# bwpriest/pyNNGP

Measured on AMD Instinct MI355X. Metric: NNGP log-lik sweeps/sec (N=1M, m=15) at 1/2/4/8 MI355X; % HBM roofline, higher is better.
Workload: dtype f64

## Files before the change

### include/nngp.h

```cpp
#ifndef NNGP_H
#define NNGP_H

#include <stddef.h>
#include <stdint.h>

#ifdef __cplusplus
extern "C" {
#endif

#define NNGP_OK 0
#define NNGP_EINVAL (-1)
#define NNGP_ENOTPD (-2)
#define NNGP_EHIP (-3)
#define NNGP_EUNSUP (-4)

#define NNGP_COV_EXPONENTIAL 0
#define NNGP_COV_MATERN32 1
#define NNGP_COV_MATERN52 2
#define NNGP_COV_GAUSSIAN 3
#define NNGP_COV_SPHERICAL 4
#define NNGP_COV_MATERN 5

#define NNGP_ALGO_AUTO 0
#define NNGP_ALGO_LANE 1
#define NNGP_ALGO_WAVE 2
#define NNGP_ALGO_QUAD 4
#define NNGP_ALGO_PAIRB 5

int32_t nngp_resolve_algo(int32_t algo, int32_t m, int32_t kind, int32_t dim);
int32_t nngp_resolve_algo_nu(int32_t algo, int32_t m, int32_t kind, int32_t dim, double nu);

#define NNGP_MAX_M 63
#define NNGP_MAX_DIM 3

const char *nngp_version(void);

#define NNGP_ABI_VERSION 4
int32_t nngp_abi_version(void);

const char *nngp_last_error(void);

size_t nngp_knn_workspace_bytes(int64_t n_points, int32_t dim, int32_t m);
int nngp_knn_prior(const double *coords, int64_t n_points, int32_t dim, int32_t m, int64_t q0, int64_t q1,
                   int32_t *nbr, void *workspace, size_t workspace_bytes, void *stream);

int nngp_knn_prior_rows(const double *coords, int64_t n_points, int32_t dim, int32_t m, const int32_t *rows,
                        int64_t n_rows, int32_t *nbr, void *workspace, size_t workspace_bytes, void *stream);

int nngp_knn_query(const double *ref, int64_t n_ref, int32_t dim, const double *query, int64_t n_query, int32_t k,
                   int32_t *nbr, void *workspace, size_t workspace_bytes, void *stream);

size_t nngp_bf_sweep_workspace_bytes(int64_t n_rows, int32_t m, int32_t kind, int32_t dim, int32_t algo);
int nngp_bf_sweep(const double *coords, int64_t n_points, int32_t dim, const int32_t *nbr, const int32_t *order,
                  int64_t n_rows, int32_t m, int64_t i0, int32_t kind, double sigma2, double phi, double tau2,
                  double nu, const double *values, double *B, double *F, double *R, double *partials, void *workspace,
                  size_t workspace_bytes, int32_t algo, void *stream);
int nngp_bf_finalize(const void *workspace, size_t workspace_bytes, int64_t n_rows, int32_t m, int32_t kind,
                     int32_t dim, int32_t algo, double *partials, void *stream);

#define NNGP_PLAN_INFO_LEN 10
int nngp_pair_plan_supported(int32_t m, int32_t kind, int32_t dim);
size_t nngp_pair_plan_bytes(int64_t n_rows, int32_t m, int32_t dim);
int nngp_pair_plan_build(const int32_t *nbr, const int32_t *order, int64_t n_rows, int32_t m, int64_t i0,
                         int64_t n_points, int32_t dim, void *plan, size_t plan_bytes, int64_t *info, void *stream);
int nngp_bf_sweep_plan(const double *coords, int64_t n_points, int32_t dim, const int32_t *nbr, const int32_t *order,
                       int64_t n_rows, int32_t m, int64_t i0, int32_t kind, double sigma2, double phi, double tau2,
                       const double *values, double *B, double *F, double *R, double *partials, void *workspace,
                       size_t workspace_bytes, const void *plan, size_t plan_bytes, const int64_t *info,
                       void *stream);

int nngp_bf_cross(const double *ref, int64_t n_ref, int32_t dim, const double *query, int64_t n_query,
                  const int32_t *nbr, const int32_t *order, int64_t n_rows, int32_t m, int64_t q0, int32_t kind,
                  double sigma2, double phi, double tau2, double nu, const double *ref_values,
                  const double *query_values,
                  double *B, double *F, double *R, double *partials, void *workspace, size_t workspace_bytes,
                  int32_t algo, void *stream);

int nngp_matern_eval(const double *u, int64_t n, double nu, double *out, void *stream);
int64_t nngp_joint_entries(int32_t m);
int nngp_joint_dist(const double *coords, int64_t n_points, int32_t dim, const double *qcoords, int64_t n_locs,
                    const int32_t *nbr, const int32_t *order, int64_t n_rows, int32_t m, int64_t i0, double *dist,
                    void *stream);
size_t nngp_bf_sweep_blocks_workspace_bytes(int64_t n_rows);
int nngp_bf_sweep_blocks(const double *cov, const int32_t *nbr, const int32_t *order, int64_t n_points, int64_t n_rows,
                         int32_t m, int64_t i0, int64_t n_locs, const double *values, const double *qvalues, double *B,
                         double *F, double *R, double *partials, void *workspace, size_t workspace_bytes, void *stream);

size_t nngp_row_order_workspace_bytes(int64_t n_rows);
int nngp_row_order(const double *coords, int64_t n_points, int32_t dim, const int32_t *nbr, int32_t m, int64_t i0,
                   int64_t n_rows, int32_t *order, int32_t *nbr_sorted, void *workspace, size_t workspace_bytes,
                   void *stream);

int nngp_combine_partials(const double *gathered, int32_t world, double *partials, void *stream);
int nngp_combine_partials_batch(const double *gathered, int32_t world, int64_t n_slots, double *partials,
                                void *stream);

size_t nngp_reverse_workspace_bytes(int64_t n, int32_t m);
int nngp_reverse_neighbors(const int32_t *nbr, int64_t n, int32_t m, int32_t *off, int32_t *rev_j, int32_t *rev_k,
                           void *workspace, size_t workspace_bytes, void *stream);
int64_t nngp_color_moral_graph(const int32_t *nbr_host, const int32_t *off_host, const int32_t *rev_j_host,
                               int64_t n, int32_t m, int32_t *color_host);
int64_t nngp_color_moral_graph_dev(const int32_t *nbr, const int32_t *off, const int32_t *rev_j, int64_t n, int32_t m,
                                   int32_t *color, void *workspace, size_t workspace_bytes, void *stream);
size_t nngp_gibbs_prep_bytes(int64_t n, int32_t m);
int nngp_gibbs_prepare(const double *B, const double *Ft, const int32_t *off, const int32_t *rev_j,
                       const int32_t *rev_k, const int32_t *order, int64_t n, int32_t m, void *prep,
                       size_t prep_bytes, void *stream);
int nngp_gibbs_member_rows(const int32_t *members, int64_t n, const int32_t *off, int32_t *member_rows, void *stream);
int nngp_gibbs_w_sweep(const int32_t *member_rows, const int32_t *color_off_host, int32_t n_colors, const void *prep,
                       int64_t n, int32_t m, double sigma2, double tau2, const double *yres, const double *noise_w,
                       double *w, double *r, const int32_t *rev_j, const double *z, uint64_t seed, uint64_t sweep,
                       void *stream);
int nngp_gibbs_w_sweep_tiles(const int32_t *tiles, const int32_t *phase_off_host, const int32_t *phase_lds_host,
                             int32_t n_phases, const int32_t *tinfo, const int32_t *tstep, int32_t ecap,
                             const int32_t *tfp, const int32_t *off, const int32_t *rev_loc, const void *prep,
                             int64_t n, int32_t m, int64_t n_entries, double sigma2, double tau2, const double *yres,
                             const double *noise_w, double *w, double *r, const double *z, void *stream);
int nngp_gibbs_w_sweep_chains(const int32_t *member_rows, const int32_t *color_off_host, int32_t n_colors,
                              int32_t chains, const void *const *prep, int64_t n, int32_t m, const double *sigma2,
                              const double *tau2, const double *const *yres, const double *noise_w, double *const *w,
                              double *const *r, const int32_t *rev_j, const double *const *z, void *stream);
int nngp_gibbs_w_sweep_chains_il(const int32_t *member_rows, const int32_t *color_off_host, int32_t n_colors,
                                 int32_t chains, const void *const *prep, int64_t n, int32_t m, const double *sigma2,
                                 const double *tau2, const double *const *yres, const double *noise_w, double *w_il,
                                 double *r_il, const int32_t *rev_j, const double *const *z, void *stream);
int nngp_gibbs_normals(int64_t n, uint64_t seed, uint64_t sweep, double *z, void *stream);
int nngp_gibbs_prepare_range(const double *B, const double *Ft, const int32_t *off, const int32_t *rev_j,
                             const int32_t *rev_k, int64_t n, int32_t m, int64_t row0, int64_t row1, void *prep,
                             size_t prep_bytes, void *stream);
int nngp_gibbs_w_color(const int32_t *member_rows, int64_t n_members, const void *prep, int64_t n, int32_t m,
                       double sigma2, double tau2, const double *yres, const double *noise_w, double *w, double *r,
                       const int32_t *rev_j, const double *z, uint64_t seed, uint64_t sweep, double *w_out,
                       void *stream);
int nngp_gibbs_w_color_dev(const int32_t *member_rows, int64_t n_members, const void *prep, int64_t n, int32_t m,
                           const double *var, const double *yres, const double *noise_w, double *w, double *r,
                           const int32_t *rev_j, const double *z, double *w_out, void *stream);
int nngp_gibbs_w_apply(const int32_t *rows, int64_t n_rows, const double *w_src, const double *B, int64_t n, int32_t m,
                       double *w, double *r, const int32_t *rev_j, const int32_t *rev_k, void *stream);
size_t nngp_gibbs_stats_workspace_bytes(int64_t n, int32_t p);
int nngp_gibbs_stats(int64_t n, const double *r, const double *Ft, const double *yres, const double *y,
                     const double *X, int32_t p, const double *w, const double *noise_w, double *out,
                     void *workspace, size_t workspace_bytes, void *stream);

int nngp_check_partials(const double *partials_host, int64_t *first_bad_row, int64_t *first_bad_index);

double nngp_loglik_from_partials(const double *partials_host, int64_t n_rows);

#ifdef __cplusplus
}
#endif
#endif
```

### pynngp_amd/_lib.py

```python
from __future__ import annotations

import ctypes
import os
from typing import Optional, Tuple

import torch

_HERE = os.path.dirname(os.path.abspath(__file__))
LIB_PATH = os.environ.get("NNGP_LIB") or os.path.join(_HERE, "_build", "libnngp_hip.so")
SYMBOLS = (
    "nngp_version",
    "nngp_abi_version",
    "nngp_last_error",
    "nngp_knn_workspace_bytes",
    "nngp_knn_prior",
    "nngp_knn_prior_rows",
    "nngp_knn_query",
    "nngp_bf_sweep_workspace_bytes",
    "nngp_bf_sweep",
    "nngp_bf_cross",
    "nngp_bf_finalize",
    "nngp_resolve_algo",
    "nngp_resolve_algo_nu",
    "nngp_loglik_from_partials",
    "nngp_check_partials",
    "nngp_row_order_workspace_bytes",
    "nngp_row_order",
    "nngp_combine_partials",
    "nngp_combine_partials_batch",
    "nngp_matern_eval",
    "nngp_joint_entries",
    "nngp_joint_dist",
    "nngp_bf_sweep_blocks_workspace_bytes",
    "nngp_bf_sweep_blocks",
    "nngp_reverse_workspace_bytes",
    "nngp_reverse_neighbors",
    "nngp_color_moral_graph",
    "nngp_gibbs_prep_bytes",
    "nngp_gibbs_prepare",
    "nngp_gibbs_member_rows",
    "nngp_gibbs_w_sweep",
    "nngp_gibbs_normals",
    "nngp_gibbs_prepare_range",
    "nngp_gibbs_w_color",
    "nngp_gibbs_w_color_dev",
    "nngp_gibbs_w_apply",
    "nngp_gibbs_stats_workspace_bytes",
    "nngp_gibbs_stats",
    "nngp_gibbs_w_sweep_chains",
    "nngp_gibbs_w_sweep_chains_il",
    "nngp_gibbs_w_sweep_tiles",
    "nngp_color_moral_graph_dev",
    "nngp_pair_plan_supported",
    "nngp_pair_plan_bytes",
    "nngp_pair_plan_build",
    "nngp_bf_sweep_plan",
)

KIND_CODES = {"exponential": 0, "matern32": 1, "matern52": 2, "gaussian": 3, "spherical": 4, "matern": 5}
MATERN_NU_MAX = 50.0
ALGO_CODES = {"auto": 0, "lane": 1, "wave": 2, "quad": 4, "pairb": 5}
MAX_M = 63
MAX_DIM = 3
ABI_VERSION = 4
PLAN_INFO_LEN = 10
BLOCKS_MAX_M = 32


class NNGPExtensionError(RuntimeError):
    """The native library is missing, failed to load, or returned an error."""


_lib = None


def load() -> ctypes.CDLL:
    global _lib
    if _lib is not None:
        return _lib
    if not os.path.exists(LIB_PATH):
        raise NNGPExtensionError(
            f"{LIB_PATH} not found: build it with `python -c 'import __graft_entry__ as g; g.build()'` "
            "or `make -C pynngp_amd/csrc` (pynngp_amd has no CPU fallback)"
        )
    lib = ctypes.CDLL(LIB_PATH)
    P, I32, I64, D, SZ = ctypes.c_void_p, ctypes.c_int32, ctypes.c_int64, ctypes.c_double, ctypes.c_size_t
    lib.nngp_version.restype = ctypes.c_char_p
    lib.nngp_abi_version.restype = I32
    if lib.nngp_abi_version() != ABI_VERSION:
        raise NNGPExtensionError(f"{LIB_PATH} has C ABI revision {lib.nngp_abi_version()}, this binding needs "
                                 f"{ABI_VERSION}: rebuild the library")
    lib.nngp_last_error.restype = ctypes.c_char_p
    lib.nngp_knn_workspace_bytes.argtypes = [I64, I32, I32]
    lib.nngp_knn_workspace_bytes.restype = SZ
    lib.nngp_knn_prior.argtypes = [P, I64, I32, I32, I64, I64, P, P, SZ, P]
    lib.nngp_knn_prior.restype = ctypes.c_int
    lib.nngp_knn_prior_rows.argtypes = [P, I64, I32, I32, P, I64, P, P, SZ, P]
    lib.nngp_knn_prior_rows.restype = ctypes.c_int
    lib.nngp_knn_query.argtypes = [P, I64, I32, P, I64, I32, P, P, SZ, P]
    lib.nngp_knn_query.restype = ctypes.c_int
    lib.nngp_bf_sweep_workspace_bytes.argtypes = [I64, I32, I32, I32, I32]
    lib.nngp_bf_sweep_workspace_bytes.restype = SZ
    lib.nngp_bf_sweep.argtypes = [P, I64, I32, P, P, I64, I32, I64, I32, D, D, D, D, P, P, P, P, P, P, SZ, I32, P]
    lib.nngp_bf_cross.argtypes = [P, I64, I32, P, I64, P, P, I64, I32, I64, I32, D, D, D, D, P, P, P, P, P, P, P, SZ,
                                  I32, P]
    lib.nngp_bf_cross.restype = ctypes.c_int
    lib.nngp_row_order_workspace_bytes.argtypes = [I64]
    lib.nngp_row_order_workspace_bytes.restype = SZ
    lib.nngp_row_order.argtypes = [P, I64, I32, P, I32, I64, I64, P, P, P, SZ, P]
    lib.nngp_row_order.restype = ctypes.c_int
    lib.nngp_combine_partials.argtypes = [P, I32, P, P]
    lib.nngp_combine_partials_batch.argtypes = [P, I32, I64, P, P]
    lib.nngp_matern_eval.argtypes = [P, I64, D, P, P]
    lib.nngp_matern_eval.restype = ctypes.c_int
    lib.nngp_joint_entries.argtypes = [I32]
    lib.nngp_joint_entries.restype = I64
    lib.nngp_joint_dist.argtypes = [P, I64, I32, P, I64, P, P, I64, I32, I64, P, P]
    lib.nngp_joint_dist.restype = ctypes.c_int
    lib.nngp_bf_sweep_blocks_workspace_bytes.argtypes = [I64]
    lib.nngp_bf_sweep_blocks_workspace_bytes.restype = SZ
    lib.nngp_bf_sweep_blocks.argtypes = [P, P, P, I64, I64, I32, I64, I64, P, P, P, P, P, P, P, SZ, P]
    lib.nngp_bf_sweep_blocks.restype = ctypes.c_int
    lib.nngp_combine_partials_batch.restype = ctypes.c_int
    lib.nngp_bf_finalize.argtypes = [P, ctypes.c_size_t, I64, I32, I32, I32, I32, P, P]
    lib.nngp_bf_finalize.restype = ctypes.c_int
    lib.nngp_resolve_algo.argtypes = [I32, I32, I32, I32]
    lib.nngp_resolve_algo.restype = I32
    lib.nngp_resolve_algo_nu.argtypes = [I32, I32, I32, I32, D]
    lib.nngp_resolve_algo_nu.restype = I32
    lib.nngp_combine_partials.restype = ctypes.c_int
    U64 = ctypes.c_uint64
    lib.nngp_reverse_workspace_bytes.argtypes = [I64, I32]
    lib.nngp_reverse_workspace_bytes.restype = SZ
    lib.nngp_reverse_neighbors.argtypes = [P, I64, I32, P, P, P, P, SZ, P]
    lib.nngp_reverse_neighbors.restype = ctypes.c_int
    lib.nngp_color_moral_graph.argtypes = [P, P, P, I64, I32, P]
    lib.nngp_color_moral_graph.restype = I64
    lib.nngp_gibbs_prep_bytes.argtypes = [I64, I32]
    lib.nngp_gibbs_prep_bytes.restype = SZ
    lib.nngp_gibbs_prepare.argtypes = [P, P, P, P, P, P, I64, I32, P, SZ, P]
    lib.nngp_gibbs_prepare.restype = ctypes.c_int
    lib.nngp_gibbs_member_rows.argtypes = [P, I64, P, P, P]
    lib.nngp_gibbs_member_rows.restype = ctypes.c_int
    lib.nngp_gibbs_w_sweep.argtypes = [P, P, I32, P, I64, I32, D, D, P, P, P, P, P, P, U64, U64, P]
    lib.nngp_gibbs_w_sweep.restype = ctypes.c_int
    lib.nngp_gibbs_normals.argtypes = [I64, U64, U64, P, P]
    lib.nngp_gibbs_normals.restype = ctypes.c_int
    lib.nngp_gibbs_prepare_range.argtypes = [P, P, P, P, P, I64, I32, I64, I64, P, SZ, P]
    lib.nngp_gibbs_prepare_range.restype = ctypes.c_int
    lib.nngp_gibbs_w_color.argtypes = [P, I64, P, I64, I32, D, D, P, P, P, P, P, P, U64, U64, P, P]
    lib.nngp_gibbs_w_color.restype = ctypes.c_int
    lib.nngp_gibbs_w_color_dev.argtypes = [P, I64, P, I64, I32, P, P, P, P, P, P, P, P, P]
    lib.nngp_gibbs_w_color_dev.restype = ctypes.c_int
    lib.nngp_gibbs_w_apply.argtypes = [P, I64, P, P, I64, I32, P, P, P, P, P]
    lib.nngp_gibbs_w_apply.restype = ctypes.c_int
    lib.nngp_gibbs_stats_workspace_bytes.argtypes = [I64, I32]
    lib.nngp_gibbs_stats_workspace_bytes.restype = SZ
    lib.nngp_gibbs_stats.argtypes = [I64, P, P, P, P, P, I32, P, P, P, P, SZ, P]
    lib.nngp_gibbs_stats.restype = ctypes.c_int
    lib.nngp_bf_sweep.restype = ctypes.c_int
    lib.nngp_color_moral_graph_dev.argtypes = [P, P, P, I64, I32, P, P, SZ, P]
    lib.nngp_color_moral_graph_dev.restype = I64
    lib.nngp_gibbs_w_sweep_tiles.argtypes = [P, P, P, I32, P, P, I32, P, P, P, P, I64, I32, I64, D, D, P, P, P, P,
                                             P, P]
    lib.nngp_gibbs_w_sweep_tiles.restype = ctypes.c_int
    lib.nngp_gibbs_w_sweep_chains.argtypes = [P, P, I32, I32, P, I64, I32, P, P, P, P, P, P, P, P, P]
    lib.nngp_gibbs_w_sweep_chains.restype = ctypes.c_int
    lib.nngp_gibbs_w_sweep_chains_il.argtypes = [P, P, I32, I32, P, I64, I32, P, P, P, P, P, P, P, P, P]
    lib.nngp_gibbs_w_sweep_chains_il.restype = ctypes.c_int
    lib.nngp_pair_plan_supported.argtypes = [I32, I32, I32]
    lib.nngp_pair_plan_supported.restype = ctypes.c_int
    lib.nngp_pair_plan_bytes.argtypes = [I64, I32, I32]
    lib.nngp_pair_plan_bytes.restype = SZ
    lib.nngp_pair_plan_build.argtypes = [P, P, I64, I32, I64, I64, I32, P, SZ, P, P]
    lib.nngp_pair_plan_build.restype = ctypes.c_int
    lib.nngp_bf_sweep_plan.argtypes = [P, I64, I32, P, P, I64, I32, I64, I32, D, D, D, P, P, P, P, P, P, SZ, P, SZ, P,
                                       P]
    lib.nngp_bf_sweep_plan.restype = ctypes.c_int
    lib.nngp_check_partials.argtypes = [P, P, P]
    lib.nngp_check_partials.restype = ctypes.c_int
    lib.nngp_loglik_from_partials.argtypes = [P, I64]
    lib.nngp_loglik_from_partials.restype = D
    _lib = lib
    return lib


def version() -> str:
    return load().nngp_version().decode()


def resolve_algo(algo: str, m: int, kind: str, dim: int, nu: Optional[float] = None) -> str:
    if nu is not None:
        code = load().nngp_resolve_algo_nu(ALGO_CODES[algo], int(m), KIND_CODES[kind], int(dim), float(nu))
    else:
        code = load().nngp_resolve_algo(ALGO_CODES[algo], int(m), KIND_CODES[kind], int(dim))
    names = {v: k for k, v in ALGO_CODES.items()}
    return names.get(code, str(code))


def _check(rc: int, what: str) -> None:
    if rc != 0:
        msg = load().nngp_last_error().decode()
        raise NNGPExtensionError(f"{what} failed ({rc}): {msg}")


def _require_gpu(*tensors: Optional[torch.Tensor]) -> torch.device:
    dev = None
    for t in tensors:
        if t is None:
            continue
        if t.device.type != "cuda":
            raise NNGPExtensionError(
                f"pynngp_amd needs ROCm GPU tensors (got {t.device}); there is no CPU fallback"
            )
        if dev is None:
            dev = t.device
        elif t.device != dev:
            raise NNGPExtensionError(f"tensors on different devices: {dev} vs {t.device}")
    if dev is None:
        raise NNGPExtensionError("no tensor arguments")
    return dev


def _ptr(t: Optional[torch.Tensor]):
    return ctypes.c_void_p(t.data_ptr()) if t is not None else None


def _stream(dev: torch.device):
    return ctypes.c_void_p(torch.cuda.current_stream(dev).cuda_stream)


def _workspace(nbytes: int, dev: torch.device) -> torch.Tensor:
    ws = torch.empty(max(int(nbytes), 256), dtype=torch.uint8, device=dev)
    ws[:256].zero_()
    return ws


def _as_coords(coords: torch.Tensor) -> torch.Tensor:
    if coords.dim() != 2 or not 1 <= coords.shape[1] <= MAX_DIM or coords.dtype != torch.float64:
        raise ValueError(f"coords must be float64 (N, dim), 1 <= dim <= {MAX_DIM}, got {tuple(coords.shape)} "
                         f"{coords.dtype}")
    return coords.contiguous()


def _same_dim(*coords: torch.Tensor) -> int:
    dims = {c.shape[1] for c in coords}
    if len(dims) != 1:
        raise ValueError(f"coordinate arrays of different dimensions: {sorted(dims)}")
    return dims.pop()


def _check_out(t: Optional[torch.Tensor], name: str, shape, dev: torch.device) -> None:
    if t is None:
        return
    if t.dtype != torch.float64 or tuple(t.shape) != tuple(shape) or not t.is_contiguous() or t.device != dev:
        raise ValueError(f"{name} must be a contiguous float64 {tuple(shape)} tensor on {dev}, got "
                         f"{t.dtype} {tuple(t.shape)} contiguous={t.is_contiguous()} on {t.device}")


def knn_prior(coords: torch.Tensor, m: int, q0: int = 0, q1: Optional[int] = None,
              out: Optional[torch.Tensor] = None) -> torch.Tensor:
# ... 36 lines not shown
    query = _as_coords(query)
    d = _same_dim(ref, query)
    dev = _require_gpu(ref, query)
    out = torch.empty((query.shape[0], k), dtype=torch.int32, device=dev)
    lib = load()
    ws = _workspace(lib.nngp_knn_workspace_bytes(ref.shape[0], d, k), dev)
    _check(lib.nngp_knn_query(_ptr(ref), ref.shape[0], d, _ptr(query), query.shape[0], k, _ptr(out), _ptr(ws),
                              ws.numel(), _stream(dev)), "nngp_knn_query")
    return out


def _check_kind(kind: str, nu: Optional[float]) -> float:
    if kind not in KIND_CODES:
        raise ValueError(f"unknown covariance kind {kind!r}; expected one of {sorted(KIND_CODES)}")
    if kind == "matern":
        if nu is None or not 0.0 < float(nu) <= MATERN_NU_MAX:
            raise ValueError(f"the matern kind needs a smoothness 0 < nu <= {MATERN_NU_MAX:g} (got {nu!r})")
        return float(nu)
    return -1.0


class PairPlan:

    def __init__(self, buf: torch.Tensor, info, nbr: torch.Tensor, order: Optional[torch.Tensor]):
        self.buf = buf
        self.info = (ctypes.c_int64 * PLAN_INFO_LEN)(*info)
        self.n_planned, self.n_direct = int(info[0]), int(info[1])
        self.n_rows, self.m, self.dim, self.i0, self.n_points = (int(v) for v in info[2:7])
        self._nbr_ptr, self._order_ptr = nbr.data_ptr(), (order.data_ptr() if order is not None else 0)
        self._versions = (nbr._version, order._version if order is not None else 0)

    def matches(self, nbr: torch.Tensor, order: Optional[torch.Tensor], i0: int, n_points: int, dim: int) -> bool:
        return (nbr.data_ptr() == self._nbr_ptr and (order.data_ptr() if order is not None else 0) == self._order_ptr
                and (nbr._version, order._version if order is not None else 0) == self._versions
                and tuple(nbr.shape) == (self.n_rows, self.m) and i0 == self.i0 and n_points == self.n_points
                and dim == self.dim)


def pair_plan_read_bytes(buf: torch.Tensor, m: int) -> int:
    hdr = buf[:256].view(torch.int64).cpu()
    nreg, sb = int(hdr[6]), int(hdr[9])
    if nreg == 0:
        return 0
    wsb = sb // 4
    w = buf[256:256 + nreg * sb].view(nreg * 4, wsb)[:, :12].contiguous().view(torch.int32).long().cpu()
    nU, nE, st = w[:, 0], w[:, 1].clamp(min=0), w[:, 2]
    planned = (st.view(nreg, 4) == 0).all(1).repeat_interleave(4)
    np_ = (m + 2) // 2
    che = (np_ * np_ + 7) // 8
    per = 12 + che * 1024 + 256 + 256 * ((nU + 63) // 64) + 1024 * ((nE + 255) // 256)
    return int(per[planned].sum())


def pair_plan_supported(m: int, kind: str, dim: int) -> bool:
    return kind in KIND_CODES and bool(load().nngp_pair_plan_supported(int(m), KIND_CODES[kind], int(dim)))


def pair_plan(nbr: torch.Tensor, n_points: int, dim: int, i0: int = 0,
              order: Optional[torch.Tensor] = None) -> PairPlan:
    if nbr.dtype != torch.int32 or nbr.dim() != 2:
        raise ValueError(f"nbr must be int32 (rows, m), got {nbr.dtype} {tuple(nbr.shape)}")
    nbr = nbr.contiguous()
    dev = _require_gpu(nbr, order)
    rows, m = nbr.shape
    if order is not None and (order.dtype != torch.int32 or order.shape != (rows,)):
        raise ValueError("order must be int32 (rows,)")
    lib = load()
    nbytes = lib.nngp_pair_plan_bytes(rows, m, dim)
    if nbytes == 0:
        raise NNGPExtensionError(f"no pair plans for m={m}, dim={dim} (2 <= m <= 17, dim 1..3)")
    buf = _workspace(nbytes, dev)
    info = (ctypes.c_int64 * PLAN_INFO_LEN)()
    _check(lib.nngp_pair_plan_build(_ptr(nbr), _ptr(order), rows, m, int(i0), int(n_points), int(dim), _ptr(buf),
                                    buf.numel(), info, _stream(dev)), "nngp_pair_plan_build")
    return PairPlan(buf, list(info), nbr, order)


def bf_sweep(coords: torch.Tensor, nbr: torch.Tensor, i0: int, kind: str, sigma2: float, phi: float,
             tau2: float = 0.0, values: Optional[torch.Tensor] = None, want_bf: bool = True,
             algo: str = "auto", B: Optional[torch.Tensor] = None, F: Optional[torch.Tensor] = None,
             partials: Optional[torch.Tensor] = None, workspace: Optional[torch.Tensor] = None,
             order: Optional[torch.Tensor] = None,
             R: Optional[torch.Tensor] = None,
             defer: bool = False, nu: Optional[float] = None, plan: Optional[PairPlan] = None
             ) -> Tuple[Optional[torch.Tensor], Optional[torch.Tensor], torch.Tensor]:
    coords = _as_coords(coords)
    if nbr.dtype != torch.int32 or nbr.dim() != 2:
        raise ValueError(f"nbr must be int32 (rows, m), got {nbr.dtype} {tuple(nbr.shape)}")
    nbr = nbr.contiguous()
    if values is not None:
        if values.dtype != torch.float64 or values.shape != (coords.shape[0],):
            raise ValueError("values must be float64 (N,)")
        values = values.contiguous()
    dev = _require_gpu(coords, nbr, values, order)
    rows, m = nbr.shape
    if order is not None and (order.dtype != torch.int32 or order.shape != (rows,)):
        raise ValueError("order must be int32 (rows,)")
    nu = _check_kind(kind, nu)
    lib = load()
    a = ALGO_CODES[algo]
    if want_bf:
        _check_out(B, "B", (rows, m), dev)
        _check_out(F, "F", (rows,), dev)
        B = torch.empty((rows, m), dtype=torch.float64, device=dev) if B is None else B
        F = torch.empty((rows,), dtype=torch.float64, device=dev) if F is None else F
    else:
        B = F = None
    if defer:
        partials = None
    else:
        _check_out(partials, "partials", (4,), dev)
        partials = torch.empty(4, dtype=torch.float64, device=dev) if partials is None else partials
    d = coords.shape[1]
    need = lib.nngp_bf_sweep_workspace_bytes(rows, m, KIND_CODES[kind], d, a)
    if workspace is None or workspace.numel() < need:
        if defer:
            raise ValueError("defer=True needs a workspace of nngp_bf_sweep_workspace_bytes bytes")
        workspace = _workspace(need, dev)
    _check_out(R, "R", (rows,), dev)
    if workspace.device != dev or not workspace.is_contiguous():
        raise ValueError("workspace must be a contiguous tensor on the sweep's device")
    if plan is not None:
        if algo not in ("auto", "pairb"):
            raise ValueError(f"a pair plan runs the pair kernel, not algo {algo!r}")
        if not isinstance(plan, PairPlan) or plan.buf.device != dev:
            raise ValueError("plan must be a PairPlan on the sweep's device")
        if not plan.matches(nbr, order, i0, coords.shape[0], d):
            raise ValueError("stale pair plan: it was built for other nbr / order tensors (or they were modified in "
                             "place since) or another geometry; rebuild it with pair_plan")
        _check(lib.nngp_bf_sweep_plan(_ptr(coords), coords.shape[0], d, _ptr(nbr), _ptr(order), rows, m, i0,
                                      KIND_CODES[kind], float(sigma2), float(phi), float(tau2), _ptr(values), _ptr(B),
                                      _ptr(F), _ptr(R), _ptr(partials), _ptr(workspace), workspace.numel(),
                                      _ptr(plan.buf), plan.buf.numel(), plan.info, _stream(dev)),
               "nngp_bf_sweep_plan")
        return B, F, partials
    _check(lib.nngp_bf_sweep(_ptr(coords), coords.shape[0], d, _ptr(nbr), _ptr(order), rows, m, i0, KIND_CODES[kind],
                             float(sigma2), float(phi), float(tau2), nu, _ptr(values), _ptr(B), _ptr(F), _ptr(R),
                             _ptr(partials), _ptr(workspace), workspace.numel(), a, _stream(dev)),
           "nngp_bf_sweep")
    return B, F, partials


def bf_finalize(workspace: torch.Tensor, rows: int, m: int, kind: str, dim: int, algo: str = "auto",
                out: Optional[torch.Tensor] = None) -> torch.Tensor:
    dev = _require_gpu(workspace, out)
    out = torch.empty(4, dtype=torch.float64, device=dev) if out is None else out
    if not workspace.is_contiguous():
        raise ValueError("workspace must be contiguous")
    _check(load().nngp_bf_finalize(_ptr(workspace), workspace.numel() * workspace.element_size(), int(rows), int(m),
                                   KIND_CODES[kind], int(dim), ALGO_CODES[algo], _ptr(out), _stream(dev)),
           "nngp_bf_finalize")
    return out


def bf_cross(ref: torch.Tensor, query: torch.Tensor, nbr: torch.Tensor, kind: str, sigma2: float, phi: float,
             tau2: float = 0.0, ref_values: Optional[torch.Tensor] = None,
             query_values: Optional[torch.Tensor] = None, q0: int = 0, algo: str = "auto",
             B: Optional[torch.Tensor] = None, F: Optional[torch.Tensor] = None,
             partials: Optional[torch.Tensor] = None, workspace: Optional[torch.Tensor] = None,
             order: Optional[torch.Tensor] = None,
             R: Optional[torch.Tensor] = None, nu: Optional[float] = None) -> Tuple[torch.Tensor, torch.Tensor, torch.Tensor]:
    ref, query = _as_coords(ref), _as_coords(query)
    d = _same_dim(ref, query)
    if nbr.dtype != torch.int32 or nbr.dim() != 2:
        raise ValueError(f"nbr must be int32 (rows, m), got {nbr.dtype} {tuple(nbr.shape)}")
    nbr = nbr.contiguous()
    if ref_values is not None:
        if ref_values.dtype != torch.float64 or ref_values.shape != (ref.shape[0],):
            raise ValueError("ref_values must be float64 (n_ref,)")
        ref_values = ref_values.contiguous()
    if query_values is not None:
        if query_values.dtype != torch.float64 or query_values.shape != (query.shape[0],):
            raise ValueError("query_values must be float64 (n_query,)")
        query_values = query_values.contiguous()
    dev = _require_gpu(ref, query, nbr, ref_values, query_values, order)
    rows, m = nbr.shape
    if order is not None and (order.dtype != torch.int32 or order.shape != (rows,)):
        raise ValueError("order must be int32 (rows,)")
    nu = _check_kind(kind, nu)
    lib = load()
    a = ALGO_CODES[algo]
    _check_out(B, "B", (rows, m), dev)
    _check_out(F, "F", (rows,), dev)
    _check_out(partials, "partials", (4,), dev)
    _check_out(R, "R", (rows,), dev)
    B = torch.empty((rows, m), dtype=torch.float64, device=dev) if B is None else B
    F = torch.empty((rows,), dtype=torch.float64, device=dev) if F is None else F
    partials = torch.empty(4, dtype=torch.float64, device=dev) if partials is None else partials
    need = lib.nngp_bf_sweep_workspace_bytes(rows, m, KIND_CODES[kind], d, a)
    if workspace is None or workspace.numel() < need:
        workspace = _workspace(need, dev)
    _check(lib.nngp_bf_cross(_ptr(ref), ref.shape[0], d, _ptr(query), query.shape[0], _ptr(nbr), _ptr(order), rows, m,
                             int(q0), KIND_CODES[kind], float(sigma2), float(phi), float(tau2), nu, _ptr(ref_values),
                             _ptr(query_values), _ptr(B), _ptr(F), _ptr(R), _ptr(partials), _ptr(workspace),
                             workspace.numel(), a, _stream(dev)), "nngp_bf_cross")
    return B, F, partials


def joint_dist(coords: torch.Tensor, nbr: torch.Tensor, i0: int = 0, qcoords: Optional[torch.Tensor] = None,
               order: Optional[torch.Tensor] = None, out: Optional[torch.Tensor] = None) -> torch.Tensor:
    coords = _as_coords(coords)
    qcoords = coords if qcoords is None else _as_coords(qcoords)
    d = _same_dim(coords, qcoords)
    if nbr.dtype != torch.int32 or nbr.dim() != 2:
        raise ValueError(f"nbr must be int32 (rows, m), got {nbr.dtype} {tuple(nbr.shape)}")
    nbr = nbr.contiguous()
    dev = _require_gpu(coords, qcoords, nbr, order)
    rows, m = nbr.shape
    if order is not None and (order.dtype != torch.int32 or order.shape != (rows,)):
        raise ValueError("order must be int32 (rows,)")
    lib = load()
    ne = int(lib.nngp_joint_entries(m))
    _check_out(out, "out", (ne, rows), dev)
    out = torch.empty((ne, rows), dtype=torch.float64, device=dev) if out is None else out
    _check(lib.nngp_joint_dist(_ptr(coords), coords.shape[0], d, _ptr(qcoords), qcoords.shape[0], _ptr(nbr),
                               _ptr(order), rows, m, int(i0), _ptr(out), _stream(dev)), "nngp_joint_dist")
    return out


def matern(u: torch.Tensor, nu: float) -> torch.Tensor:
    if u.dtype != torch.float64:
        raise ValueError("u must be float64")
    dev = _require_gpu(u)
# ... 353 lines not shown
```

### pynngp_amd/csrc/bf_pairb.h

```cpp
#pragma once
#include <hip/hip_runtime.h>
#include <stdint.h>
#include <stdlib.h>
#include <string.h>

#include "bf_group.h"
#include "nngp_internal.h"
#include "nngp_math.h"
#include "pair_plan.h"

namespace nngp {

constexpr int kPairbDedupMax = 17;
constexpr int kPairbLeftMin = 18;
constexpr int kPairbLeftOneWaveMin = 23;
constexpr int kPairbLeftLdsRows = 5;
constexpr int kPairbLeftLdsRows1W = 7;
constexpr int kPairbLeftMaternM = 18;
constexpr int kPairbLeftLdsRowsMT = 6;
constexpr bool pairb_left(int m) { return m >= kPairbLeftMin && m <= 32; }
constexpr bool pairb_lk(int m, int kind) {
    return pairb_left(m) && (kind != NNGP_KIND_MATERN || m == kPairbLeftMaternM) &&
           (kind != NNGP_KIND_BLOCKS || m <= 24);
}
#ifndef NNGP_PHASE
#define NNGP_PHASE(name)
#endif
__device__ __forceinline__ double pr_swap(double v) { return dpp_f64<0xB1>(v); }
__device__ __forceinline__ double pr_from0(double v) { return dpp_f64<0xA0>(v); }
__device__ __forceinline__ double pr_from1(double v) { return dpp_f64<0xF5>(v); }
__device__ __forceinline__ double pr_sel(bool q1, double v1, double v0) { return q1 ? v1 : v0; }
__device__ __forceinline__ double pr_pick(uint32_t mask1, double v1, double v0) {
    const long long a = __double_as_longlong(v1), b = __double_as_longlong(v0);
    const uint32_t lo = ((uint32_t)a & mask1) | ((uint32_t)b & ~mask1);
    const uint32_t hi = ((uint32_t)(a >> 32) & mask1) | ((uint32_t)(b >> 32) & ~mask1);
    return __hiloint2double((int)hi, (int)lo);
}

constexpr int kPairbTwoWavesMax = 18;
constexpr int kPairbThreeWavesMax = 13;
constexpr int pairb_waves_per_simd(int m, int kind) {
    return m <= kPairbThreeWavesMax ? 3
           : (pairb_lk(m, kind) && kind == NNGP_KIND_MATERN) ? 1
           : (m <= kPairbTwoWavesMax || (pairb_lk(m, kind) && m < kPairbLeftOneWaveMin)) ? 2
                                                                                          : 1;
}
#define NNGP_PAIRB_ATTR \
    __attribute__((amdgpu_waves_per_eu(pairb_waves_per_simd(M, KIND), M <= kPairbThreeWavesMax ? 3 : 2)))

constexpr int kPairbThreads = 256;
constexpr int kPairbWaves = kPairbThreads / 64;
constexpr int kPairbTile = kPairbThreads / 2;
constexpr int kDeviceCUs = 256;

struct PairbTiling {
    int64_t tiles, q, rem;
};
inline PairbTiling pairb_tiling(int64_t n_rows, int m, int kind) {
    (void)m;
    (void)kind;
    const int64_t T = (n_rows + kPairbTile - 1) / kPairbTile;
    if (T == 0) return {0, 0, 0};
    return {T, n_rows / T, n_rows % T};
}
inline int64_t pairb_tiles_bound(int64_t n_rows) {
    const int64_t T = (n_rows + kPairbTile - 1) / kPairbTile;
    const int64_t b = T + 3 * kDeviceCUs - 1 < n_rows / 97 ? T + 3 * kDeviceCUs - 1 : n_rows / 97;
    return b > T ? b : T;
}

__device__ __forceinline__ void pairb_tile_store(double lm, int le, double qq, double badp, double badi,
                                                 double (*sh)[kPairbWaves][5], int par, double4* __restrict__ rec,
                                                 int32_t* __restrict__ lexp, int64_t tile) {
#pragma unroll
    for (int o = 32; o > 1; o >>= 1) {
        lm *= __shfl_xor(lm, o);
        le += __shfl_xor(le, o);
        qq += __shfl_xor(qq, o);
    }
    if (__any(badp != INFINITY || badi != INFINITY)) {
        badp = wave_min(badp);
        badi = wave_min(badi);
    }
    const int w = threadIdx.x >> 6;
    if ((threadIdx.x & 63) == 0) {
        sh[par][w][0] = lm;
        sh[par][w][1] = (double)le;
        sh[par][w][2] = qq;
        sh[par][w][3] = badp;
        sh[par][w][4] = badi;
    }
}

__device__ __forceinline__ void pairb_tile_fold(double (*sh)[kPairbWaves][5], int par, double4* __restrict__ rec,
                                                int32_t* __restrict__ lexp, int64_t tile) {
    double lm = 1.0, le = 0.0, qq = 0.0, bp = INFINITY, bi = INFINITY;
#pragma unroll
    for (int k = 0; k < kPairbWaves; ++k) {
        lm *= sh[par][k][0];
        le += sh[par][k][1];
        qq += sh[par][k][2];
        bp = fmin(bp, sh[par][k][3]);
        bi = fmin(bi, sh[par][k][4]);
    }
    rec[tile] = make_double4(__builtin_amdgcn_frexp_mant(lm), qq, bp, bi);
    lexp[tile] = (int32_t)le + __builtin_amdgcn_frexp_exp(lm);
// ... 25 lines not shown

__device__ __forceinline__ void pairb_fold_records(const double4* __restrict__ rec, const int32_t* __restrict__ lexp,
                                                   int64_t n_tiles, double* __restrict__ partials,
                                                   double (*sh)[5]) {
    constexpr int NT = kPairbThreads;
    const int t = threadIdx.x;
    double a = 1.0, e = 0.0, b = 0.0, c = INFINITY, d = INFINITY;
    for (int64_t k0 = t; k0 < n_tiles; k0 += 8 * NT) {
        double4 r[8];
        int32_t x[8];
#pragma unroll
        for (int u = 0; u < 8; ++u) {
            const int64_t k = k0 + (int64_t)u * NT;
            r[u] = k < n_tiles ? rec[k] : make_double4(1.0, 0.0, INFINITY, INFINITY);
            x[u] = k < n_tiles ? lexp[k] : 0;
        }
        double pm = 1.0;
        int32_t pe = 0;
#pragma unroll
        for (int u = 0; u < 8; ++u) {
            pm *= r[u].x;
            pe += x[u];
            b += r[u].y;
            c = fmin(c, r[u].z);
            d = fmin(d, r[u].w);
        }
        a *= pm;
        e += (double)pe;
        mant_norm(a, e);
    }
    a = wave_fold_dpp<1>(a);
    e = wave_fold_dpp<0>(e);
    mant_norm(a, e);
    b = wave_fold_dpp<0>(b);
    c = wave_fold_dpp<2>(c);
    d = wave_fold_dpp<2>(d);
    if ((t & 63) == 0) {
        sh[t >> 6][0] = a;
        sh[t >> 6][1] = e;
        sh[t >> 6][2] = b;
        sh[t >> 6][3] = c;
        sh[t >> 6][4] = d;
    }
    __syncthreads();
    if (t == 0) {
        a = 1.0, e = 0.0, b = 0.0, c = INFINITY, d = INFINITY;
#pragma unroll
        for (int w = 0; w < NT / 64; ++w) {
            a *= sh[w][0];
            e += sh[w][1];
            b += sh[w][2];
            c = fmin(c, sh[w][3]);
            d = fmin(d, sh[w][4]);
        }
        partials[0] = fma(e, 0.6931471805599453, log(a));
        partials[1] = b;
        partials[2] = c == INFINITY ? -1.0 : c;
        partials[3] = d == INFINITY ? -1.0 : d;
    }
}

__device__ __forceinline__ double pr_rcp(double x) {
    const double y = __builtin_amdgcn_rcp(x);
    const double e = fma(-x, y, 1.0);
    return fma(y, fma(e, e, e), y);
}

struct PairPlanArgs {
    const uint8_t* slots = nullptr;
    const int32_t* tiles = nullptr;
    int64_t slot_bytes = 0;
    int64_t n_tiles = 0;
};

template <int M, int KIND, int D, bool PL = false>
__global__ __launch_bounds__(kPairbThreads) NNGP_PAIRB_ATTR void bf_pairb(const double* __restrict__ coords, int64_t n_points,
                                                const int32_t* __restrict__ nbr, const int32_t* __restrict__ order,
                                                int64_t n_rows, int64_t i0, const CovParams Pc, double sigma2,
                                                const double* __restrict__ values, const double* __restrict__ qcoords,
                                                const double* __restrict__ qvalues, double* __restrict__ Bout,
                                                double* __restrict__ Fout, double* __restrict__ Rout,
                                                double4* __restrict__ rec, int32_t* __restrict__ lexp, int dim,
                                                const double* __restrict__ cblk, int64_t tq, int64_t trem,
                                                int64_t* __restrict__ hdr, const PairPlanArgs pp) {
    static_assert(M >= 1 && M <= 32, "pairb instantiated for 1 <= m <= 32");
    static_assert(D >= 0 && D <= 3, "0 (runtime dimension) <= D <= 3");
    constexpr bool CM = KIND == NNGP_KIND_BLOCKS;
    constexpr bool MT = KIND == NNGP_KIND_MATERN;
    constexpr int DA = point_arity<D>();
    const int ds = D == 0 ? dim : D;
    constexpr int NR = M + 1;
    constexpr int NP = (NR + 1) / 2;
    constexpr int T = M / 2;
    constexpr bool LEFT = !PL && pairb_lk(M, KIND);
    static_assert(!PL || (!CM && !MT && !LEFT && D >= 1 && M >= kPlanMinM && M <= kPlanMaxM),
                  "pair plans: the right-looking fused kinds, 1 <= D <= 3");
    constexpr int PSL = PL ? plan_slice_bytes(M) : 16;
    __shared__ __attribute__((aligned(16))) double wsl[PL ? kPairbWaves * PSL / 8 : 1];
    constexpr bool SLDL = !LEFT;
    constexpr int KL0 = MT ? kPairbLeftLdsRowsMT
                           : (M >= kPairbLeftOneWaveMin ? kPairbLeftLdsRows1W : kPairbLeftLdsRows);
    constexpr int KL = !LEFT ? 0 : (KL0 < M / 2 - 1 ? KL0 : M / 2 - 1);
    constexpr int LXW = (NP + 3 + 1) / 2;
    __shared__ double lbuf[LEFT ? NNGP_EXP_TAB_N + (KL * (KL + 1) + LXW) * kPairbThreads : 1];
    double(*const lrow)[kPairbThreads] = (double(*)[kPairbThreads])(lbuf + NNGP_EXP_TAB_N);
    int32_t(*const lidx)[kPairbThreads] =
        (int32_t(*)[kPairbThreads])(lbuf + NNGP_EXP_TAB_N + KL * (KL + 1) * kPairbThreads);
    __shared__ double etab_own[MT || LEFT ? 1 : NNGP_EXP_TAB_N];
    double* const etab = LEFT ? lbuf : etab_own;
    extern __shared__ double4 pairb_mtab[];
    const double* ctab = MT ? (const double*)pairb_mtab : etab;
    constexpr int kTabPer = kPairbThreads >= NNGP_EXP_TAB_N ? 1 : NNGP_EXP_TAB_N / kPairbThreads;
    static_assert(kPairbThreads >= NNGP_EXP_TAB_N || kTabPer * kPairbThreads == NNGP_EXP_TAB_N, "table fill");
    double etab_entry[kTabPer];
    if constexpr (!CM && !MT) {
#pragma unroll
        for (int e = 0; e < kTabPer; ++e)
            etab_entry[e] = nngp_exp_table_entry_unit(((int)threadIdx.x + e * kPairbThreads) & (NNGP_EXP_TAB_N - 1));
    }

    __shared__ double sh[1][kPairbWaves][5];
    const int64_t ltile = xcd_logical_block(blockIdx.x, gridDim.x);
    const int64_t tile = pp.tiles != nullptr ? (int64_t)__builtin_amdgcn_readfirstlane(pp.tiles[ltile]) : ltile;
    if (blockIdx.x == 0 && threadIdx.x == 0) hdr[0] = pp.tiles != nullptr ? pp.n_tiles : gridDim.x;
    const int q = (int)(threadIdx.x & 1);
    const bool q1 = q == 1;
    const bool lead0 = !q1;
    const double wq1 = q1 ? 1.0 : 0.0, wq0 = 1.0 - wq1;
    uint32_t mask1 = q1 ? 0xffffffffu : 0u;
    asm volatile("" : "+v"(mask1));
    {
        const int64_t lr = threadIdx.x >> 1;
        const int64_t r = tile * tq + (tile < trem ? tile : trem) + lr;
        const bool live = lr < tq + (tile < trem ? 1 : 0);
        const int64_t rl = live ? r : n_rows - 1;
        const int32_t ov = (order != nullptr ? order : nbr)[rl];
        const int64_t rr = order != nullptr ? (int64_t)ov : rl;
        const int64_t i = i0 + rr;

        int32_t jn[NP];
#pragma unroll
        for (int s = 0; s < NP; ++s) {
            const int a = 2 * s + q;
            jn[s] = nbr[rl * M + (a < M ? a : M - 1)];
        }
        double o[NP][DA], z[NP];
        const uint32_t n32 = n_points < (int64_t)0x80000000ll ? (uint32_t)n_points : 0x80000000u;
        int32_t jmax = -1, jmin = -1;
#pragma unroll
        for (int s = 0; s < NP; ++s) {
            const int a = 2 * s + q;
            const int32_t j = a < M ? jn[s] : -1;
            jmax = max(jmax, j);
            jmin = min(jmin, j);
            const bool in_range = (uint32_t)j < n32;
            const bool self = a == M;
            const double* pc = self ? qcoords + i * ds : (in_range ? coords + (int64_t)j * ds : far_point<DA>(a));
            const double* pv = self ? (qvalues != nullptr ? qvalues + i : kZeroValue)
                                    : ((values != nullptr && in_range) ? values + j : kZeroValue);
            if constexpr (CM || PL) {
            } else if constexpr (D == 0) {
                load_point_rt(pc, dim, o[s]);
            } else {
                load_point<D>(pc, o[s]);
            }
            if constexpr (!LEFT) z[s] = *pv;
        }
        const bool bad_index = (int64_t)jmax >= n_points || jmin < -1;
        if constexpr (LEFT) {
#pragma unroll
            for (int s = 0; s < NP; ++s) lidx[s][threadIdx.x] = jn[s];
            lidx[NP][threadIdx.x] = (int32_t)(uint32_t)(uint64_t)rr;
            lidx[NP + 1][threadIdx.x] = (int32_t)(uint32_t)((uint64_t)rr >> 32);
            lidx[NP + 2][threadIdx.x] = bad_index ? 1 : 0;
        }

        if constexpr (MT) {
            const int n4 = Pc.mt_noct * (NNGP_MT_K * NNGP_MT_NC / 4);
            const double4* g = (const double4*)cblk;
            for (int k = (int)threadIdx.x; k < n4; k += kPairbThreads) pairb_mtab[k] = g[k];
            __syncthreads();
        } else if constexpr (!CM && !PL) {
#pragma unroll
            for (int e = 0; e < kTabPer; ++e)
                if (kPairbThreads <= NNGP_EXP_TAB_N || threadIdx.x < NNGP_EXP_TAB_N)
                    etab[threadIdx.x + e * kPairbThreads] = etab_entry[e];
            __syncthreads();
        }

        double R[NP][NP][2];
        bool bad = false;
        bool stale_plan = false;
        double Fu, res;
        if constexpr (PL) {
            constexpr int CHE = plan_map_chunks(M);
            constexpr int PS = plan_ps(DA);
            constexpr int UK = plan_ucap(M) / 64;
            constexpr int64_t WSB = plan_wave_slot_bytes(M);
            const int wv = (int)(threadIdx.x >> 6), L = (int)(threadIdx.x & 63);
            const uint8_t* wsp = pp.slots + tile * pp.slot_bytes + (int64_t)__builtin_amdgcn_readfirstlane(wv) * WSB;
            const int nU0 = __builtin_amdgcn_readfirstlane(((const int32_t*)wsp)[0]);
            const int nE0 = __builtin_amdgcn_readfirstlane(((const int32_t*)wsp)[1]);
            const int st0 = __builtin_amdgcn_readfirstlane(((const int32_t*)wsp)[2]);
            const bool over = st0 != 0 || nU0 < 0 || nU0 > plan_ucap(M) || nE0 < 0 || nE0 > plan_ecap(M) ||
                              !plan_fits(nU0, nE0, PS, PSL);
            const int nU = over ? 0 : nU0, nE = over ? 0 : nE0;
            bad = over;
            const __amdgpu_buffer_rsrc_t srd =
                __builtin_amdgcn_make_buffer_rsrc((void*)wsp, (short)0, (int)WSB, 0x00020000);
            typedef uint32_t u32x4 __attribute__((ext_vector_type(4)));
            uint32_t mw[4 * CHE];
#pragma unroll
            for (int c = 0; c < CHE; ++c) {
                const u32x4 v = __builtin_amdgcn_raw_buffer_load_b128(srd, plan_map_off(M) + 16 * L, c * 64 * 16, 0);
                mw[4 * c] = v.x;
                mw[4 * c + 1] = v.y;
                mw[4 * c + 2] = v.z;
                mw[4 * c + 3] = v.w;
            }
            const uint32_t ck = __builtin_amdgcn_raw_buffer_load_b32(srd, plan_chk_off(M) + 4 * L, 0, 0);
            int32_t ug[UK];
#pragma unroll
            for (int k = 0; k < UK; ++k)
                ug[k] = (int32_t)__builtin_amdgcn_raw_buffer_load_b32(srd, plan_u_off() + 4 * L, 256 * k, 0);
            static_assert(kPlanPairGroup == 4, "one 16-byte word load per lane and group");
            constexpr int PG = kPlanPairGroup;
            constexpr int KG = plan_pair_groups(M);
            const int ngr = (nE + 64 * PG - 1) / (64 * PG);
            u32x4 wg[KG];
#pragma unroll
            for (int g = 0; g < KG; ++g)
                wg[g] = (g < 2 || g < ngr) ? __builtin_amdgcn_raw_buffer_load_b128(srd, plan_pair_off(M) + 16 * L, 1024 * g, 0)
                                           : u32x4{0u, 0u, 0u, 0u};
#pragma unroll
            for (int e = 0; e < kTabPer; ++e)
                if (kPairbThreads <= NNGP_EXP_TAB_N || threadIdx.x < NNGP_EXP_TAB_N)
                    etab[threadIdx.x + e * kPairbThreads] = etab_entry[e];
            __syncthreads();
            NNGP_PHASE(plan_points);
            char* const sl = (char*)wsl + wv * PSL;
            const int cb = PSL - nU * PS;
#pragma unroll
            for (int k = 0; k < UK; ++k) {
                if (64 * k < nU) {
                    const uint32_t g = (uint32_t)ug[k] < (uint32_t)n_points ? (uint32_t)ug[k] : 0u;
                    double x[DA];
                    load_point<DA>(coords + (int64_t)g * ds, x);
                    if (L + 64 * k < nU) {
                        double* pd = (double*)(sl + cb + (L + 64 * k) * PS);
                        if constexpr (DA == 2) {
                            *(double2*)pd = make_double2(x[0], x[1]);
// ... 45 lines not shown
            pair_points(wg[0], xa0, xb0);
            u32x4 wA = wg[KG > 1 ? 1 : 0], wB;
#pragma unroll 1
            for (int g = 0; g < ngr; g += 2) {
                wB = group_words(g + 2);
                pair_points(wA, xa1, xb1);
                pair_covs(g, xa0, xb0);
                if (g + 1 >= ngr) break;
                wA = group_words(g + 3);
                pair_points(wB, xa0, xb0);
                pair_covs(g + 1, xa1, xb1);
            }
            if (L == 0) *(double*)sl = 0.0;
            asm volatile("" ::: "memory");
            __builtin_amdgcn_wave_barrier();
            NNGP_PHASE(plan_fill);
            auto rd = [&](int e) -> double {
                const uint32_t off = (e & 1) ? (mw[e >> 1] >> 16) : (mw[e >> 1] & 0xffffu);
                return *(const double*)(sl + off);
            };
            int e = 0;
#pragma unroll
            for (int s = 0; s < NP; ++s) {
#pragma unroll
                for (int t = 0; t < s; ++t) {
                    R[s][t][0] = rd(e++);
                    R[s][t][1] = rd(e++);
                }
                R[s][s][0] = Pc.diag;
                R[s][s][1] = rd(e++);
            }
            uint32_t h = plan_chk_init((uint32_t)(uint64_t)rr);
#pragma unroll
            for (int s = 0; s < NP; ++s) h = plan_chk_step(h, jn[s], s);
            const int stale = h != ck ? 1 : 0;
            stale_plan = (stale | __builtin_amdgcn_mov_dpp(stale, 0xB1, 0xf, 0xf, true)) != 0;
        }
        uint32_t vm = 0;
        if constexpr (CM) {
#pragma unroll
            for (int s = 0; s < NP; ++s) {
                const int a = 2 * s + q;
                const bool ok = a == M || (a < M && (uint32_t)jn[s] < n32);
                vm |= ok ? (1u << a) : 0u;
            }
            vm |= (uint32_t)__builtin_amdgcn_mov_dpp((int)vm, 0xB1, 0xf, 0xf, true);
        }
        const double* cb = cblk + rl;
        auto ldc2 = [&](int a0, int b0, int a1, int b1) -> double {
            const int e0 = (a0 * (a0 + 1) >> 1) + b0, e1 = (a1 * (a1 + 1) >> 1) + b1;
            const uint32_t need = q1 ? ((1u << a1) | (1u << b1)) : ((1u << a0) | (1u << b0));
            const bool ok = (vm & need) == need;
            const int64_t e = ok ? (q1 ? e1 : e0) : 0;
            const double v = cb[e * n_rows];
            return ok ? v : 0.0;
        };
        if constexpr (CM && !LEFT) {
#pragma unroll
            for (int s = 0; s < NP; ++s) {
                const int a0 = 2 * s, a1 = 2 * s + 1;
#pragma unroll
                for (int t = 0; t < s; ++t) {
                    R[s][t][0] = ldc2(a0, 2 * t, a1, 2 * t + 1);
                    R[s][t][1] = ldc2(a0, 2 * t + 1, a1, 2 * t);
                }
                const double dg = ldc2(a0, a0, a1, a1);
                R[s][s][0] = ((vm >> (2 * s + q)) & 1u) ? dg : 1.0;
                const double w = ldc2(a0, a0, a1, a0);
                R[s][s][1] = q1 ? w : 0.0;
            }
        }
        if constexpr (!LEFT) {
        NNGP_PHASE(covariances);
        if constexpr (!CM && !PL) {
            double p[NP][DA];
#pragma unroll
            for (int t = 0; t < NP; ++t)
#pragma unroll
                for (int k = 0; k < DA; ++k) p[t][k] = pr_swap(o[t][k]);
#pragma unroll
            for (int s = 0; s < NP; ++s) {
#pragma unroll
                for (int t = 0; t < s; ++t) {
                    R[s][t][0] = nngp_cov_unit<KIND>(Pc, ctab, point_d2<DA>(o[s], o[t]));
                    R[s][t][1] = nngp_cov_unit<KIND>(Pc, ctab, point_d2<DA>(o[s], p[t]));
                }
                R[s][s][0] = Pc.diag;
            }
#pragma unroll
            for (int s0 = 0; s0 < NP; s0 += 2) {
                const int s1 = s0 + 1;
                if (M <= kPairbDedupMax && s1 < NP) {
                    double a[DA], b[DA];
#pragma unroll
                    for (int k = 0; k < DA; ++k) {
                        a[k] = pr_pick(mask1, o[s1][k], o[s0][k]);
                        b[k] = pr_pick(mask1, p[s1][k], p[s0][k]);
                    }
                    const double c = nngp_cov_unit<KIND>(Pc, ctab, point_d2<DA>(a, b));
                    R[s1][s1][1] = c;
                    R[s0][s0][1] = pr_from0(c);
                } else {
                    R[s0][s0][1] = nngp_cov_unit<KIND>(Pc, ctab, point_d2<DA>(o[s0], p[s0]));
                    if (s1 < NP) R[s1][s1][1] = nngp_cov_unit<KIND>(Pc, ctab, point_d2<DA>(o[s1], p[s1]));
                }
            }
        }

        NNGP_PHASE(elimination);
        if constexpr (SLDL) {
#pragma unroll
            for (int t = 0; t < T; ++t) {
                const double d00 = pr_from0(R[t][t][0]);
                const double d11 = pr_from1(R[t][t][0]);
                const double d10 = pr_from1(R[t][t][1]);
                bad |= !(d00 > 0.0);
                const double r00 = pr_rcp(d00);
                const double l10 = d10 * r00;
                const double e11 = fma(-l10, d10, d11);
                bad |= !(e11 > 0.0);
                const double r11 = pr_rcp(e11);
                R[t][t][1] = l10;
                const double town = pr_sel(q1, r11, r00), toth = pr_sel(q1, r00, r11);
                const double g1 = -l10 * wq1, g0 = -l10 * wq0;
#pragma unroll
                for (int s = t + 1; s < NP; ++s) {
                    const double x0 = R[s][t][0], x1 = R[s][t][1];
                    R[s][t][0] = fma(g1, x1, x0);
                    R[s][t][1] = fma(g0, x0, x1);
                }
#pragma unroll
                for (int u = t + 1; u < NP; ++u) {
                    const double Q0 = R[u][t][0] * town, Q1 = R[u][t][1] * toth;
                    const double P0 = pr_swap(Q0), P1 = pr_swap(Q1);
#pragma unroll
                    for (int s = u; s < NP; ++s) {
                        const double w0 = R[s][t][0], w1 = R[s][t][1];
                        R[s][u][0] = fma(-w0, Q0, fma(-w1, Q1, R[s][u][0]));
                        R[s][u][1] = fma(-w0, P1, fma(-w1, P0, R[s][u][1]));
                    }
                    R[u][t][0] = Q0;
                    R[u][t][1] = Q1;
                }
            }
        } else {
#pragma unroll
        for (int t = 0; t < T; ++t) {
            const double a00 = pr_from0(R[t][t][0]);
            const double a11 = pr_from1(R[t][t][0]);
            const double a10 = pr_from1(R[t][t][1]);
            bad |= !(a00 > 0.0);
            const double i00 = nngp_rsqrt(a00);
            const double l10 = a10 * i00;
            const double s11 = fma(-l10, l10, a11);
            bad |= !(s11 > 0.0);
            const double i11 = nngp_rsqrt(s11);
            R[t][t][0] = pr_sel(q1, i11, i00);
            R[t][t][1] = l10;
            const double u01 = -(l10 * i00) * i11;
            const double c00 = pr_sel(q1, i11, i00), c10 = u01 * wq1;
            const double c01 = u01 * wq0, c11 = pr_sel(q1, i00, i11);
#pragma unroll
            for (int s = t + 1; s < NP; ++s) {
                const double x0 = R[s][t][0], x1 = R[s][t][1];
                const double y0 = fma(x0, c00, x1 * c10);
                const double y1 = fma(x0, c01, x1 * c11);
                R[s][t][0] = y0;
                R[s][t][1] = y1;
            }
#pragma unroll
            for (int u = t + 1; u < NP; ++u) {
                const double S0 = R[u][t][0], S1 = R[u][t][1];
                const double P0 = pr_swap(S0), P1 = pr_swap(S1);
#pragma unroll
                for (int s = u; s < NP; ++s) {
                    const double y0 = R[s][t][0], y1 = R[s][t][1];
                    R[s][u][0] = fma(-y0, S0, fma(-y1, S1, R[s][u][0]));
                    R[s][u][1] = fma(-y0, P1, fma(-y1, P0, R[s][u][1]));
                }
            }
        }
        }

        NNGP_PHASE(lastpair);
        if (M % 2 == 1 && SLDL) {
            const double a00 = pr_from0(R[T][T][0]);
            const double a11 = pr_from1(R[T][T][0]);
            const double a10 = pr_from1(R[T][T][1]);
            bad |= !(a00 > 0.0);
            const double l10 = a10 * pr_rcp(a00);
            Fu = fma(-l10, a10, a11);
            R[T][T][0] = 1.0;
            R[T][T][1] = l10;
        } else if (M % 2 == 1) {
            const double a00 = pr_from0(R[T][T][0]);
            const double a11 = pr_from1(R[T][T][0]);
            const double a10 = pr_from1(R[T][T][1]);
            bad |= !(a00 > 0.0);
            const double i00 = nngp_rsqrt(a00);
            const double l10 = a10 * i00;
            Fu = fma(-l10, l10, a11);
            R[T][T][0] = i00;
            R[T][T][1] = l10;
        } else {
            Fu = pr_from0(R[T][T][0]);
        }
        } else {
            NNGP_PHASE(leftlooking);
            double pnext[DA], wpnext = 0.0;
#pragma unroll
            for (int u = 0; u < NP; ++u) {
                if constexpr (CM) {
#pragma unroll
                    for (int s = u + 1; s < NP; ++s) {
                        R[s][u][0] = ldc2(2 * s, 2 * u, 2 * s + 1, 2 * u + 1);
                        R[s][u][1] = ldc2(2 * s, 2 * u + 1, 2 * s + 1, 2 * u);
                    }
                    const double dg = ldc2(2 * u, 2 * u, 2 * u + 1, 2 * u + 1);
                    R[u][u][0] = ((vm >> (2 * u + q)) & 1u) ? dg : 1.0;
                    const double wv = ldc2(2 * u, 2 * u, 2 * u + 1, 2 * u);
                    R[u][u][1] = q1 ? wv : 0.0;
                } else {
                double pu[DA];
#pragma unroll
                for (int k = 0; k < DA; ++k) pu[k] = (u % 2 == 1) ? pnext[k] : pr_swap(o[u][k]);
#pragma unroll
                for (int s = u + 1; s < NP; ++s) {
                    R[s][u][0] = nngp_cov_unit<KIND>(Pc, ctab, point_d2<DA>(o[s], o[u]));
                    R[s][u][1] = nngp_cov_unit<KIND>(Pc, ctab, point_d2<DA>(o[s], pu));
                }
                R[u][u][0] = Pc.diag;
                if (u % 2 == 0 && u + 1 < NP) {
                    double a[DA], b[DA];
#pragma unroll
                    for (int k = 0; k < DA; ++k) {
                        pnext[k] = pr_swap(o[u + 1][k]);
                        a[k] = pr_pick(mask1, o[u + 1][k], o[u][k]);
                        b[k] = pr_pick(mask1, pnext[k], pu[k]);
                    }
                    wpnext = nngp_cov_unit<KIND>(Pc, ctab, point_d2<DA>(a, b));
                    R[u][u][1] = pr_from0(wpnext);
                } else if (u % 2 == 1) {
                    R[u][u][1] = wpnext;
                } else {
                    R[u][u][1] = nngp_cov_unit<KIND>(Pc, ctab, point_d2<DA>(o[u], pu));
                }
                }
#pragma unroll
                for (int t = 0; t < u; ++t) {
                    const double S0 = R[u][t][0], S1 = R[u][t][1];
                    const double P0 = pr_swap(S0), P1 = pr_swap(S1);
#pragma unroll
                    for (int s = u; s < NP; ++s) {
                        const double y0 = R[s][t][0], y1 = R[s][t][1];
                        R[s][u][0] = fma(-y0, S0, fma(-y1, S1, R[s][u][0]));
                        R[s][u][1] = fma(-y0, P1, fma(-y1, P0, R[s][u][1]));
                    }
                }
                if (u < T) {
                    const double a00 = pr_from0(R[u][u][0]);
                    const double a11 = pr_from1(R[u][u][0]);
                    const double a10 = pr_from1(R[u][u][1]);
                    bad |= !(a00 > 0.0);
                    const double i00 = nngp_rsqrt(a00);
                    const double l10 = a10 * i00;
                    const double s11 = fma(-l10, l10, a11);
                    bad |= !(s11 > 0.0);
                    const double i11 = nngp_rsqrt(s11);
                    R[u][u][0] = pr_sel(q1, i11, i00);
                    R[u][u][1] = l10;
                    const double u01 = -(l10 * i00) * i11;
                    const double c00 = pr_sel(q1, i11, i00), c10 = u01 * wq1;
                    const double c01 = u01 * wq0, c11 = pr_sel(q1, i00, i11);
#pragma unroll
                    for (int s = u + 1; s < NP; ++s) {
                        const double x0 = R[s][u][0], x1 = R[s][u][1];
                        R[s][u][0] = fma(x0, c00, x1 * c10);
                        R[s][u][1] = fma(x0, c01, x1 * c11);
                    }
                } else if (M % 2 == 1) {
                    const double a00 = pr_from0(R[T][T][0]);
                    const double a11 = pr_from1(R[T][T][0]);
                    const double a10 = pr_from1(R[T][T][1]);
                    bad |= !(a00 > 0.0);
                    const double i00 = nngp_rsqrt(a00);
                    const double l10 = a10 * i00;
                    Fu = fma(-l10, l10, a11);
                    R[T][T][0] = i00;
                    R[T][T][1] = l10;
                } else {
                    Fu = pr_from0(R[T][T][0]);
                }
                if (u < KL) {
#pragma unroll
                    for (int t = 0; t <= u; ++t) {
                        lrow[u * (u + 1) + 2 * t][threadIdx.x] = R[u][t][0];
                        lrow[u * (u + 1) + 2 * t + 1][threadIdx.x] = R[u][t][1];
                    }
                }
            }
        }
        auto RB = [&](int u, int t, int k) -> double {
            if (u < KL) return lrow[u * (u + 1) + 2 * t + k][threadIdx.x];
            return R[u][t][k];
        };
        bad |= !(Fu > 0.0);
        const double F = Fu * sigma2;
        int64_t rrl = rr, il = i;
        bool bidx = bad_index || stale_plan;
        if constexpr (LEFT) {
            __builtin_amdgcn_fence(__ATOMIC_ACQUIRE, "workgroup");
            rrl = (int64_t)(((uint64_t)(uint32_t)lidx[NP + 1][threadIdx.x] << 32) | (uint32_t)lidx[NP][threadIdx.x]);
            il = i0 + rrl;
            bidx = lidx[NP + 2][threadIdx.x] != 0;
        }

        {
            constexpr int SM = M / 2;
            constexpr bool VQ1 = (M % 2) == 1;
            NNGP_PHASE(backsub);
            if constexpr (LEFT) {
#pragma unroll
                for (int s = 0; s < NP; ++s) {
                    const int a = 2 * s + q;
                    const int32_t j = a < M ? lidx[s][threadIdx.x] : -1;
                    const bool in_range = (uint32_t)j < n32;
                    const double* pv = a == M ? (qvalues != nullptr ? qvalues + il : kZeroValue)
                                              : ((values != nullptr && in_range) ? values + j : kZeroValue);
                    z[s] = *pv;
                }
            }
            double bown[NP];
#pragma unroll
            for (int s = 0; s < NP; ++s) bown[s] = 0.0;
            if (M % 2 == 1) bown[T] = RB(T, T, 1) * RB(T, T, 0);
#pragma unroll
            for (int t = T - 1; t >= 0; --t) {
                double acc0 = 0.0, acc1 = 0.0;
#pragma unroll
                for (int u = t + 1; u < NP; ++u) {
                    if (2 * u >= M) continue;
                    const bool row_ok = 2 * u + 1 < M;
                    double bu = bown[u];
                    if (!row_ok) bu = q1 ? 0.0 : bu;
                    acc0 = fma(RB(u, t, 0), bu, acc0);
                    acc1 = fma(RB(u, t, 1), bu, acc1);
                }
                const double tot = acc0 + pr_swap(acc1);
                const double vrow0 = RB(SM, t, 0), vrow1 = RB(SM, t, 1);
                double v;
                if (VQ1) {
                    v = pr_sel(q1, vrow0, pr_swap(vrow1));
                } else {
                    v = pr_sel(q1, pr_swap(vrow1), vrow0);
                }
                const double l10 = RB(t, t, 1);
                double bx, b0;
                if constexpr (SLDL) {
                    bx = v - tot;
                    b0 = fma(-l10, pr_swap(bx), bx);
                } else {
                    const double iown = RB(t, t, 0);
                    bx = (v - tot) * iown;
                    b0 = fma(-(l10 * iown), pr_swap(bx), bx);
                }
                bown[t] = pr_sel(q1, bx, b0);
            }
            NNGP_PHASE(residual);
            {
                double acc = 0.0;
#pragma unroll
                for (int s = 0; s < NP; ++s) {
                    if (2 * s >= M) continue;
                    double bs = bown[s];
                    if (2 * s + 1 >= M) bs = q1 ? 0.0 : bs;
                    acc = fma(bs, z[s], acc);
                }
                const double zm = z[SM];
                const double vi = VQ1 ? pr_from1(zm) : pr_from0(zm);
                res = vi - (acc + pr_swap(acc));
            }
            NNGP_PHASE(stores);
            if (Bout != nullptr && live) {
                const double bscale = (bad || stale_plan) ? NAN : 1.0;
#pragma unroll
                for (int s = 0; s < NP; ++s) {
                    const int a = 2 * s + q;
                    if (a < M) Bout[rrl * M + a] = bown[s] * bscale;
                }
            }
        }
        NNGP_PHASE(tail);
        const bool lead = live && lead0;
        if (Fout != nullptr && lead) Fout[rrl] = (bad || stale_plan) ? NAN : F;
        if (Rout != nullptr && lead) Rout[rrl] = (bad || stale_plan) ? NAN : res;
        pairb_tile_store(lead ? __builtin_amdgcn_frexp_mant(F) : 1.0, lead ? __builtin_amdgcn_frexp_exp(F) : 0,
                         lead ? res * res * pr_rcp(F) : 0.0, (lead && bad) ? (double)il : INFINITY,
                         (live && bidx) ? (double)il : INFINITY, sh, 0, rec, lexp, tile);
        __syncthreads();
        if (threadIdx.x == 0) pairb_tile_fold(sh, 0, rec, lexp, tile);
    }
}

inline size_t pairb_align(size_t b) { return (b + 255) & ~(size_t)255; }
constexpr size_t kPairbHeader = 256;
inline size_t bf_pairb_workspace_bytes(int64_t n_rows) {
    const int64_t t = pairb_tiles_bound(n_rows);
    return t > 0 ? kPairbHeader + pairb_align((size_t)t * 32) + pairb_align((size_t)t * 4) : 0;
}
inline int64_t* pairb_hdr(void* ws) { return (int64_t*)ws; }
inline double4* pairb_rec(void* ws) { return (double4*)((char*)ws + kPairbHeader); }
inline int32_t* pairb_lexp(void* ws, int64_t n_rows) {
    return (int32_t*)((char*)ws + kPairbHeader + pairb_align((size_t)pairb_tiles_bound(n_rows) * 32));
}

template <int M, int KIND, int D, bool PL = false>
static void launch_pairb_mkd(const BfArgs& a, const CovParams& Pc, hipStream_t s, const PairPlanArgs* ppl = nullptr) {
    const size_t lds = KIND == NNGP_KIND_MATERN ? NNGP_MT_BYTES(Pc.mt_noct) : 0;
    const PairbTiling tl = pairb_tiling(a.n_rows, M, KIND);
    PairPlanArgs pp = ppl != nullptr ? *ppl : PairPlanArgs{};
    if (!PL && a.tiles != nullptr) {
        pp.tiles = a.tiles;
        pp.n_tiles = a.n_tiles;
    }
    const int64_t nb = PL ? a.n_plan_blocks : (a.tiles != nullptr ? a.n_tile_list : tl.tiles);
    if (nb == 0) return;
    hipLaunchKernelGGL((bf_pairb<M, KIND, D, PL>), dim3((unsigned)nb), dim3(kPairbThreads), lds, s, a.coords,
                       a.n_points, a.nbr, a.order, a.n_rows, a.i0, Pc, KIND == NNGP_KIND_BLOCKS ? 1.0 : a.sigma2, a.values,
                       a.qcoords, a.qvalues, a.B, a.F, a.R, pairb_rec(a.bpart), pairb_lexp(a.bpart, a.n_rows), a.dim,
                       a.cblk, tl.q, tl.rem, pairb_hdr(a.bpart), pp);
}

template <int M, int KIND, int D>
static void launch_pairb_planned_mkd(const BfArgs& a, const CovParams& Pc, const PlanLaunch& pl, hipStream_t s) {
    PairPlanArgs pp;
    pp.slots = pl.plan + kPlanGlobalHdr;
    pp.slot_bytes = pl.slot_bytes;
    pp.n_tiles = pl.n_regions;
    pp.tiles = pl.planned;
    BfArgs b = a;
    b.n_plan_blocks = pl.n_planned;
    launch_pairb_mkd<M, KIND, D, true>(b, Pc, s, &pp);
}

template <int M, int D>
static bool launch_pairb_planned_if(const BfArgs& a, const CovParams& Pc, const PlanLaunch& pl, hipStream_t s) {
    if (a.m != M || a.dim != D) return false;
    switch (a.kind) {
        case 0: launch_pairb_planned_mkd<M, 0, D>(a, Pc, pl, s); return true;
        case 1: launch_pairb_planned_mkd<M, 1, D>(a, Pc, pl, s); return true;
        case 2: launch_pairb_planned_mkd<M, 2, D>(a, Pc, pl, s); return true;
        case 3: launch_pairb_planned_mkd<M, 3, D>(a, Pc, pl, s); return true;
        case 4: launch_pairb_planned_mkd<M, 4, D>(a, Pc, pl, s); return true;
        default: return false;
    }
}

template <int M>
static bool launch_pairb_generic_if(const BfArgs& a, const CovParams& Pc, hipStream_t s) {
    if (a.m != M) return false;
    launch_pairb_mkd<M, NNGP_KIND_GENERIC, 0>(a, Pc, s);
    return true;
}

template <int M>
static bool launch_pairb_blocks_if(const BfArgs& a, const CovParams& Pc, hipStream_t s) {
    if (a.m != M) return false;
    launch_pairb_mkd<M, NNGP_KIND_BLOCKS, 2>(a, Pc, s);
    return true;
}

template <int M, int D>
static bool launch_pairb_if(const BfArgs& a, const CovParams& Pc, hipStream_t s) {
    if (a.m != M || a.dim != D) return false;
    switch (a.kind) {
        case 0: launch_pairb_mkd<M, 0, D>(a, Pc, s); return true;
        case 1: launch_pairb_mkd<M, 1, D>(a, Pc, s); return true;
        case 2: launch_pairb_mkd<M, 2, D>(a, Pc, s); return true;
        case 3: launch_pairb_mkd<M, 3, D>(a, Pc, s); return true;
        case 4: launch_pairb_mkd<M, 4, D>(a, Pc, s); return true;
        case NNGP_KIND_MATERN:
            if constexpr (M <= 24) {
                launch_pairb_mkd<M, NNGP_KIND_MATERN, D>(a, Pc, s);
                return true;
            } else {
                return false;
            }
        default: return false;
    }
}

}
```

### pynngp_amd/csrc/capi.hip

```cpp
#include <hip/hip_runtime.h>
#include <math.h>
#include <stdarg.h>
#include <stdio.h>
#include <string.h>

#include "../../include/nngp.h"
#include "nngp_internal.h"
#include "bf_pairb.h"

namespace {
thread_local char g_err[512] = "";

int fail(int code, const char* fmt, ...) {
    va_list ap;
    va_start(ap, fmt);
    vsnprintf(g_err, sizeof g_err, fmt, ap);
    va_end(ap);
    return code;
}

int hip_fail(hipError_t e, const char* what) {
    return fail(NNGP_EHIP, "%s: %s", what, hipGetErrorString(e));
}

size_t align256(size_t x) { return (x + 255) & ~(size_t)255; }

int resolve_algo(int32_t algo, int32_t m, int32_t kind, int32_t dim) {
    (void)dim;
    if (algo != NNGP_ALGO_AUTO) return algo;
    if (kind == NNGP_COV_MATERN)
        return m >= 1 && m <= 24 ? nngp::kAlgoPairB : (m >= 25 && m <= 32 ? nngp::kAlgoQuad : nngp::kAlgoWave);
    if (m >= 1 && m <= 32) return m == 31 ? nngp::kAlgoQuad : nngp::kAlgoPairB;
    return nngp::kAlgoWave;
}

int resolve_algo_nu(int32_t algo, int32_t m, int32_t kind, int32_t dim, double nu) {
    const int a = resolve_algo(algo, m, kind, dim);
    if (algo != NNGP_ALGO_AUTO || kind != NNGP_COV_MATERN || (a != nngp::kAlgoPairB && a != nngp::kAlgoQuad)) return a;
    int e0, noct;
    return nu > 0.0 && nu <= NNGP_MATERN_NU_MAX && nngp::matern_table_extent(nu, &e0, &noct) ? a : nngp::kAlgoWave;
}

int64_t bf_blocks(int64_t n_rows, int algo, int m) { return nngp::bf_record_count(n_rows, algo, m); }
}

extern "C" {

const char* nngp_version(void) { return "pynngp_amd 0.4.0 gfx950"; }

int32_t nngp_abi_version(void) { return NNGP_ABI_VERSION; }

const char* nngp_last_error(void) { return g_err; }

int32_t nngp_resolve_algo(int32_t algo, int32_t m, int32_t kind, int32_t dim) { return resolve_algo(algo, m, kind, dim); }

int32_t nngp_resolve_algo_nu(int32_t algo, int32_t m, int32_t kind, int32_t dim, double nu) {
    return resolve_algo_nu(algo, m, kind, dim, nu);
}

int nngp_check_partials(const double* p, int64_t* first_bad_row, int64_t* first_bad_index) {
    if (p == nullptr) return fail(NNGP_EINVAL, "partials must be non-null");
    if (first_bad_row != nullptr) *first_bad_row = p[2] >= 0.0 ? (int64_t)p[2] : -1;
    if (first_bad_index != nullptr) *first_bad_index = p[3] >= 0.0 ? (int64_t)p[3] : -1;
    if (p[3] >= 0.0) return fail(NNGP_EINVAL, "neighbour index out of range at location %lld", (long long)p[3]);
    if (p[2] >= 0.0) return fail(NNGP_ENOTPD, "C_N or F not positive definite at location %lld", (long long)p[2]);
    return NNGP_OK;
}

double nngp_loglik_from_partials(const double* p, int64_t n_rows) {
    return -0.5 * ((double)n_rows * 1.8378770664093453 + p[0] + p[1]);
}

size_t nngp_bf_sweep_workspace_bytes(int64_t n_rows, int32_t m, int32_t kind, int32_t dim, int32_t algo) {
    if (n_rows < 0 || m < 0 || m > NNGP_MAX_M) return 0;
    const int a = resolve_algo(algo, m, kind, dim);
    const int64_t nbw = n_rows > 0 ? bf_blocks(n_rows, nngp::kAlgoWave, m) : 0;
    if (kind == NNGP_COV_MATERN && a == nngp::kAlgoPairB) {
        const size_t pb = nngp::bf_pairb_workspace_bytes(n_rows) + align256(NNGP_MT_BYTES(NNGP_MT_MAX_OCT));
        const size_t wb = align256((size_t)nbw * 4 * sizeof(double));
        return algo == NNGP_ALGO_AUTO && wb > pb ? wb : pb;
    }
    if (kind == NNGP_COV_MATERN && a == nngp::kAlgoQuad) {
        const int64_t nq = n_rows > 0 ? bf_blocks(n_rows, nngp::kAlgoQuad, m) : 0;
        const size_t qb = align256((size_t)nq * 4 * sizeof(double)) + align256(NNGP_MT_BYTES(NNGP_MT_MAX_OCT));
        const size_t wb = align256((size_t)nbw * 4 * sizeof(double));
        return algo == NNGP_ALGO_AUTO && wb > qb ? wb : qb;
    }
    if (a == nngp::kAlgoPairB) return nngp::bf_pairb_workspace_bytes(n_rows);
    const int64_t nb = n_rows > 0 ? bf_blocks(n_rows, a, m) : 0;
    return align256((size_t)nb * 4 * sizeof(double));
}

static int bf_common(const double* coords, int64_t n_points, int32_t dim, const double* qcoords, int64_t n_locs,
                     const int32_t* nbr, const int32_t* order, int64_t n_rows, int32_t m, int64_t i0, int32_t kind,
                     double sigma2, double phi, double tau2, double nu, const double* values, const double* qvalues, double* B,
                     double* F, double* R, double* partials, void* workspace, size_t workspace_bytes, int32_t algo,
                     void* stream) {
    if (coords == nullptr || qcoords == nullptr || workspace == nullptr)
        return fail(NNGP_EINVAL, "coordinates and workspace must be non-null");
    if (dim < 1 || dim > NNGP_MAX_DIM) return fail(NNGP_EUNSUP, "dim=%d outside [1, %d]", dim, NNGP_MAX_DIM);
    if (m < 0 || m > NNGP_MAX_M) return fail(NNGP_EUNSUP, "m=%d outside [0, %d]", m, NNGP_MAX_M);
    if (m > 0 && n_rows > 0 && nbr == nullptr) return fail(NNGP_EINVAL, "nbr must be non-null for m > 0");
    if (n_points < 1 || n_rows < 0 || i0 < 0 || i0 + n_rows > n_locs)
        return fail(NNGP_EINVAL, "rows [%lld, %lld) outside [0, %lld)", (long long)i0, (long long)(i0 + n_rows),
                    (long long)n_locs);
    if (kind < NNGP_COV_EXPONENTIAL || kind > NNGP_COV_MATERN) return fail(NNGP_EINVAL, "unknown kind %d", kind);
    if (!(sigma2 > 0.0) || !(phi > 0.0) || !(tau2 >= 0.0) || !isfinite(sigma2) || !isfinite(phi) || !isfinite(tau2))
        return fail(NNGP_EINVAL, "theta must satisfy sigma2 > 0, phi > 0, tau2 >= 0 (finite)");
    if (kind == NNGP_COV_MATERN && !(nu > 0.0 && nu <= NNGP_MATERN_NU_MAX))
        return fail(NNGP_EINVAL, "the matern kind needs 0 < nu <= %g (nu=%g)", NNGP_MATERN_NU_MAX, nu);
    if (B != nullptr && F == nullptr) return fail(NNGP_EINVAL, "B given without F");
    if (F != nullptr && B == nullptr && m > 0 && n_rows > 0) return fail(NNGP_EINVAL, "F given without B");
    if (R != nullptr && values == nullptr) return fail(NNGP_EINVAL, "R (residuals) needs values");
    if (((uintptr_t)workspace & 255) != 0) return fail(NNGP_EINVAL, "workspace must be 256-byte aligned");
    int a = resolve_algo_nu(algo, m, kind, dim, nu);
    if (a != nngp::kAlgoLane && a != nngp::kAlgoWave && a != nngp::kAlgoQuad && a != nngp::kAlgoPairB)
        return fail(NNGP_EINVAL, "unknown algo %d", algo);
    if (kind == NNGP_COV_MATERN && a != nngp::kAlgoWave && a != nngp::kAlgoPairB && a != nngp::kAlgoQuad)
        return fail(NNGP_EUNSUP, "the matern kind runs on the pair (m <= 24), four-lane (25..32) or wavefront kernel, "
                                 "not algo %d", algo);
    if (kind == NNGP_COV_MATERN && (a == nngp::kAlgoPairB || a == nngp::kAlgoQuad)) {
        int e0, noct;
        if (!nngp::matern_table_extent(nu, &e0, &noct))
            return fail(NNGP_EUNSUP, "matern nu=%g needs %d table octaves (> %d; nu below ~%g): use NNGP_ALGO_AUTO or "
                                     "WAVE", nu, noct, NNGP_MT_MAX_OCT, NNGP_MT_NU_MIN);
    }
    const bool classic = dim == 2 && kind <= NNGP_COV_MATERN32;
    if (a == nngp::kAlgoLane && !classic)
        return fail(NNGP_EUNSUP, "the lane kernel serves 2-D exponential and Matern-3/2 only "
                                 "(kind=%d, dim=%d): use NNGP_ALGO_AUTO, PAIRB, QUAD or WAVE", kind, dim);
    if (a == nngp::kAlgoLane && (m < 1 || m > nngp::kLaneMaxM))
        return fail(NNGP_EUNSUP, "lane kernel needs 1 <= m <= %d (m=%d)", nngp::kLaneMaxM, m);
    if (a == nngp::kAlgoQuad && !nngp::bf_group_supported(m, 4))
        return fail(NNGP_EUNSUP, "no 4-lane kernel instantiated for m=%d (25..32)", m);
    if (a == nngp::kAlgoPairB && !nngp::bf_pairb_supported(m))
        return fail(NNGP_EUNSUP, "no blocked pair kernel instantiated for m=%d", m);
    if (a == nngp::kAlgoPairB && kind == NNGP_COV_MATERN && m > 24)
        return fail(NNGP_EUNSUP, "the matern kind runs on the pair kernel for m <= 24 (m=%d): use NNGP_ALGO_AUTO or "
                                 "QUAD", m);
    const size_t need = nngp_bf_sweep_workspace_bytes(n_rows, m, kind, dim, algo);
    if (workspace_bytes < need)
        return fail(NNGP_EINVAL, "workspace too small: %zu < %zu bytes", workspace_bytes, need);

    hipStream_t s = (hipStream_t)stream;
    nngp::BfArgs args{coords, n_points, nbr, n_rows, i0, m, kind, dim, sigma2, phi, tau2, nu, order, values, qcoords,
                      qvalues, B, F, R, partials, (double*)workspace};
    hipError_t e = nngp::bf_launch(args, a, s);
    if (e != hipSuccess) return hip_fail(e, "bf_sweep launch");
    return NNGP_OK;
}

int nngp_bf_sweep(const double* coords, int64_t n_points, int32_t dim, const int32_t* nbr, const int32_t* order,
                  int64_t n_rows, int32_t m, int64_t i0, int32_t kind, double sigma2, double phi, double tau2,
                  double nu, const double* values, double* B, double* F, double* R, double* partials, void* workspace,
                  size_t workspace_bytes, int32_t algo, void* stream) {
    return bf_common(coords, n_points, dim, coords, n_points, nbr, order, n_rows, m, i0, kind, sigma2, phi, tau2, nu,
                     values, values, B, F, R, partials, workspace, workspace_bytes, algo, stream);
}

int nngp_bf_cross(const double* ref, int64_t n_ref, int32_t dim, const double* query, int64_t n_query,
                  const int32_t* nbr, const int32_t* order, int64_t n_rows, int32_t m, int64_t q0, int32_t kind,
                  double sigma2, double phi, double tau2, double nu, const double* ref_values,
                  const double* query_values, double* B, double* F, double* R, double* partials, void* workspace,
                  size_t workspace_bytes, int32_t algo, void* stream) {
    if (query_values != nullptr && ref_values == nullptr)
        return fail(NNGP_EINVAL, "query_values need ref_values");
    return bf_common(ref, n_ref, dim, query, n_query, nbr, order, n_rows, m, q0, kind, sigma2, phi, tau2, nu, ref_values,
                     query_values, B, F, R, partials, workspace, workspace_bytes, algo, stream);
}

int nngp_pair_plan_supported(int32_t m, int32_t kind, int32_t dim) {
    return nngp::bf_pairb_planned_supported(m, kind, dim) ? 1 : 0;
}

size_t nngp_pair_plan_bytes(int64_t n_rows, int32_t m, int32_t dim) {
    if (n_rows < 0 || n_rows > INT32_MAX || !nngp::bf_pairb_planned_supported(m, 0, dim)) return 0;
    return (size_t)nngp::plan_total_bytes(n_rows, m);
}

int nngp_pair_plan_build(const int32_t* nbr, const int32_t* order, int64_t n_rows, int32_t m, int64_t i0,
                         int64_t n_points, int32_t dim, void* plan, size_t plan_bytes, int64_t* info, void* stream) {
    if (plan == nullptr || info == nullptr || (n_rows > 0 && nbr == nullptr))
        return fail(NNGP_EINVAL, "plan, info (and nbr for n_rows > 0) must be non-null");
    if (!nngp::bf_pairb_planned_supported(m, 0, dim))
        return fail(NNGP_EUNSUP, "pair plans serve 2 <= m <= 17, dim 1..3 (m=%d, dim=%d)", m, dim);
    if (n_rows < 0 || n_rows > INT32_MAX || i0 < 0 || n_points < 1 || i0 + n_rows > n_points || n_points > INT32_MAX)
        return fail(NNGP_EINVAL, "rows [%lld, %lld) outside [0, %lld) (or n_rows / n_points >= 2^31)", (long long)i0,
                    (long long)(i0 + n_rows), (long long)n_points);
    if (((uintptr_t)plan & 255) != 0) return fail(NNGP_EINVAL, "plan must be 256-byte aligned");
    const size_t need = (size_t)nngp::plan_total_bytes(n_rows, m);
    if (plan_bytes < need) return fail(NNGP_EINVAL, "plan too small: %zu < %zu bytes", plan_bytes, need);
    hipStream_t s = (hipStream_t)stream;
    const nngp::PairbTiling tl = nngp::pairb_tiling(n_rows, m, 0);
    if (tl.tiles != nngp::plan_regions(n_rows)) return fail(NNGP_EUNSUP, "plan regions differ from the pair tiling");
    hipError_t e = nngp::pair_plan_build_launch(nbr, order, n_rows, m, dim, i0, n_points, tl.q, tl.rem, plan, s);
    if (e != hipSuccess) return hip_fail(e, "pair_plan build");
    nngp::PlanHeader h;
    e = hipMemcpyAsync(&h, plan, sizeof h, hipMemcpyDeviceToHost, s);
    if (e == hipSuccess) e = hipStreamSynchronize(s);
    if (e != hipSuccess) return hip_fail(e, "pair_plan counts");
    info[0] = h.n_planned;
    info[1] = h.n_direct;
    info[2] = n_rows;
    info[3] = m;
    info[4] = dim;
    info[5] = i0;
    info[6] = n_points;
    info[7] = nngp::kPlanMagic;
    info[8] = (int64_t)(uintptr_t)nbr;
    info[9] = (int64_t)(uintptr_t)order;
    return NNGP_OK;
}

int nngp_bf_sweep_plan(const double* coords, int64_t n_points, int32_t dim, const int32_t* nbr, const int32_t* order,
                       int64_t n_rows, int32_t m, int64_t i0, int32_t kind, double sigma2, double phi, double tau2,
                       const double* values, double* B, double* F, double* R, double* partials, void* workspace,
                       size_t workspace_bytes, const void* plan, size_t plan_bytes, const int64_t* info,
                       void* stream) {
    if (coords == nullptr || workspace == nullptr || plan == nullptr || info == nullptr)
        return fail(NNGP_EINVAL, "coordinates, workspace, plan and info must be non-null");
    if (info[7] != nngp::kPlanMagic || info[2] != n_rows || info[3] != m || info[4] != dim || info[5] != i0 ||
        info[6] != n_points)
        return fail(NNGP_EINVAL, "the plan was built for (n_rows %lld, m %lld, dim %lld, i0 %lld, n_points %lld), not "
                                 "this sweep's (%lld, %d, %d, %lld, %lld)", (long long)info[2], (long long)info[3],
                    (long long)info[4], (long long)info[5], (long long)info[6], (long long)n_rows, m, dim,
                    (long long)i0, (long long)n_points);
    if (info[8] != (int64_t)(uintptr_t)nbr || info[9] != (int64_t)(uintptr_t)order)
        return fail(NNGP_EINVAL, "stale plan: it was built for other nbr / order buffers (rebuild it with the "
                                 "sweep's neighbour sets)");
    if (!nngp::bf_pairb_planned_supported(m, kind, dim))
        return fail(NNGP_EUNSUP, "planned sweeps serve kinds 0..4, 2 <= m <= 17, dim 1..3 (kind=%d)", kind);
    if (plan_bytes < (size_t)nngp::plan_total_bytes(n_rows, m)) return fail(NNGP_EINVAL, "plan too small");
    const int64_t nreg = nngp::plan_regions(n_rows);
    if (info[0] < 0 || info[1] < 0 || info[0] + info[1] != nreg)
        return fail(NNGP_EINVAL, "plan counts %lld + %lld != %lld tiles", (long long)info[0], (long long)info[1],
                    (long long)nreg);
    if (m < 1 || (n_rows > 0 && nbr == nullptr)) return fail(NNGP_EINVAL, "nbr must be non-null");
    if (!(sigma2 > 0.0) || !(phi > 0.0) || !(tau2 >= 0.0) || !isfinite(sigma2) || !isfinite(phi) || !isfinite(tau2))
        return fail(NNGP_EINVAL, "theta must satisfy sigma2 > 0, phi > 0, tau2 >= 0 (finite)");
    if (B != nullptr && F == nullptr) return fail(NNGP_EINVAL, "B given without F");
// ... 486 lines not shown
```

### pynngp_amd/csrc/nngp_internal.h

```cpp
#pragma once
#include <hip/hip_runtime.h>
#include <stdint.h>

#include "nngp_math.h"
#include "pair_plan.h"

namespace nngp {

constexpr double kFar = 1e150;
static __device__ double2 kFarPoints[64] = {{1e150, 0.0}, {2e150, 0.0}, {3e150, 0.0}, {4e150, 0.0}, {5e150, 0.0}, {6e150, 0.0}, {7e150, 0.0}, {8e150, 0.0}, {9e150, 0.0}, {10e150, 0.0}, {11e150, 0.0}, {12e150, 0.0}, {13e150, 0.0}, {14e150, 0.0}, {15e150, 0.0}, {16e150, 0.0}, {17e150, 0.0}, {18e150, 0.0}, {19e150, 0.0}, {20e150, 0.0}, {21e150, 0.0}, {22e150, 0.0}, {23e150, 0.0}, {24e150, 0.0}, {25e150, 0.0}, {26e150, 0.0}, {27e150, 0.0}, {28e150, 0.0}, {29e150, 0.0}, {30e150, 0.0}, {31e150, 0.0}, {32e150, 0.0}, {33e150, 0.0}, {34e150, 0.0}, {35e150, 0.0}, {36e150, 0.0}, {37e150, 0.0}, {38e150, 0.0}, {39e150, 0.0}, {40e150, 0.0}, {41e150, 0.0}, {42e150, 0.0}, {43e150, 0.0}, {44e150, 0.0}, {45e150, 0.0}, {46e150, 0.0}, {47e150, 0.0}, {48e150, 0.0}, {49e150, 0.0}, {50e150, 0.0}, {51e150, 0.0}, {52e150, 0.0}, {53e150, 0.0}, {54e150, 0.0}, {55e150, 0.0}, {56e150, 0.0}, {57e150, 0.0}, {58e150, 0.0}, {59e150, 0.0}, {60e150, 0.0}, {61e150, 0.0}, {62e150, 0.0}, {63e150, 0.0}, {64e150, 0.0}};
static __device__ double kZeroValue[1] = {0.0};
static __device__ double kFarPoints1[64] = {1e150, 2e150, 3e150, 4e150, 5e150, 6e150, 7e150, 8e150, 9e150, 10e150, 11e150, 12e150, 13e150, 14e150, 15e150, 16e150, 17e150, 18e150, 19e150, 20e150, 21e150, 22e150, 23e150, 24e150, 25e150, 26e150, 27e150, 28e150, 29e150, 30e150, 31e150, 32e150, 33e150, 34e150, 35e150, 36e150, 37e150, 38e150, 39e150, 40e150, 41e150, 42e150, 43e150, 44e150, 45e150, 46e150, 47e150, 48e150, 49e150, 50e150, 51e150, 52e150, 53e150, 54e150, 55e150, 56e150, 57e150, 58e150, 59e150, 60e150, 61e150, 62e150, 63e150, 64e150};
static __device__ double kFarPoints3[64 * 3] = {1e150, 0.0, 0.0, 2e150, 0.0, 0.0, 3e150, 0.0, 0.0, 4e150, 0.0, 0.0, 5e150, 0.0, 0.0, 6e150, 0.0, 0.0, 7e150, 0.0, 0.0, 8e150, 0.0, 0.0, 9e150, 0.0, 0.0, 10e150, 0.0, 0.0, 11e150, 0.0, 0.0, 12e150, 0.0, 0.0, 13e150, 0.0, 0.0, 14e150, 0.0, 0.0, 15e150, 0.0, 0.0, 16e150, 0.0, 0.0, 17e150, 0.0, 0.0, 18e150, 0.0, 0.0, 19e150, 0.0, 0.0, 20e150, 0.0, 0.0, 21e150, 0.0, 0.0, 22e150, 0.0, 0.0, 23e150, 0.0, 0.0, 24e150, 0.0, 0.0, 25e150, 0.0, 0.0, 26e150, 0.0, 0.0, 27e150, 0.0, 0.0, 28e150, 0.0, 0.0, 29e150, 0.0, 0.0, 30e150, 0.0, 0.0, 31e150, 0.0, 0.0, 32e150, 0.0, 0.0, 33e150, 0.0, 0.0, 34e150, 0.0, 0.0, 35e150, 0.0, 0.0, 36e150, 0.0, 0.0, 37e150, 0.0, 0.0, 38e150, 0.0, 0.0, 39e150, 0.0, 0.0, 40e150, 0.0, 0.0, 41e150, 0.0, 0.0, 42e150, 0.0, 0.0, 43e150, 0.0, 0.0, 44e150, 0.0, 0.0, 45e150, 0.0, 0.0, 46e150, 0.0, 0.0, 47e150, 0.0, 0.0, 48e150, 0.0, 0.0, 49e150, 0.0, 0.0, 50e150, 0.0, 0.0, 51e150, 0.0, 0.0, 52e150, 0.0, 0.0, 53e150, 0.0, 0.0, 54e150, 0.0, 0.0, 55e150, 0.0, 0.0, 56e150, 0.0, 0.0, 57e150, 0.0, 0.0, 58e150, 0.0, 0.0, 59e150, 0.0, 0.0, 60e150, 0.0, 0.0, 61e150, 0.0, 0.0, 62e150, 0.0, 0.0, 63e150, 0.0, 0.0, 64e150, 0.0, 0.0};

template <int D>
__device__ __forceinline__ const double* far_point(int a) {
    if constexpr (D == 1) return kFarPoints1 + (a & 63);
    else if constexpr (D == 2) return (const double*)(kFarPoints + (a & 63));
    else return kFarPoints3 + 3 * (a & 63);
}
template <int D>
constexpr int point_arity() { return D == 0 ? 3 : D; }

template <int D>
__device__ __forceinline__ void load_point(const double* __restrict__ p, double (&x)[D]) {
    if constexpr (D == 2) {
        const double2 v = *(const double2*)p;
        x[0] = v.x;
        x[1] = v.y;
    } else {
#pragma unroll
        for (int k = 0; k < D; ++k) x[k] = p[k];
    }
}

__device__ __forceinline__ void load_point_rt(const double* __restrict__ p, int dim, double (&x)[3]) {
#pragma unroll
    for (int k = 0; k < 3; ++k) x[k] = *(k < dim ? p + k : kZeroValue);
}

template <int D>
__device__ __forceinline__ double point_d2(const double (&a)[D], const double (&b)[D]) {
    double acc = NNGP_D2_FLOOR;
#pragma unroll
    for (int k = D - 1; k >= 0; --k) {
        const double t = a[k] - b[k];
        acc = fma(t, t, acc);
    }
    return acc;
}

constexpr int kAlgoAuto = 0;
constexpr int kAlgoLane = 1;
constexpr int kAlgoWave = 2;
constexpr int kAlgoQuad = 4;
constexpr int kAlgoPairB = 5;
constexpr int kLaneMaxM = 16;

struct BfArgs {
    const double* coords;
    int64_t n_points;
    const int32_t* nbr;
    int64_t n_rows;
    int64_t i0;
    int m;
    int kind;
    int dim;
    double sigma2, phi, tau2;
    double nu;
    const int32_t* order;
    const double* values;
    const double* qcoords;
    const double* qvalues;
    double* B;
    double* F;
    double* R;
    double* partials;
    double* bpart;
    const double* cblk = nullptr;
    const int32_t* tiles = nullptr;
    int64_t n_tiles = 0, n_tile_list = 0, n_plan_blocks = 0;
};

int64_t bf_record_count(int64_t n_rows, int algo, int m);
hipError_t bf_finalize_launch(const double* bpart, int64_t n_records, double* partials, hipStream_t s);
hipError_t bf_finalize_pairb_launch(void* ws, int64_t n_rows, double* partials, hipStream_t s);
hipError_t bf_launch(const BfArgs& a, int algo, hipStream_t s);
hipError_t combine_partials_launch(const double* gathered, int world, int64_t n_slots, double* out, hipStream_t s);
bool bf_wave_launch(const BfArgs& a, const CovParams& P, int64_t n_blocks, hipStream_t s);
bool bf_group_launch(const BfArgs& a, const CovParams& P, int lanes, hipStream_t s);
bool bf_group_supported(int m, int lanes);
bool bf_pairb_launch(const BfArgs& a, const CovParams& P, hipStream_t s);
bool bf_pairb_supported(int m);
bool bf_pairb_blocks_launch(const BfArgs& a, hipStream_t s);
bool bf_pairb_planned_supported(int m, int kind, int dim);
bool bf_pairb_planned_launch(const BfArgs& a, const CovParams& P, const PlanLaunch& pl, hipStream_t s);
hipError_t bf_launch_planned(const BfArgs& a, const PlanLaunch& pl, hipStream_t s);
size_t pair_plan_build_lds(int m);
hipError_t pair_plan_build_launch(const int32_t* nbr, const int32_t* order, int64_t n_rows, int m, int dim, int64_t i0,
                                  int64_t n_points, int64_t tq, int64_t trem, void* plan, hipStream_t s);
bool bf_pairb_blocks_supported(int m);
bool bf_group_blocks_launch(const BfArgs& a, hipStream_t s);
bool bf_group_blocks_supported(int m);
hipError_t matern_table_launch(const CovParams& P, double* tab, hipStream_t s);
bool matern_table_extent(double nu, int* e0, int* noct);
bool matern_table_params(double nu, CovParams* p);
hipError_t matern_eval_launch(const double* u, int64_t n, double nu, double* out, hipStream_t s);
hipError_t joint_dist_launch(const double* coords, int64_t n_points, int dim, const double* qcoords,
                             const int32_t* nbr, const int32_t* order, int64_t n_rows, int m, int64_t i0, double* dist,
                             hipStream_t s);
int64_t bf_group_blocks(int64_t n_rows, int lanes);
int64_t bf_lane_blocks(int64_t n_rows);
int64_t bf_wave_blocks(int64_t n_rows);

constexpr int kKnnMaxLevels = 16;
struct KnnLevel {
    int64_t np;
    int g;
    int64_t n_cells;
    size_t off_idx_sorted, off_pts_sorted, off_cell_start;
};
struct KnnPlan {
    int64_t n_points;
    int dim;
    int g;
    int64_t n_cells;
    int n_levels;
    KnnLevel lv[kKnnMaxLevels];
    size_t sort_temp_bytes;
    size_t total_bytes;
    size_t off_bbox, off_key, off_key_sorted, off_sort_temp, off_idx, off_perm;
};

hipError_t knn_plan(int64_t n_points, int dim, KnnPlan* plan);
hipError_t knn_launch(bool prior, const double* coords, int64_t n_points, int m, const double* query, int64_t q0,
                      int64_t q1, const int32_t* rows, int32_t* nbr, void* workspace, const KnnPlan& plan,
                      hipStream_t s);

size_t reverse_workspace_bytes(int64_t n, int m);
hipError_t reverse_launch(const int32_t* nbr, int64_t n, int m, int32_t* off, int32_t* rev_j, int32_t* rev_k,
                          void* workspace, hipStream_t s);
int64_t color_moral_graph_host(const int32_t* nbr, const int32_t* off, const int32_t* rev_j, int64_t n, int m,
                               int32_t* color);
int64_t color_moral_graph_device(const int32_t* nbr, const int32_t* off, const int32_t* rev_j, int64_t n, int m,
                                 int32_t* color, void* workspace, hipStream_t s, hipError_t* err);
size_t gibbs_prep_bytes(int64_t n, int m);
hipError_t philox_normals_launch(int64_t n, uint64_t seed, uint64_t sweep, double* z, hipStream_t s);
hipError_t gibbs_prepare_launch(const double* B, const double* Ft, const int32_t* off, const int32_t* rev_j,
                                const int32_t* rev_k, const int32_t* order, int64_t n, int m, void* prep,
                                hipStream_t s);
hipError_t gibbs_prepare_range_launch(const double* B, const double* Ft, const int32_t* off, const int32_t* rev_j,
                                      const int32_t* rev_k, int64_t n, int m, int64_t row0, int64_t row1, void* prep,
                                      hipStream_t s);
hipError_t gibbs_w_color_launch(const int32_t* member_rows, int64_t n_members, const void* prep, int64_t n, int m,
                                double sigma2, double tau2, const double* yres, const double* noise_w, double* w,
                                double* r, const int32_t* rev_j, const double* z, uint64_t seed, uint64_t sweep,
                                double* w_out, const double* var, hipStream_t s);
hipError_t gibbs_w_apply_launch(const int32_t* rows, int64_t n_rows, const double* wsrc, const double* B, int m,
                                double* w, double* r, const int32_t* rev_j, const int32_t* rev_k, hipStream_t s);
hipError_t gibbs_member_rows_launch(const int32_t* members, int64_t n, const int32_t* off, int32_t* rows,
                                    hipStream_t s);
hipError_t gibbs_tile_sweep_launch(const int32_t* tiles, const int32_t* phase_off_host, const int32_t* phase_lds_host,
                                   int n_phases, const int32_t* tinfo, const int32_t* tstep, int ecap,
                                   const int32_t* tfp, const int32_t* off, const int32_t* rev_loc, const void* prep,
                                   int64_t n, int m, int64_t n_entries, double sigma2, double tau2,
                                   const double* yres, const double* noise_w, double* w, double* r, const double* z,
                                   hipStream_t s);
hipError_t gibbs_w_sweep_launch(const int32_t* member_rows, int n_colors, const int32_t* color_off_host,
                                const void* prep, int64_t n, int m, double sigma2, double tau2,
                                const double* yres, const double* noise_w, double* w, double* r,
                                const int32_t* rev_j, const double* z, uint64_t seed, uint64_t sweep, hipStream_t s);
hipError_t gibbs_w_sweep_chains_launch(const int32_t* member_rows, int n_colors, const int32_t* color_off_host,
                                       int chains, const void* const* preps, int64_t n, int m, const double* sigma2,
                                       const double* tau2, const double* const* yres, const double* noise_w,
                                       double* const* w, double* const* r, const int32_t* rev_j,
                                       const double* const* z, hipStream_t s, double* w_il = nullptr,
                                       double* r_il = nullptr);
size_t gibbs_stats_workspace_bytes(int64_t n, int p);
hipError_t gibbs_stats_launch(int64_t n, const double* r, const double* Ft, const double* yres, const double* y,
                              const double* X, int p, const double* w, const double* noise_w, double* out,
                              void* workspace, hipStream_t s);

size_t row_order_workspace_bytes(int64_t n_rows);
// ... 63 lines not shown
```

### pynngp_amd/csrc/nngp_math.h

```cpp
#pragma once

#include "exp2_table.h"
#include "rgamma_series.h"

#ifdef NNGP_MATH_HOST
#include <math.h>
#include <string.h>
#include <stdint.h>
#define NNGP_FN static inline
#define NNGP_HD static inline
static inline double nngp_rsq_approx(double x) {
    double y = 1.0 / sqrt(x);
    uint64_t u;
    memcpy(&u, &x, 8);
    return y * ((u >> 7) & 1 ? 1.0 + 0x1p-24 : 1.0 - 0x1p-24);
}
static inline int32_t nngp_lo_dword(double t) {
    uint64_t u;
    memcpy(&u, &t, 8);
    return (int32_t)(uint32_t)u;
}
static const double kExp2Tab[256] = NNGP_EXP2_TAB;
#else
#include <hip/hip_runtime.h>
// ... 344 lines not shown
    const double g = e * fma(0.375, e, 0.5);
    return fma(s, g, s);
}

NNGP_FN double nngp_rsqrt(double x) {
    const double y = nngp_rsq_approx(x);
    const double e = fma(-(x * y), y, 1.0);
    const double g = e * fma(0.375, e, 0.5);
    return fma(y, g, y);
}

template <int KIND>
NNGP_FN double nngp_cov_d2(const CovParams& P, const double* tab, double d2) {
    const double x = fmin(d2, P.d2max);
    if (KIND == NNGP_KIND_GAUSSIAN) return nngp_exp_tab(P, tab, x);
    const double d = nngp_sqrt(x);
    if (KIND == NNGP_KIND_MATERN) return P.sigma2 * nngp_matern_rho(P, P.phi * d);
    if (KIND == NNGP_KIND_GENERIC) {
        const double e = nngp_exp_tab(P, tab, P.gauss ? x : d);
        const double u = fmin(P.phi * d, P.umax);
        return fma(u, fma(u, fma(u, P.c[2], P.c[1]), P.c[0]), 1.0) * e;
    }
    if (KIND == NNGP_KIND_SPHERICAL) {
        const double u = fmin(P.phi * d, 1.0);
        const double p = fma(u, fma(0.5 * u, u, -1.5), 1.0);
        return P.sigma2 * p;
    }
    const double e = nngp_exp_tab(P, tab, d);
    if (KIND == NNGP_KIND_MATERN32) {
        const double pd = P.phi * d;
        return fma(pd, e, e);
    }
    if (KIND == NNGP_KIND_MATERN52) {
        const double u = P.phi * d;
        const double p = fma(fma(u, 1.0 / 3.0, 1.0), u, 1.0);
        return p * e;
    }
    return e;
}

NNGP_FN double nngp_d2(double ax, double ay, double bx, double by) {
    const double dx = ax - bx;
    const double dy = ay - by;
    return fma(dx, dx, fma(dy, dy, NNGP_D2_FLOOR));
}

#define NNGP_UNIT_CLAMP (1023.0 + 1.0 / 1024.0)
NNGP_HD CovParams nngp_cov_params_unit(int kind, double phi, double tau2_over_sigma2) {
    CovParams p = nngp_cov_params(kind, 1.0, phi, tau2_over_sigma2);
    if (kind == NNGP_KIND_GAUSSIAN) {
        p.d2max = NNGP_UNIT_CLAMP / (phi * phi * NNGP_LOG2E);
    } else if (kind != NNGP_KIND_SPHERICAL) {
        const double dmax = NNGP_UNIT_CLAMP / (phi * NNGP_LOG2E);
        p.d2max = dmax * dmax;
    }
    return p;
}

NNGP_FN double nngp_exp_unit(const CovParams& P, const double* tab, double u) {
    const double t = fma(P.nphi256, u, NNGP_EXP_MAGIC);
    const double k = t - NNGP_EXP_MAGIC;
    const double f = fma(P.nphi256, u, -k);
    const int32_t ki = nngp_lo_dword(t);
    const double Tadj = tab[ki & (NNGP_EXP_TAB_N - 1)];
    constexpr double Q[4] = NNGP_EXP2_Q;
    double q = fma(Q[3], f, Q[2]);
    q = fma(q, f, Q[1]);
    q = fma(q, f, Q[0]);
    const double fq = f * q;
#ifdef NNGP_MATH_HOST
    uint64_t bits;
    memcpy(&bits, &Tadj, 8);
    bits += (uint64_t)((uint32_t)ki << 12) << 32;
    double Ts;
    memcpy(&Ts, &bits, 8);
#else
    const long long tb = __double_as_longlong(Tadj);
    const int32_t hi = (int32_t)(tb >> 32) + (int32_t)((uint32_t)ki << 12);
    const double Ts = __hiloint2double(hi, (int32_t)(tb & 0xffffffffll));
#endif
    return fma(Ts, fq, Ts);
}

template <int KIND>
NNGP_FN double nngp_cov_unit(const CovParams& P, const double* tab, double d2) {
    if (KIND == NNGP_KIND_MATERN) return nngp_matern_tab(P, tab, d2);
    const double x = fmin(d2, P.d2max);
    if (KIND == NNGP_KIND_GAUSSIAN) return nngp_exp_unit(P, tab, x);
    const double d = nngp_sqrt(x);
    if (KIND == NNGP_KIND_SPHERICAL) {
        const double u = fmin(P.phi * d, 1.0);
        return fma(u, fma(0.5 * u, u, -1.5), 1.0);
    }
    if (KIND == NNGP_KIND_GENERIC) {
        const double e = nngp_exp_unit(P, tab, P.gauss ? x : d);
        const double u = fmin(P.phi * d, P.umax);
        return fma(u, fma(u, fma(u, P.c[2], P.c[1]), P.c[0]), 1.0) * e;
    }
    const double e = nngp_exp_unit(P, tab, d);
    if (KIND == NNGP_KIND_MATERN32) return fma(P.phi * d, e, e);
    if (KIND == NNGP_KIND_MATERN52) {
        const double u = P.phi * d;
        return fma(fma(u, 1.0 / 3.0, 1.0), u, 1.0) * e;
    }
    return e;
}

#ifndef NNGP_MATH_HOST
NNGP_FN double nngp_exp_table_entry_unit(int j) {
    const long long b = __double_as_longlong(kExp2Tab[j]);
    return __hiloint2double((int32_t)(b >> 32) - (j << 12), (int32_t)(b & 0xffffffffll));
}
NNGP_FN double nngp_exp_table_fetch_unit() { return nngp_exp_table_entry_unit((int)threadIdx.x & (NNGP_EXP_TAB_N - 1)); }
NNGP_FN void nngp_exp_table_store_unit(double* tab, double v) {
    if (threadIdx.x < NNGP_EXP_TAB_N) tab[threadIdx.x] = v;
    __syncthreads();
}

NNGP_FN void nngp_exp_table_load_unit(double* tab) {
    for (int j = threadIdx.x; j < NNGP_EXP_TAB_N; j += blockDim.x) {
        const long long b = __double_as_longlong(kExp2Tab[j]);
        tab[j] = __hiloint2double((int32_t)(b >> 32) - (j << 12), (int32_t)(b & 0xffffffffll));
    }
    __syncthreads();
}
#else
static inline void nngp_exp_table_load_unit(double* tab) {
    for (int j = 0; j < NNGP_EXP_TAB_N; ++j) {
        uint64_t b;
        memcpy(&b, &kExp2Tab[j], 8);
        b -= (uint64_t)((uint32_t)j << 12) << 32;
        memcpy(&tab[j], &b, 8);
    }
}
#endif
```

### pynngp_amd/csrc/torch_ops.cpp

```cpp
#include <ATen/ATen.h>
#include <ATen/hip/HIPContext.h>
#include <c10/core/DeviceGuard.h>
#include <torch/library.h>

#include "../../include/nngp.h"

namespace {

void* stream(const at::Tensor& t) { return (void*)at::hip::getCurrentHIPStream(t.device().index()).stream(); }

void check_rc(int rc, const char* what) { TORCH_CHECK(rc == NNGP_OK, what, " failed (", rc, "): ", nngp_last_error()); }

void check_coords(const at::Tensor& c, const char* name) {
    TORCH_CHECK(c.is_cuda(), name, " must be a ROCm GPU tensor (there is no CPU fallback)");
    TORCH_CHECK(c.scalar_type() == at::kDouble && c.dim() == 2 && c.size(1) >= 1 && c.size(1) <= NNGP_MAX_DIM,
                name, " must be float64 (N, dim), 1 <= dim <= ", NNGP_MAX_DIM);
    TORCH_CHECK(c.is_contiguous(), name, " must be contiguous");
}

void check_same_device(const at::Tensor& a, const at::Tensor& b, const char* name) {
    TORCH_CHECK(b.device() == a.device(), name, " is on ", b.device(), ", expected ", a.device());
}

void check_f64(const c10::optional<at::Tensor>& t, at::IntArrayRef shape, const at::Tensor& like, const char* name) {
    if (!t.has_value()) return;
    TORCH_CHECK(t->scalar_type() == at::kDouble && t->sizes() == shape && t->is_contiguous(), name,
                " must be a contiguous float64 tensor of shape ", shape);
    check_same_device(like, *t, name);
}

void check_nbr(const at::Tensor& nbr, const at::Tensor& like) {
    TORCH_CHECK(nbr.scalar_type() == at::kInt && nbr.dim() == 2 && nbr.is_contiguous(),
                "nbr must be a contiguous int32 (rows, m) tensor");
    check_same_device(like, nbr, "nbr");
}

template <typename T>
T* ptr(const c10::optional<at::Tensor>& t) {
    return t.has_value() ? (T*)t->data_ptr() : nullptr;
}

at::Tensor workspace(int64_t bytes, const at::Tensor& like) {
    auto ws = at::empty({bytes > 256 ? bytes : 256}, like.options().dtype(at::kByte));
    ws.narrow(0, 0, 256).zero_();
    return ws;
}

at::Tensor knn_prior(const at::Tensor& coords, int64_t m, int64_t q0, int64_t q1) {
    check_coords(coords, "coords");
    const at::OptionalDeviceGuard guard(coords.device());
    const int64_t n = coords.size(0), d = coords.size(1);
    TORCH_CHECK(0 <= q0 && q0 <= q1 && q1 <= n, "query rows [", q0, ", ", q1, ") outside [0, ", n, ")");
    auto out = at::empty({q1 - q0, m}, coords.options().dtype(at::kInt));
    auto ws = workspace((int64_t)nngp_knn_workspace_bytes(n, (int32_t)d, (int32_t)m), coords);
    check_rc(nngp_knn_prior(coords.data_ptr<double>(), n, (int32_t)d, (int32_t)m, q0, q1, out.data_ptr<int32_t>(),
                            ws.data_ptr(), ws.numel(), stream(coords)),
             "nngp_knn_prior");
    return out;
}

at::Tensor knn_prior_rows(const at::Tensor& coords, int64_t m, const at::Tensor& rows) {
    check_coords(coords, "coords");
    const at::OptionalDeviceGuard guard(coords.device());
    TORCH_CHECK(rows.scalar_type() == at::kInt && rows.dim() == 1 && rows.is_contiguous(), "rows must be int32 (n_rows,)");
    check_same_device(coords, rows, "rows");
    const int64_t n = coords.size(0), d = coords.size(1);
    auto out = at::empty({rows.size(0), m}, coords.options().dtype(at::kInt));
    auto ws = workspace((int64_t)nngp_knn_workspace_bytes(n, (int32_t)d, (int32_t)m), coords);
    check_rc(nngp_knn_prior_rows(coords.data_ptr<double>(), n, (int32_t)d, (int32_t)m, rows.data_ptr<int32_t>(),
                                 rows.size(0), out.data_ptr<int32_t>(), ws.data_ptr(), ws.numel(), stream(coords)),
             "nngp_knn_prior_rows");
    return out;
}

at::Tensor knn_query(const at::Tensor& ref, const at::Tensor& query, int64_t k) {
    check_coords(ref, "ref");
    const at::OptionalDeviceGuard guard(ref.device());
    check_coords(query, "query");
    check_same_device(ref, query, "query");
    TORCH_CHECK(ref.size(1) == query.size(1), "ref and query have different dimensions");
    const int64_t d = ref.size(1);
    auto out = at::empty({query.size(0), k}, ref.options().dtype(at::kInt));
    auto ws = workspace((int64_t)nngp_knn_workspace_bytes(ref.size(0), (int32_t)d, (int32_t)k), ref);
    check_rc(nngp_knn_query(ref.data_ptr<double>(), ref.size(0), (int32_t)d, query.data_ptr<double>(), query.size(0),
                            (int32_t)k, out.data_ptr<int32_t>(), ws.data_ptr(), ws.numel(), stream(ref)),
             "nngp_knn_query");
    return out;
}

void bf_sweep_out(const at::Tensor& coords, const at::Tensor& nbr, const c10::optional<at::Tensor>& order, int64_t i0,
                  int64_t kind, double sigma2, double phi, double tau2, const c10::optional<at::Tensor>& values,
                  const c10::optional<at::Tensor>& B, const c10::optional<at::Tensor>& F,
                  const c10::optional<at::Tensor>& R, const at::Tensor& partials, const at::Tensor& ws,
                  int64_t algo, double nu, const c10::optional<at::Tensor>& plan,
                  const c10::optional<at::Tensor>& plan_info) {
    check_coords(coords, "coords");
    const at::OptionalDeviceGuard guard(coords.device());
    check_nbr(nbr, coords);
    const int64_t rows = nbr.size(0), m = nbr.size(1), n = coords.size(0), d = coords.size(1);
    if (order.has_value()) {
        TORCH_CHECK(order->scalar_type() == at::kInt && order->sizes() == at::IntArrayRef{rows} && order->is_contiguous(),
                    "order must be a contiguous int32 (rows,) tensor");
        check_same_device(coords, *order, "order");
    }
    check_f64(values, {n}, coords, "values");
    check_f64(B, {rows, m}, coords, "B");
    check_f64(F, {rows}, coords, "F");
    check_f64(R, {rows}, coords, "R");
    check_f64(partials, {4}, coords, "partials");
    TORCH_CHECK(ws.is_contiguous(), "workspace must be contiguous");
    check_same_device(coords, ws, "workspace");
    if (plan.has_value()) {
        TORCH_CHECK(plan_info.has_value() && plan_info->device().is_cpu() && plan_info->scalar_type() == at::kLong &&
                        plan_info->numel() == NNGP_PLAN_INFO_LEN && plan_info->is_contiguous(),
                    "plan_info must be the pair_plan op's CPU int64 (", NNGP_PLAN_INFO_LEN, ",) tensor");
        TORCH_CHECK(plan->scalar_type() == at::kByte && plan->is_contiguous(), "plan must be a contiguous uint8 tensor");
        check_same_device(coords, *plan, "plan");
        TORCH_CHECK(algo == NNGP_ALGO_AUTO || algo == NNGP_ALGO_PAIRB, "a pair plan runs the pair kernel (algo ", algo, ")");
        check_rc(nngp_bf_sweep_plan(coords.data_ptr<double>(), n, (int32_t)d, nbr.data_ptr<int32_t>(), ptr<int32_t>(order),
                                    rows, (int32_t)m, i0, (int32_t)kind, sigma2, phi, tau2, ptr<double>(values),
                                    ptr<double>(B), ptr<double>(F), ptr<double>(R), partials.data_ptr<double>(),
                                    ws.data_ptr(), (size_t)ws.nbytes(), plan->data_ptr(), (size_t)plan->nbytes(),
                                    plan_info->data_ptr<int64_t>(), stream(coords)),
                 "nngp_bf_sweep_plan");
        return;
    }
    check_rc(nngp_bf_sweep(coords.data_ptr<double>(), n, (int32_t)d, nbr.data_ptr<int32_t>(), ptr<int32_t>(order), rows,
                           (int32_t)m, i0, (int32_t)kind, sigma2, phi, tau2, nu, ptr<double>(values), ptr<double>(B),
                           ptr<double>(F), ptr<double>(R), partials.data_ptr<double>(), ws.data_ptr(),
                           (size_t)ws.nbytes(), (int32_t)algo, stream(coords)),
             "nngp_bf_sweep");
}

std::tuple<at::Tensor, at::Tensor, at::Tensor> bf_sweep(const at::Tensor& coords, const at::Tensor& nbr, int64_t i0,
                                                        int64_t kind, double sigma2, double phi, double tau2,
                                                        const c10::optional<at::Tensor>& values, bool want_bf,
                                                        int64_t algo, const c10::optional<at::Tensor>& order,
                                                        double nu) {
    check_coords(coords, "coords");
    const at::OptionalDeviceGuard guard(coords.device());
    check_nbr(nbr, coords);
    const int64_t rows = nbr.size(0), m = nbr.size(1);
    auto f64 = coords.options();
    at::Tensor B = want_bf ? at::empty({rows, m}, f64) : at::empty({0, m}, f64);
    at::Tensor F = want_bf ? at::empty({rows}, f64) : at::empty({0}, f64);
    at::Tensor p = at::empty({4}, f64);
    auto ws = workspace((int64_t)nngp_bf_sweep_workspace_bytes(rows, (int32_t)m, (int32_t)kind,
                                                               (int32_t)coords.size(1), (int32_t)algo), coords);
    bf_sweep_out(coords, nbr, order, i0, kind, sigma2, phi, tau2, values,
                 want_bf ? c10::optional<at::Tensor>(B) : c10::nullopt,
                 want_bf ? c10::optional<at::Tensor>(F) : c10::nullopt, c10::nullopt, p, ws, algo, nu, c10::nullopt,
                 c10::nullopt);
    return {B, F, p};
}

std::tuple<at::Tensor, at::Tensor, at::Tensor> bf_cross(const at::Tensor& ref, const at::Tensor& query,
                                                        const at::Tensor& nbr, int64_t kind, double sigma2, double phi,
                                                        double tau2, const c10::optional<at::Tensor>& ref_values,
                                                        int64_t algo, double nu) {
    check_coords(ref, "ref");
    const at::OptionalDeviceGuard guard(ref.device());
    check_coords(query, "query");
    check_same_device(ref, query, "query");
    TORCH_CHECK(ref.size(1) == query.size(1), "ref and query have different dimensions");
    check_nbr(nbr, ref);
    const int64_t rows = nbr.size(0), m = nbr.size(1), d = ref.size(1);
    check_f64(ref_values, {ref.size(0)}, ref, "ref_values");
    auto f64 = ref.options();
    at::Tensor B = at::empty({rows, m}, f64), F = at::empty({rows}, f64), R = at::empty({rows}, f64);
    at::Tensor p = at::empty({4}, f64);
    auto ws = workspace((int64_t)nngp_bf_sweep_workspace_bytes(rows, (int32_t)m, (int32_t)kind, (int32_t)d,
                                                               (int32_t)algo), ref);
    check_rc(nngp_bf_cross(ref.data_ptr<double>(), ref.size(0), (int32_t)d, query.data_ptr<double>(), query.size(0),
                           nbr.data_ptr<int32_t>(), nullptr, rows, (int32_t)m, 0, (int32_t)kind, sigma2, phi, tau2,
                           nu, ptr<double>(ref_values), nullptr, B.data_ptr<double>(), F.data_ptr<double>(),
                           ref_values.has_value() ? R.data_ptr<double>() : nullptr, p.data_ptr<double>(),
                           ws.data_ptr(), ws.nbytes(), (int32_t)algo, stream(ref)),
             "nngp_bf_cross");
    at::Tensor mean = ref_values.has_value() ? R.neg() : at::zeros({rows}, f64);
    return {B, F, mean};
}

std::tuple<at::Tensor, at::Tensor> pair_plan(const at::Tensor& nbr, const c10::optional<at::Tensor>& order, int64_t i0,
                                             int64_t n_points, int64_t dim) {
    TORCH_CHECK(nbr.is_cuda(), "nbr must be a ROCm GPU tensor (there is no CPU fallback)");
    const at::OptionalDeviceGuard guard(nbr.device());
    check_nbr(nbr, nbr);
    const int64_t rows = nbr.size(0), m = nbr.size(1);
    if (order.has_value()) {
        TORCH_CHECK(order->scalar_type() == at::kInt && order->sizes() == at::IntArrayRef{rows} && order->is_contiguous(),
                    "order must be a contiguous int32 (rows,) tensor");
        check_same_device(nbr, *order, "order");
    }
    const size_t bytes = nngp_pair_plan_bytes(rows, (int32_t)m, (int32_t)dim);
    TORCH_CHECK(bytes > 0, "no pair plans for m=", m, ", dim=", dim, " (2 <= m <= 17, dim 1..3)");
    auto plan = workspace((int64_t)bytes, nbr);
    auto info = at::empty({NNGP_PLAN_INFO_LEN}, at::TensorOptions().dtype(at::kLong));
    check_rc(nngp_pair_plan_build(nbr.data_ptr<int32_t>(), ptr<int32_t>(order), rows, (int32_t)m, i0, n_points,
                                  (int32_t)dim, plan.data_ptr(), (size_t)plan.nbytes(), info.data_ptr<int64_t>(),
                                  stream(nbr)),
             "nngp_pair_plan_build");
    return {plan, info};
}

std::tuple<at::Tensor, at::Tensor> row_order(const at::Tensor& coords, int64_t i0, int64_t rows,
                                             const c10::optional<at::Tensor>& nbr) {
    check_coords(coords, "coords");
    const at::OptionalDeviceGuard guard(coords.device());
    const int64_t n = coords.size(0);
    TORCH_CHECK(0 <= i0 && 0 <= rows && i0 + rows <= n, "rows [", i0, ", ", i0 + rows, ") outside [0, ", n, ")");
    int64_t m = 0;
    if (nbr.has_value()) {
        check_nbr(*nbr, coords);
        TORCH_CHECK(nbr->size(0) == rows, "nbr must have one row per location");
        m = nbr->size(1);
    }
    auto order = at::empty({rows}, coords.options().dtype(at::kInt));
    at::Tensor srt = nbr.has_value() ? at::empty_like(*nbr) : at::empty({0, 0}, coords.options().dtype(at::kInt));
    auto ws = workspace((int64_t)nngp_row_order_workspace_bytes(rows), coords);
    check_rc(nngp_row_order(coords.data_ptr<double>(), n, (int32_t)coords.size(1), ptr<int32_t>(nbr), (int32_t)m, i0,
                            rows, order.data_ptr<int32_t>(), nbr.has_value() ? srt.data_ptr<int32_t>() : nullptr,
                            ws.data_ptr(), ws.nbytes(), stream(coords)),
             "nngp_row_order");
    return {order, srt};
}

void combine_partials_out(const at::Tensor& gathered, const at::Tensor& out) {
    TORCH_CHECK(gathered.is_cuda() && gathered.scalar_type() == at::kDouble &&
                    (gathered.dim() == 2 || gathered.dim() == 3) && gathered.size(-1) == 4 && gathered.is_contiguous(),
                "gathered must be a contiguous float64 (world, 4) or (world, n_slots, 4) GPU tensor");
    const at::OptionalDeviceGuard guard(gathered.device());
    const int64_t slots = gathered.dim() == 3 ? gathered.size(1) : 1;
    if (gathered.dim() == 3)
        check_f64(out, {slots, 4}, gathered, "out");
    else
        check_f64(out, {4}, gathered, "out");
    check_rc(nngp_combine_partials_batch(gathered.data_ptr<double>(), (int32_t)gathered.size(0), slots,
                                         out.data_ptr<double>(), stream(gathered)),
             "nngp_combine_partials_batch");
}

}

TORCH_LIBRARY(nngp, m) {
    m.def("knn_prior(Tensor coords, int m, int q0, int q1) -> Tensor");
    m.def("knn_prior_rows(Tensor coords, int m, Tensor rows) -> Tensor");
    m.def("knn_query(Tensor ref, Tensor query, int k) -> Tensor");
    m.def("bf_sweep(Tensor coords, Tensor nbr, int i0, int kind, float sigma2, float phi, float tau2, Tensor? values, "
          "bool want_bf, int algo, Tensor? order=None, float nu=-1.0) -> (Tensor, Tensor, Tensor)");
    m.def("bf_sweep_out(Tensor coords, Tensor nbr, Tensor? order, int i0, int kind, float sigma2, float phi, "
          "float tau2, Tensor? values, Tensor(a!)? B, Tensor(b!)? F, Tensor(c!)? R, Tensor(d!) partials, "
          "Tensor(e!) workspace, int algo, float nu=-1.0, Tensor? plan=None, Tensor? plan_info=None) -> ()");
    m.def("pair_plan(Tensor nbr, Tensor? order, int i0, int n_points, int dim) -> (Tensor, Tensor)");
    m.def("bf_cross(Tensor ref, Tensor query, Tensor nbr, int kind, float sigma2, float phi, float tau2, "
          "Tensor? ref_values, int algo, float nu=-1.0) -> (Tensor, Tensor, Tensor)");
    m.def("row_order(Tensor coords, int i0, int rows, Tensor? nbr) -> (Tensor, Tensor)");
    m.def("combine_partials_out(Tensor gathered, Tensor(a!) out) -> ()");
}

TORCH_LIBRARY_IMPL(nngp, CUDA, m) {
    m.impl("knn_prior", &knn_prior);
    m.impl("knn_prior_rows", &knn_prior_rows);
    m.impl("knn_query", &knn_query);
    m.impl("bf_sweep", &bf_sweep);
    m.impl("bf_sweep_out", &bf_sweep_out);
    m.impl("bf_cross", &bf_cross);
    m.impl("row_order", &row_order);
    m.impl("pair_plan", &pair_plan);
    m.impl("combine_partials_out", &combine_partials_out);
}
```

### pynngp_amd/gibbs.py

```python
from __future__ import annotations

import dataclasses
import math
from typing import Optional

import numpy as np
import torch

from . import _lib, ops
from .nngp import NNGPNumericalError, _default_device


def _as_points(a, what):
    h = np.ascontiguousarray(a, dtype=np.float64)
    if h.ndim == 1:
        h = h[:, None]
    if h.ndim != 2 or not 1 <= h.shape[1] <= _lib.MAX_DIM or h.shape[0] < 1:
        raise ValueError(f"{what} must be (N >= 1, d) with 1 <= d <= {_lib.MAX_DIM}, got {h.shape}")
    if not np.all(np.isfinite(h)):
        raise ValueError(f"{what} must be finite (NaN / inf would silently decouple locations)")
    return h


def colour_dag(nbr, off, rev_j, n_s):
# ... 149 lines not shown
                x_ref = np.asarray(X_ref, dtype=np.float64).reshape(n_s, -1)
                if x_ref.shape[1] != self.p or not np.all(np.isfinite(x_ref)):
                    raise ValueError(f"X_ref must be finite ({n_s}, {self.p})")
                X_n[:n_s][free] = x_ref[free]
            un_nodes = np.concatenate([un_nodes, self.unobserved_ref])
            un_sd = np.concatenate([un_sd, np.ones(self.unobserved_ref.size)])
            x_un = np.concatenate([x_un, x_ref[self.unobserved_ref]])
        XtX = (X_n * h_n[:, None]).T @ X_n
        if np.linalg.matrix_rank(XtX) < self.p:
            raise ValueError("X' H X is singular over the observed locations")
        self._XtX_inv = np.linalg.inv(XtX)
        self._XtX_inv_chol = np.linalg.cholesky(self._XtX_inv)
        homoscedastic = eps is None and self.n_obs == n

        off0, rev_j0, _ = _lib.reverse_neighbors(nbr0)
        colors0, self.n_colors, self.n_colors_ref = colour_dag(nbr0, off0, rev_j0, n_s)
        del off0, rev_j0
        perm, _ = _lib.row_order(coords0)
        self._relabel(perm.long(), coords0, y_n, X_n, None if homoscedastic else h_n, nbr0, colors0)
        self._tiles = None
        if sweep == "tiled":
            from .gibbs_tiles import build_tile_plan

            tp0 = build_tile_plan(self.coords, self.off, self.rev_j, self._colors_d, self.n_colors, self.n_colors_ref,
                                  tile_nodes=self._tile_nodes, max_levels=self._tile_max_levels,
                                  coarse=self._tile_coarse)
            t0 = tp0.tnodes.long()
            self._relabel(self.perm[t0], coords0, y_n, X_n, None if homoscedastic else h_n, nbr0, colors0)
            self._tiles = build_tile_plan(self.coords, self.off, self.rev_j, self._colors_d, self.n_colors,
                                          self.n_colors_ref, assign=(tp0.node_tile[t0], tp0.tile_level, tp0.coarse_tile))
            assert self._tiles.contiguous
            del tp0, t0
        del self._colors_d
        pos_h = self.pos.cpu().numpy()
        self._un_nodes = torch.from_numpy(pos_h[un_nodes].astype(np.int64)).to(dev)
        self._un_sd = to(un_sd)
        self._un_X = to(x_un.reshape(-1, self.p))
        self.y_unobserved = torch.zeros(len(un_nodes), dtype=torch.float64, device=dev)
        self._zy = torch.empty(len(un_nodes), dtype=torch.float64, device=dev)

        self.beta = self._XtX_inv @ ((X_n * h_n[:, None]).T @ y_n)
        self.sigma2 = float(sigma2)
        self.tau2 = float(tau2)
        lo, hi = self.priors.phi_unif
        self.phi = float(phi) if phi is not None else math.sqrt(lo * hi)
        self.phi_tuning = float(phi_tuning)
        self.yres = self._residual_y(self.beta)
        if w_init is None:
            obs_idx = np.nonzero(observed)[0]
            t_obs = t_dev[torch.from_numpy(obs_idx).to(dev)]
            k = min(5, self.n_obs)
            idx = _lib.knn_query(t_obs, coords0, k).long()
            r_obs = y_host[observed] - X_t[observed] @ self.beta
            w0 = to(r_obs)[idx].mean(dim=1).cpu().numpy()
        else:
            w0 = np.asarray(w_init, dtype=np.float64).reshape(-1)
            if w0.shape != (n,):
                raise ValueError(f"w_init must hold one value per node ({n}: reference points, then the data "
                                 "locations outside the reference set)")
        self.w = to(w0)[self.perm].contiguous()
        self.iteration = 0
        self.n_accept = 0
        self.n_notpd_reject = 0

        z = lambda *s: torch.empty(s, dtype=torch.float64, device=dev)
        self.B, self.Ft, self.r = z(n, self.m), z(n), z(n)
        self._B2, self._Ft2, self._r2 = z(n, self.m), z(n), z(n)
        self._part = z(4)
        self._z = z(n)
        ops.load()
        if self._custom is not None:
            if not 1 <= self.m <= _lib.BLOCKS_MAX_M:
                raise ValueError(f"a callable covariance needs 1 <= m <= {_lib.BLOCKS_MAX_M} (m={self.m})")
            self._cblocks = self._custom.blocks(self.coords, self.nbr, 0)
            self._ws = _lib._workspace(_lib.load().nngp_bf_sweep_blocks_workspace_bytes(n), dev)
            self._kind_code, self._algo_code = -1, ops.algo_code(algo)
        else:
            self._ws = _lib.bf_workspace(n, self.m, algo, dev, kind=kind, dim=self.coords.shape[1])
            self._kind_code, self._algo_code = ops.kind_code(kind), ops.algo_code(algo)
        self._plan = (None, None)
        if (self._use_plan and self._custom is None and algo in ("auto", "pairb")
                and _lib.pair_plan_supported(self.m, kind, self.coords.shape[1])):
            self._plan = ops.pair_plan(self.nbr, None, 0, n, self.coords.shape[1])
        self._stats_buf = z(2 + self.p)
        self._sweep_into(self.phi, self.B, self.Ft, self.r)
        self._prep = _lib.gibbs_prepare(self.B, self.Ft, self.off, self.rev_j, self.rev_k)
        ph = self._part.cpu().numpy()
        self._check(ph)
        self.sum_logF, self.quad = float(ph[0]), float(ph[1])

    def _relabel(self, perm, coords0, y_n, X_n, h_n, nbr0, colors0):
        dev = self.device
        to = lambda a: torch.as_tensor(np.ascontiguousarray(a, dtype=np.float64)).to(dev)
        n = coords0.shape[0]
        self.perm = perm
        self.pos = torch.empty_like(self.perm)
        self.pos[self.perm] = torch.arange(n, device=dev)
        self.coords = coords0[self.perm].contiguous()
        self.y = to(y_n)[self.perm].contiguous()
        self.X = to(X_n)[self.perm].contiguous()
        self._Xcols = self.X.t().contiguous()
        self.noise_w = None if h_n is None else to(h_n)[self.perm].contiguous()
        nb = nbr0[self.perm].long()
        self.nbr = torch.where(nb >= 0, self.pos[nb.clamp(min=0)], -1).to(torch.int32).contiguous()
        self.off, self.rev_j, self.rev_k = _lib.reverse_neighbors(self.nbr)
        colors_d = colors0[self.perm]
        self._colors_d = colors_d
        self.colors = colors_d.cpu().numpy()
        self.members = torch.sort(colors_d, stable=True)[1].to(torch.int32)
        self.color_off = np.concatenate([[0], np.cumsum(torch.bincount(colors_d, minlength=self.n_colors).cpu().numpy())
                                         ]).astype(np.int32)

    def _residual_y(self, beta):
        out = getattr(self, "_yres_buf", None)
        if out is None:
            out = self._yres_buf = torch.empty_like(self.y)
        if self.p == 0:
            return out.copy_(self.y)
        torch.sub(self.y, self._Xcols[0], alpha=float(beta[0]), out=out)
        for c in range(1, self.p):
            out.sub_(self._Xcols[c], alpha=float(beta[c]))
        return out

    def _sweep_into(self, phi, B, Ft, r):
        if self._custom is not None:
            _lib.bf_sweep_blocks(self._cblocks, self.nbr, self.n, 0, values=self.w, qvalues=self.w, R=r, B=B, F=Ft,
                                 partials=self._part, workspace=self._ws)
            return
        torch.ops.nngp.bf_sweep_out(self.coords, self.nbr, None, 0, self._kind_code, 1.0, float(phi), 0.0, self.w, B,
                                    Ft, r, self._part, self._ws, self._algo_code, self._nu_arg, *self._plan)

    @staticmethod
    def _check(p):
        if p[2] >= 0:
            raise NNGPNumericalError(
                f"latent NNGP factor not positive definite at location {int(p[2])} at the initial phi "
                "(duplicate or near-duplicate coordinates make C_N singular; remove duplicates or lower phi)")

    def _ig(self, a, b):
        return 1.0 / self.rng.gamma(a, 1.0 / b)

    def loglik_w(self, sum_logF, quad, sigma2):
        return -0.5 * (self.n * math.log(2 * math.pi * sigma2) + sum_logF + quad / sigma2)

    def update_phi(self):
        prop = self._phi_draw()
        if prop is not None:
            self._phi_decide(prop, self._propose(prop[0]))

    def _phi_draw(self):
        if self.fix_phi:
            return None
        phi_p = self.phi * math.exp(self.phi_tuning * self.rng.standard_normal())
        lo, hi = self.priors.phi_unif
        u = self.rng.random()
        if not lo <= phi_p <= hi:
            return None
        return phi_p, u

    def _phi_decide(self, prop, ph):
        phi_p, u = prop
        if ph[2] >= 0:
            self.n_notpd_reject += 1
            return
        l_new = self.loglik_w(ph[0], ph[1], self.sigma2)
        l_old = self.loglik_w(self.sum_logF, self.quad, self.sigma2)
        if math.log(u) < l_new - l_old + math.log(phi_p) - math.log(self.phi):
            self.phi = phi_p
            self.B, self._B2 = self._B2, self.B
            self.Ft, self._Ft2 = self._Ft2, self.Ft
            self.r, self._r2 = self._r2, self.r
            self._prepare()
            self.sum_logF, self.quad = float(ph[0]), float(ph[1])
            self.n_accept += 1

    def _propose(self, phi):
        self._sweep_into(phi, self._B2, self._Ft2, self._r2)
        return self._part.cpu().numpy()

    def _prepare(self):
        self._prep = _lib.gibbs_prepare(self.B, self.Ft, self.off, self.rev_j, self.rev_k, prep=self._prep)

    def _stats(self):
        return self._stats_dev().cpu().numpy()

    def _stats_dev(self):
        return _lib.gibbs_stats(self.r, self.Ft, self.yres, self.y, self.X, self.w, out=self._stats_buf,
                                noise_w=self.noise_w)

    def _member_rows_t(self):
        if getattr(self, "_member_rows", None) is None and self.members.numel() > 0:
            self._member_rows = _lib.gibbs_member_rows(self.members, self.off)
        return getattr(self, "_member_rows", None)

    def _assemble(self, t):
        return t

    def _assemble_unobserved(self, t):
        return t

    def _sweep_colours(self, c0, c1):
        if c1 > c0:
            self._member_rows_t()
            _lib.gibbs_w_sweep(self.members, self.color_off[c0:c1 + 1], self._prep, self.m, self.sigma2, self.tau2,
                               self.yres, self.w, self.r, self.off, self.rev_j, self.seed, self.iteration, z=self._z,
                               noise_w=self.noise_w, member_rows=self._member_rows)

    def update_wt(self):
        self._sweep_colours(self.n_colors_ref, self.n_colors)

    def update_ws(self):
        self._sweep_colours(0, self.n_colors_ref)

# ... 266 lines not shown
```

### pynngp_amd/ops.py

```python
from __future__ import annotations

import os

import torch

from . import _lib

_KINDS = tuple(_lib.KIND_CODES)
_ALGOS = dict(_lib.ALGO_CODES)
LIB_PATH = os.path.join(os.path.dirname(os.path.abspath(__file__)), "_build", "libnngp_torch_ops.so")

_loaded = False


def load() -> None:
    global _loaded
    if _loaded:
        return
    if not os.path.exists(LIB_PATH):
        raise _lib.NNGPExtensionError(
            f"{LIB_PATH} not found: build it with `python -c 'import __graft_entry__ as g; g.build()'` "
            "(pynngp_amd has no CPU fallback)")
    _lib.load()
    torch.ops.load_library(LIB_PATH)
    _register_fakes()
    _loaded = True


def _register_fakes() -> None:
    def fake(name):
        return torch.library.register_fake(f"nngp::{name}")

    @fake("knn_prior")
    def _(coords, m, q0, q1):
        return coords.new_empty((q1 - q0, m), dtype=torch.int32)

    @fake("knn_prior_rows")
    def _(coords, m, rows):
        return coords.new_empty((rows.shape[0], m), dtype=torch.int32)

    @fake("knn_query")
    def _(ref, query, k):
        return query.new_empty((query.shape[0], k), dtype=torch.int32)

    @fake("bf_sweep")
    def _(coords, nbr, i0, kind, sigma2, phi, tau2, values, want_bf, algo, order=None, nu=-1.0):
        rows, m = nbr.shape
        if want_bf:
            return coords.new_empty((rows, m)), coords.new_empty((rows,)), coords.new_empty((4,))
        return coords.new_empty((0, m)), coords.new_empty((0,)), coords.new_empty((4,))

    @fake("bf_sweep_out")
    def _(coords, nbr, order, i0, kind, sigma2, phi, tau2, values, B, F, R, partials, workspace, algo, nu=-1.0,
          plan=None, plan_info=None):
        return None

    @fake("pair_plan")
    def _(nbr, order, i0, n_points, dim):
        raise RuntimeError("pair_plan is a setup call (it synchronises to read its tile counts): build it eagerly")

    @fake("bf_cross")
    def _(ref, query, nbr, kind, sigma2, phi, tau2, ref_values, algo, nu=-1.0):
        rows, m = nbr.shape
        return query.new_empty((rows, m)), query.new_empty((rows,)), query.new_empty((rows,))

    @fake("row_order")
    def _(coords, i0, rows, nbr):
        srt = torch.empty_like(nbr) if nbr is not None else coords.new_empty((0, 0), dtype=torch.int32)
        return coords.new_empty((rows,), dtype=torch.int32), srt

    @fake("combine_partials_out")
    def _(gathered, out):
        return None


def kind_code(kind: str) -> int:
    try:
        return _KINDS.index(kind)
    except ValueError:
        raise ValueError(f"unknown covariance kind {kind!r}; expected one of {_KINDS}") from None


def algo_code(algo: str) -> int:
    try:
        return _ALGOS[algo]
    except KeyError:
        raise ValueError(f"unknown algo {algo!r}; expected one of {tuple(_ALGOS)}") from None


def bf_sweep_out(coords, nbr, order, i0, kind: str, theta, values, B, F, R, partials, workspace,
                 algo: str = "auto", plan=None) -> None:
    load()
    nu = float(theta[3]) if len(theta) > 3 else -1.0
    pbuf, pinfo = plan if plan is not None else (None, None)
    torch.ops.nngp.bf_sweep_out(coords, nbr, order, int(i0), kind_code(kind), float(theta[0]), float(theta[1]),
                                float(theta[2]), values, B, F, R, partials, workspace, algo_code(algo), nu, pbuf,
                                pinfo)


def pair_plan(nbr, order, i0: int, n_points: int, dim: int):
    load()
    return torch.ops.nngp.pair_plan(nbr, order, int(i0), int(n_points), int(dim))


def pair_plan_supported(m: int, kind: str, dim: int) -> bool:
    return _lib.pair_plan_supported(m, kind, dim)
```

### pynngp_amd/sweep.py

```python
from __future__ import annotations

import math
import time
from typing import Callable, Optional

import torch
import torch.distributed as dist

from . import _lib, ops
from .nngp import Covariance, LOG_2PI, _raise_on_bad


PLAN_DEFAULT = False


def shard_range(n: int, rank: int, world: int):
    return (n * rank) // world, (n * (rank + 1)) // world


def _collective_default(collective: Optional[bool]) -> bool:
    if collective is not None:
        return bool(collective)
    return dist.is_available() and dist.is_initialized()


def combine_partials(local: torch.Tensor, world: int, group=None, force: bool = False) -> torch.Tensor:
    if world == 1 and not force:
        return local
    gathered = torch.empty((world, 4), dtype=local.dtype, device=local.device)
    dist.all_gather_into_tensor(gathered, local.reshape(1, 4), group=group)
    if gathered.device.type == "cuda":
        ops.load()
        out = torch.empty(4, dtype=local.dtype, device=local.device)
        torch.ops.nngp.combine_partials_out(gathered, out)
        return out
    return combine_partials_host(gathered)


class ShardedLogLik:

    def __init__(self, coords: torch.Tensor, m: int, rank: int = 0, world: int = 1, group=None,
                 algo: str = "auto", build_nbr: Optional[Callable] = None, compute: Optional[Callable] = None,
                 spatial_order: bool = True, layout: str = "natural", build_perm: Optional[Callable] = None,
                 api: str = "ops", collective: Optional[bool] = None, plan: Optional[bool] = None):
        if layout not in ("natural", "storage"):
            raise ValueError(f"layout must be 'natural' or 'storage', got {layout!r}")
        if api not in ("ops", "ctypes"):
            raise ValueError(f"api must be 'ops' (torch.ops.nngp) or 'ctypes' (the same C ABI via ctypes), got {api!r}")
        self.api = api
        self.layout = layout
        if not bool(torch.isfinite(coords).all()):
            raise ValueError("coordinates must be finite (NaN / inf would silently decouple locations)")
        self.coords = coords
        self.n = coords.shape[0]
        self.m = int(m)
        self.rank, self.world, self.group = rank, world, group
        self.collective = _collective_default(collective)
        self.lo, self.hi = shard_range(self.n, rank, world)
        self.algo = algo
        self._compute = compute
        self._ws = None
        self._partials = None
        self.order = None
        self.perm = self.pos = None
        if layout == "storage":
            perm = _lib.row_order(coords)[0] if build_perm is None else build_perm(coords)
            self.perm = perm
            self.pos = torch.empty(self.n, dtype=torch.int32, device=coords.device)
            self.pos[perm.long()] = torch.arange(self.n, dtype=torch.int32, device=coords.device)
            self._coords_sweep = coords[perm.long()].contiguous()
            rows = perm[self.lo:self.hi].contiguous()
            nbr0 = _lib.knn_prior_rows(coords, self.m, rows) if build_nbr is None else build_nbr(coords, self.m, rows)
            nb = nbr0.long()
            self.nbr = torch.where(nb >= 0, self.pos[nb.clamp(min=0)], -1).to(torch.int32).contiguous()
            self._nbr_sweep = self.nbr
            self._vstore = torch.empty(self.n, dtype=torch.float64, device=coords.device)
        else:
            self._coords_sweep = coords
            if build_nbr is None:
                self.nbr = _lib.knn_prior(coords, self.m, self.lo, self.hi)
            else:
                self.nbr = build_nbr(coords, self.m, self.lo, self.hi)
            self._nbr_sweep = self.nbr
            if compute is None and spatial_order and self.hi > self.lo:
                self.order, self._nbr_sweep = _lib.row_order(coords, self.lo, self.hi - self.lo, self.nbr)
        if compute is None:
            ops.load()
            self._sweep_op = torch.ops.nngp.bf_sweep_out.default
            self._algo_code = ops.algo_code(algo)
            self._ws = _lib.bf_workspace(self.hi - self.lo, self.m, algo, coords.device, dim=coords.shape[1])
            self._partials = torch.empty(4, dtype=torch.float64, device=coords.device)
            self._B = torch.empty((self.hi - self.lo, self.m), dtype=torch.float64, device=coords.device)
            self._F = torch.empty((self.hi - self.lo,), dtype=torch.float64, device=coords.device)
        self._plan = self._plan_ctypes = None
        self.plan_build_s = 0.0
        self.plan_read_bytes = 0
        want = plan if plan is not None else PLAN_DEFAULT
        d = coords.shape[1]
        if (compute is None and want and self.hi > self.lo and algo in ("auto", "pairb")
                and _lib.pair_plan_supported(self.m, "exponential", d)):
            t0 = time.perf_counter()
            self._plan = ops.pair_plan(self._nbr_sweep, self.order, self.lo, self.n, d)
            self.plan_build_s = time.perf_counter() - t0
            self._plan_ctypes = _lib.PairPlan(self._plan[0], self._plan[1].tolist(), self._nbr_sweep, self.order)
            self.plan_read_bytes = _lib.pair_plan_read_bytes(self._plan[0], self.m)
        elif plan:
            raise ValueError(f"pair plans serve algo auto / pairb, 2 <= m <= 17, dim 1..3 (m={self.m}, dim={d})")

    @property
    def planned(self) -> bool:
        return self._plan is not None

    def _plan_for(self, kind: str):
        return self._plan if (self._plan is not None and _lib.KIND_CODES.get(kind, 99) <= 4) else None

    def to_storage(self, values: torch.Tensor, out: Optional[torch.Tensor] = None) -> torch.Tensor:
        return torch.index_select(values, 0, self.perm, out=out)

    def local_partials(self, cov: Covariance, values: Optional[torch.Tensor], want_bf: bool = True,
                       values_layout: str = "input", out: Optional[torch.Tensor] = None) -> torch.Tensor:
        if self.layout == "storage" and values is not None and values_layout == "input":
            values = self.to_storage(values, out=self._vstore)
        if self._compute is not None:
            p = self._compute(self, cov, values, want_bf)
            return p if out is None else out.copy_(p)
        B, F = (self._B, self._F) if want_bf else (None, None)
        p = self._partials if out is None else out
        s2, phi, tau2 = cov.theta
        plan = self._plan_for(cov.kind)
        if self.api == "ctypes":
            _lib.bf_sweep(self._coords_sweep, self._nbr_sweep, self.lo, cov.kind, s2, phi, tau2, values=values,
                          want_bf=want_bf, algo=self.algo, B=B, F=F, partials=p, workspace=self._ws, order=self.order,
                          nu=cov.nu_arg, plan=self._plan_ctypes if plan is not None else None)
            return p
        pb, pi = plan if plan is not None else (None, None)
        self._sweep_op(self._coords_sweep, self._nbr_sweep, self.order, self.lo, ops.kind_code(cov.kind),
                       float(s2), float(phi), float(tau2), values, B, F, None, p, self._ws, self._algo_code,
                       -1.0 if cov.nu_arg is None else cov.nu_arg, pb, pi)
        return p

    def partials(self, cov: Covariance, values: Optional[torch.Tensor], want_bf: bool = True,
                 values_layout: str = "input") -> torch.Tensor:
        return combine_partials(self.local_partials(cov, values, want_bf, values_layout), self.world, self.group,
                                force=self.collective)

    def loglik(self, cov: Covariance, values: torch.Tensor, want_bf: bool = False,
               values_layout: str = "input") -> float:
        p = self.partials(cov, values, want_bf, values_layout).cpu().numpy()
        _raise_on_bad(p)
        return -0.5 * (self.n * LOG_2PI + p[0] + p[1])

    def loglik_scan(self, covs, values: torch.Tensor, values_layout: str = "input") -> list:
        covs = list(covs)
        if self.layout == "storage" and values is not None and values_layout == "input":
            values = self.to_storage(values, out=self._vstore)
            values_layout = "storage"
        pipe = PipelinedCombine(self, len(covs))
        for k, cov in enumerate(covs):
            self.local_partials(cov, values, False, values_layout, out=pipe.local[k])
            pipe.exchange(k)
        res = pipe.finish().cpu().numpy()
        out = []
        for p in res:
            _raise_on_bad(p)
            out.append(-0.5 * (self.n * LOG_2PI + p[0] + p[1]))
        return out

    @property
    def rows_input(self) -> torch.Tensor:
        if self.layout == "storage":
            return self.perm[self.lo:self.hi].long()
        return torch.arange(self.lo, self.hi, device=self.coords.device)

    @property
    def B(self):
        return self._B

    @property
    def F(self):
        return self._F


class PipelinedCombine:

    def __init__(self, sweep: "ShardedLogLik", slots: int, batch: int = 16):
        dev = sweep.coords.device
        self.sweep = sweep
        self.world = sweep.world
        self.active = self.world > 1 or getattr(sweep, "collective", False)
        if dev.type == "cuda":
            ops.load()
        self.batch = max(1, int(batch))
        self.local = torch.empty((slots, 4), dtype=torch.float64, device=dev)
        self.gathered = torch.empty((slots * self.world * 4,), dtype=torch.float64, device=dev)
        self.results = torch.empty((slots, 4), dtype=torch.float64, device=dev)
        self.side = torch.cuda.Stream(device=dev) if dev.type == "cuda" else None
        self.k = 0
        self.flushed = 0
        self.n_collectives = 0

    def exchange(self, k: int) -> None:
        self.k = max(self.k, k + 1)
        if self.active and self.k - self.flushed >= self.batch:
            self._flush()

    def _flush(self) -> None:
        b0, b1 = self.flushed, self.k
        if b1 <= b0:
            return
        nb = b1 - b0
        out = self.gathered[b0 * self.world * 4: b1 * self.world * 4]
        work = dist.all_gather_into_tensor(out, self.local[b0:b1].reshape(-1), group=self.sweep.group,
                                           async_op=True)
        self.flushed = b1
        self.n_collectives += 1
        g = out.view(self.world, nb, 4)
        if self.side is None:
            work.wait()
            for j in range(nb):
                self.results[b0 + j].copy_(combine_partials_host(g[:, j, :]))
            return
# ... 29 lines not shown
```

Measured before the change: 5.827 billion.

## Add neighbor certificate to skip index and clamp checks on trusted tiles

Adds a setup-time neighbor certificate that marks, per tile, whether every neighbor index is in range and valid. The pairb sweep kernel reads this bitmask and, for certified tiles, runs a specialised body that drops index bounds checks, far-point substitution and covariance clamping. This is meant to cut per-pair branching and ALU work in the hot sweep. It costs a one-time build pass plus a duplicated kernel body, which raises code size and possibly register pressure.

```diff
diff --git a/include/nngp.h b/include/nngp.h
--- a/include/nngp.h
+++ b/include/nngp.h
@@ -68,6 +68,18 @@
                        const double *values, double *B, double *F, double *R, double *partials, void *workspace,
                        size_t workspace_bytes, const void *plan, size_t plan_bytes, const int64_t *info,
                        void *stream);
+
+#define NNGP_CERT_INFO_LEN 16
+size_t nngp_nbr_cert_bytes(int64_t n_rows);
+int nngp_nbr_cert_build(const double *coords, int64_t n_points, int32_t dim, const int32_t *nbr, const int32_t *order,
+                        int64_t n_rows, int32_t m, int64_t i0, void *cert, size_t cert_bytes, int64_t *info,
+                        void *stream);
+int64_t nngp_nbr_cert_trusted_tiles(const int64_t *info, int32_t kind, double sigma2, double phi, double tau2);
+int nngp_bf_sweep_cert(const double *coords, int64_t n_points, int32_t dim, const int32_t *nbr, const int32_t *order,
+                       int64_t n_rows, int32_t m, int64_t i0, int32_t kind, double sigma2, double phi, double tau2,
+                       double nu, const double *values, double *B, double *F, double *R, double *partials,
+                       void *workspace, size_t workspace_bytes, int32_t algo, const void *cert, size_t cert_bytes,
+                       const int64_t *info, void *stream);
 
 int nngp_bf_cross(const double *ref, int64_t n_ref, int32_t dim, const double *query, int64_t n_query,
                   const int32_t *nbr, const int32_t *order, int64_t n_rows, int32_t m, int64_t q0, int32_t kind,
diff --git a/pynngp_amd/_lib.py b/pynngp_amd/_lib.py
--- a/pynngp_amd/_lib.py
+++ b/pynngp_amd/_lib.py
@@ -55,6 +55,10 @@
     "nngp_pair_plan_bytes",
     "nngp_pair_plan_build",
     "nngp_bf_sweep_plan",
+    "nngp_nbr_cert_bytes",
+    "nngp_nbr_cert_build",
+    "nngp_nbr_cert_trusted_tiles",
+    "nngp_bf_sweep_cert",
 )
 
 KIND_CODES = {"exponential": 0, "matern32": 1, "matern52": 2, "gaussian": 3, "spherical": 4, "matern": 5}
@@ -64,6 +68,7 @@
 MAX_DIM = 3
 ABI_VERSION = 4
 PLAN_INFO_LEN = 10
+CERT_INFO_LEN = 16
 BLOCKS_MAX_M = 32
 
 
@@ -177,6 +182,15 @@
     lib.nngp_bf_sweep_plan.argtypes = [P, I64, I32, P, P, I64, I32, I64, I32, D, D, D, P, P, P, P, P, P, SZ, P, SZ, P,
                                        P]
     lib.nngp_bf_sweep_plan.restype = ctypes.c_int
+    lib.nngp_nbr_cert_bytes.argtypes = [I64]
+    lib.nngp_nbr_cert_bytes.restype = SZ
+    lib.nngp_nbr_cert_build.argtypes = [P, I64, I32, P, P, I64, I32, I64, P, SZ, P, P]
+    lib.nngp_nbr_cert_build.restype = ctypes.c_int
+    lib.nngp_nbr_cert_trusted_tiles.argtypes = [P, I32, D, D, D]
+    lib.nngp_nbr_cert_trusted_tiles.restype = I64
+    lib.nngp_bf_sweep_cert.argtypes = [P, I64, I32, P, P, I64, I32, I64, I32, D, D, D, D, P, P, P, P, P, P, SZ, I32, P,
+                                       SZ, P, P]
+    lib.nngp_bf_sweep_cert.restype = ctypes.c_int
     lib.nngp_check_partials.argtypes = [P, P, P]
     lib.nngp_check_partials.restype = ctypes.c_int
     lib.nngp_loglik_from_partials.argtypes = [P, I64]
@@ -379,8 +393,8 @@
              partials: Optional[torch.Tensor] = None, workspace: Optional[torch.Tensor] = None,
              order: Optional[torch.Tensor] = None,
              R: Optional[torch.Tensor] = None,
-             defer: bool = False, nu: Optional[float] = None, plan: Optional[PairPlan] = None
-             ) -> Tuple[Optional[torch.Tensor], Optional[torch.Tensor], torch.Tensor]:
+             defer: bool = False, nu: Optional[float] = None, plan: Optional[PairPlan] = None,
+             cert=None) -> Tuple[Optional[torch.Tensor], Optional[torch.Tensor], torch.Tensor]:
     coords = _as_coords(coords)
     if nbr.dtype != torch.int32 or nbr.dim() != 2:
         raise ValueError(f"nbr must be int32 (rows, m), got {nbr.dtype} {tuple(nbr.shape)}")
@@ -431,11 +445,37 @@
                                       _ptr(plan.buf), plan.buf.numel(), plan.info, _stream(dev)),
                "nngp_bf_sweep_plan")
         return B, F, partials
+    if cert is not None:
+        cbuf, cinfo = cert
+        if cbuf.device != dev:
+            raise ValueError("cert must be on the sweep's device")
+        _check(lib.nngp_bf_sweep_cert(_ptr(coords), coords.shape[0], d, _ptr(nbr), _ptr(order), rows, m, i0,
+                                      KIND_CODES[kind], float(sigma2), float(phi), float(tau2), nu, _ptr(values),
+                                      _ptr(B), _ptr(F), _ptr(R), _ptr(partials), _ptr(workspace), workspace.numel(), a,
+                                      _ptr(cbuf), cbuf.numel(), cinfo, _stream(dev)),
+               "nngp_bf_sweep_cert")
+        return B, F, partials
     _check(lib.nngp_bf_sweep(_ptr(coords), coords.shape[0], d, _ptr(nbr), _ptr(order), rows, m, i0, KIND_CODES[kind],
                              float(sigma2), float(phi), float(tau2), nu, _ptr(values), _ptr(B), _ptr(F), _ptr(R),
                              _ptr(partials), _ptr(workspace), workspace.numel(), a, _stream(dev)),
            "nngp_bf_sweep")
     return B, F, partials
+
+
+def nbr_cert(coords: torch.Tensor, nbr: torch.Tensor, i0: int = 0, order: Optional[torch.Tensor] = None):
+    if not (coords.is_contiguous() and nbr.is_contiguous() and coords.dtype == torch.float64 and coords.dim() == 2
+            and nbr.dtype == torch.int32 and nbr.dim() == 2):
+        raise ValueError("nbr_cert needs contiguous float64 (N, dim) coords and int32 (rows, m) nbr")
+    dev = _require_gpu(coords, nbr, order)
+    rows, m = nbr.shape
+    if order is not None and (order.dtype != torch.int32 or order.shape != (rows,) or not order.is_contiguous()):
+        raise ValueError("order must be a contiguous int32 (rows,) tensor")
+    lib = load()
+    buf = _workspace(lib.nngp_nbr_cert_bytes(rows), dev)
+    info = (ctypes.c_int64 * CERT_INFO_LEN)()
+    _check(lib.nngp_nbr_cert_build(_ptr(coords), coords.shape[0], coords.shape[1], _ptr(nbr), _ptr(order), rows, m,
+                                   int(i0), _ptr(buf), buf.numel(), info, _stream(dev)), "nngp_nbr_cert_build")
+    return buf, info
 
 
 def bf_finalize(workspace: torch.Tensor, rows: int, m: int, kind: str, dim: int, algo: str = "auto",
diff --git a/pynngp_amd/csrc/bf_pairb.h b/pynngp_amd/csrc/bf_pairb.h
--- a/pynngp_amd/csrc/bf_pairb.h
+++ b/pynngp_amd/csrc/bf_pairb.h
@@ -3,6 +3,8 @@
 #include <stdint.h>
 #include <stdlib.h>
 #include <string.h>
+
+#include <type_traits>
 
 #include "bf_group.h"
 #include "nngp_internal.h"
@@ -22,6 +24,10 @@
 constexpr bool pairb_lk(int m, int kind) {
     return pairb_left(m) && (kind != NNGP_KIND_MATERN || m == kPairbLeftMaternM) &&
            (kind != NNGP_KIND_BLOCKS || m <= 24);
+}
+constexpr int kPairbCertMaxM = 24;
+constexpr bool pairb_cert_trustable(int m, int kind, int d, bool planned) {
+    return !planned && kind >= 0 && kind <= 4 && d >= 1 && d <= 3 && m >= 1 && m <= kPairbCertMaxM;
 }
 #ifndef NNGP_PHASE
 #define NNGP_PHASE(name)
@@ -213,9 +219,11 @@
                                                 double* __restrict__ Fout, double* __restrict__ Rout,
                                                 double4* __restrict__ rec, int32_t* __restrict__ lexp, int dim,
                                                 const double* __restrict__ cblk, int64_t tq, int64_t trem,
-                                                int64_t* __restrict__ hdr, const PairPlanArgs pp) {
+                                                int64_t* __restrict__ hdr, const PairPlanArgs pp,
+                                                const uint32_t* __restrict__ ckmask) {
     static_assert(M >= 1 && M <= 32, "pairb instantiated for 1 <= m <= 32");
     static_assert(D >= 0 && D <= 3, "0 (runtime dimension) <= D <= 3");
+    constexpr bool TRUSTABLE = pairb_cert_trustable(M, KIND, D, PL);
     constexpr bool CM = KIND == NNGP_KIND_BLOCKS;
     constexpr bool MT = KIND == NNGP_KIND_MATERN;
     constexpr int DA = point_arity<D>();
@@ -260,11 +268,16 @@
     const double wq1 = q1 ? 1.0 : 0.0, wq0 = 1.0 - wq1;
     uint32_t mask1 = q1 ? 0xffffffffu : 0u;
     asm volatile("" : "+v"(mask1));
-    {
+    auto body = [&](auto trust_tag) __attribute__((always_inline)) {
+        constexpr bool TRUST = decltype(trust_tag)::value;
+        auto cov = [&](double d2, int s, int t) __attribute__((always_inline)) -> double {
+            const bool clamp = !TRUST || (M % 2 == 0 && (s == NP - 1 || t == NP - 1));
+            return clamp ? nngp_cov_unit<KIND, true>(Pc, ctab, d2) : nngp_cov_unit<KIND, false>(Pc, ctab, d2);
+        };
         const int64_t lr = threadIdx.x >> 1;
         const int64_t r = tile * tq + (tile < trem ? tile : trem) + lr;
         const bool live = lr < tq + (tile < trem ? 1 : 0);
-        const int64_t rl = live ? r : n_rows - 1;
+        const int64_t rl = live ? r : (TRUST ? r - lr : n_rows - 1);
         const int32_t ov = (order != nullptr ? order : nbr)[rl];
         const int64_t rr = order != nullptr ? (int64_t)ov : rl;
         const int64_t i = i0 + rr;
@@ -284,7 +297,7 @@
             const int32_t j = a < M ? jn[s] : -1;
             jmax = max(jmax, j);
             jmin = min(jmin, j);
-            const bool in_range = (uint32_t)j < n32;
+            const bool in_range = TRUST ? (s < NP - 1 || M % 2 == 1) : (uint32_t)j < n32;
             const bool self = a == M;
             const double* pc = self ? qcoords + i * ds : (in_range ? coords + (int64_t)j * ds : far_point<DA>(a));
             const double* pv = self ? (qvalues != nullptr ? qvalues + i : kZeroValue)
@@ -297,7 +310,7 @@
             }
             if constexpr (!LEFT) z[s] = *pv;
         }
-        const bool bad_index = (int64_t)jmax >= n_points || jmin < -1;
+        const bool bad_index = !TRUST && ((int64_t)jmax >= n_points || jmin < -1);
         if constexpr (LEFT) {
 #pragma unroll
             for (int s = 0; s < NP; ++s) lidx[s][threadIdx.x] = jn[s];
@@ -509,8 +522,8 @@
             for (int s = 0; s < NP; ++s) {
 #pragma unroll
                 for (int t = 0; t < s; ++t) {
-                    R[s][t][0] = nngp_cov_unit<KIND>(Pc, ctab, point_d2<DA>(o[s], o[t]));
-                    R[s][t][1] = nngp_cov_unit<KIND>(Pc, ctab, point_d2<DA>(o[s], p[t]));
+                    R[s][t][0] = cov(point_d2<DA>(o[s], o[t]), s, t);
+                    R[s][t][1] = cov(point_d2<DA>(o[s], p[t]), s, t);
                 }
                 R[s][s][0] = Pc.diag;
             }
@@ -524,12 +537,12 @@
                         a[k] = pr_pick(mask1, o[s1][k], o[s0][k]);
                         b[k] = pr_pick(mask1, p[s1][k], p[s0][k]);
                     }
-                    const double c = nngp_cov_unit<KIND>(Pc, ctab, point_d2<DA>(a, b));
+                    const double c = cov(point_d2<DA>(a, b), s0, s1);
                     R[s1][s1][1] = c;
                     R[s0][s0][1] = pr_from0(c);
                 } else {
-                    R[s0][s0][1] = nngp_cov_unit<KIND>(Pc, ctab, point_d2<DA>(o[s0], p[s0]));
-                    if (s1 < NP) R[s1][s1][1] = nngp_cov_unit<KIND>(Pc, ctab, point_d2<DA>(o[s1], p[s1]));
+                    R[s0][s0][1] = cov(point_d2<DA>(o[s0], p[s0]), s0, s0);
+                    if (s1 < NP) R[s1][s1][1] = cov(point_d2<DA>(o[s1], p[s1]), s1, s1);
                 }
             }
         }
@@ -653,8 +666,8 @@
                 for (int k = 0; k < DA; ++k) pu[k] = (u % 2 == 1) ? pnext[k] : pr_swap(o[u][k]);
 #pragma unroll
                 for (int s = u + 1; s < NP; ++s) {
-                    R[s][u][0] = nngp_cov_unit<KIND>(Pc, ctab, point_d2<DA>(o[s], o[u]));
-                    R[s][u][1] = nngp_cov_unit<KIND>(Pc, ctab, point_d2<DA>(o[s], pu));
+                    R[s][u][0] = cov(point_d2<DA>(o[s], o[u]), s, u);
+                    R[s][u][1] = cov(point_d2<DA>(o[s], pu), s, u);
                 }
                 R[u][u][0] = Pc.diag;
                 if (u % 2 == 0 && u + 1 < NP) {
@@ -665,12 +678,12 @@
                         a[k] = pr_pick(mask1, o[u + 1][k], o[u][k]);
                         b[k] = pr_pick(mask1, pnext[k], pu[k]);
                     }
-                    wpnext = nngp_cov_unit<KIND>(Pc, ctab, point_d2<DA>(a, b));
+                    wpnext = cov(point_d2<DA>(a, b), u, u + 1);
                     R[u][u][1] = pr_from0(wpnext);
                 } else if (u % 2 == 1) {
                     R[u][u][1] = wpnext;
                 } else {
-                    R[u][u][1] = nngp_cov_unit<KIND>(Pc, ctab, point_d2<DA>(o[u], pu));
+                    R[u][u][1] = cov(point_d2<DA>(o[u], pu), u, u);
                 }
                 }
 #pragma unroll
@@ -739,7 +752,7 @@
             __builtin_amdgcn_fence(__ATOMIC_ACQUIRE, "workgroup");
             rrl = (int64_t)(((uint64_t)(uint32_t)lidx[NP + 1][threadIdx.x] << 32) | (uint32_t)lidx[NP][threadIdx.x]);
             il = i0 + rrl;
-            bidx = lidx[NP + 2][threadIdx.x] != 0;
+            bidx = !TRUST && lidx[NP + 2][threadIdx.x] != 0;
         }
 
         {
@@ -751,7 +764,7 @@
                 for (int s = 0; s < NP; ++s) {
                     const int a = 2 * s + q;
                     const int32_t j = a < M ? lidx[s][threadIdx.x] : -1;
-                    const bool in_range = (uint32_t)j < n32;
+                    const bool in_range = TRUST ? (s < NP - 1 || M % 2 == 1) : (uint32_t)j < n32;
                     const double* pv = a == M ? (qvalues != nullptr ? qvalues + il : kZeroValue)
                                               : ((values != nullptr && in_range) ? values + j : kZeroValue);
                     z[s] = *pv;
@@ -826,7 +839,17 @@
                          (live && bidx) ? (double)il : INFINITY, sh, 0, rec, lexp, tile);
         __syncthreads();
         if (threadIdx.x == 0) pairb_tile_fold(sh, 0, rec, lexp, tile);
-    }
+    };
+    if constexpr (TRUSTABLE) {
+        const bool trusted =
+            ckmask != nullptr &&
+            ((uint32_t)__builtin_amdgcn_readfirstlane((int)ckmask[tile >> 5]) >> (uint32_t)(tile & 31) & 1u) == 0u;
+        if (trusted) {
+            body(std::true_type{});
+            return;
+        }
+    }
+    body(std::false_type{});
 }
 
 inline size_t pairb_align(size_t b) { return (b + 255) & ~(size_t)255; }
@@ -855,7 +878,7 @@
     hipLaunchKernelGGL((bf_pairb<M, KIND, D, PL>), dim3((unsigned)nb), dim3(kPairbThreads), lds, s, a.coords,
                        a.n_points, a.nbr, a.order, a.n_rows, a.i0, Pc, KIND == NNGP_KIND_BLOCKS ? 1.0 : a.sigma2, a.values,
                        a.qcoords, a.qvalues, a.B, a.F, a.R, pairb_rec(a.bpart), pairb_lexp(a.bpart, a.n_rows), a.dim,
-                       a.cblk, tl.q, tl.rem, pairb_hdr(a.bpart), pp);
+                       a.cblk, tl.q, tl.rem, pairb_hdr(a.bpart), pp, a.checked);
 }
 
 template <int M, int KIND, int D>
diff --git a/pynngp_amd/csrc/capi.hip b/pynngp_amd/csrc/capi.hip
--- a/pynngp_amd/csrc/capi.hip
+++ b/pynngp_amd/csrc/capi.hip
@@ -7,6 +7,7 @@
 #include "../../include/nngp.h"
 #include "nngp_internal.h"
 #include "bf_pairb.h"
+#include "nbr_cert.h"
 
 namespace {
 thread_local char g_err[512] = "";
@@ -95,7 +96,7 @@
                      const int32_t* nbr, const int32_t* order, int64_t n_rows, int32_t m, int64_t i0, int32_t kind,
                      double sigma2, double phi, double tau2, double nu, const double* values, const double* qvalues, double* B,
                      double* F, double* R, double* partials, void* workspace, size_t workspace_bytes, int32_t algo,
-                     void* stream) {
+                     void* stream, const uint32_t* checked = nullptr) {
     if (coords == nullptr || qcoords == nullptr || workspace == nullptr)
         return fail(NNGP_EINVAL, "coordinates and workspace must be non-null");
     if (dim < 1 || dim > NNGP_MAX_DIM) return fail(NNGP_EUNSUP, "dim=%d outside [1, %d]", dim, NNGP_MAX_DIM);
@@ -145,6 +146,7 @@
     hipStream_t s = (hipStream_t)stream;
     nngp::BfArgs args{coords, n_points, nbr, n_rows, i0, m, kind, dim, sigma2, phi, tau2, nu, order, values, qcoords,
                       qvalues, B, F, R, partials, (double*)workspace};
+    if (a == nngp::kAlgoPairB) args.checked = checked;
     hipError_t e = nngp::bf_launch(args, a, s);
     if (e != hipSuccess) return hip_fail(e, "bf_sweep launch");
     return NNGP_OK;
@@ -156,6 +158,80 @@
                   size_t workspace_bytes, int32_t algo, void* stream) {
     return bf_common(coords, n_points, dim, coords, n_points, nbr, order, n_rows, m, i0, kind, sigma2, phi, tau2, nu,
                      values, values, B, F, R, partials, workspace, workspace_bytes, algo, stream);
+}
+
+size_t nngp_nbr_cert_bytes(int64_t n_rows) { return n_rows < 0 ? 0 : nngp::cert_total_bytes(n_rows); }
+
+int nngp_nbr_cert_build(const double* coords, int64_t n_points, int32_t dim, const int32_t* nbr, const int32_t* order,
+                        int64_t n_rows, int32_t m, int64_t i0, void* cert, size_t cert_bytes, int64_t* info,
+                        void* stream) {
+    if (coords == nullptr || cert == nullptr || info == nullptr || (n_rows > 0 && nbr == nullptr))
+        return fail(NNGP_EINVAL, "coords, cert, info (and nbr for n_rows > 0) must be non-null");
+    if (dim < 1 || dim > NNGP_MAX_DIM) return fail(NNGP_EUNSUP, "dim=%d outside [1, %d]", dim, NNGP_MAX_DIM);
+    if (m < 1 || m > NNGP_MAX_M) return fail(NNGP_EUNSUP, "m=%d outside [1, %d]", m, NNGP_MAX_M);
+    if (n_points < 1 || n_rows < 0 || i0 < 0 || i0 + n_rows > n_points)
+        return fail(NNGP_EINVAL, "rows [%lld, %lld) outside [0, %lld)", (long long)i0, (long long)(i0 + n_rows),
+                    (long long)n_points);
+    if (((uintptr_t)cert & 255) != 0) return fail(NNGP_EINVAL, "cert must be 256-byte aligned");
+    const size_t need = nngp::cert_total_bytes(n_rows);
+    if (cert_bytes < need) return fail(NNGP_EINVAL, "cert too small: %zu < %zu bytes", cert_bytes, need);
+    hipStream_t s = (hipStream_t)stream;
+    hipError_t e = nngp::nbr_cert_launch(coords, n_points, dim, nbr, n_rows, m, cert, s);
+    if (e != hipSuccess) return hip_fail(e, "nbr_cert build");
+    const int64_t tiles = nngp::cert_tiles(n_rows);
+    int32_t n_checked = 0;
+    double rec[nngp::kCertSpanBlocks * 8];
+    e = hipMemcpyAsync(&n_checked, cert, sizeof n_checked, hipMemcpyDeviceToHost, s);
+    if (e == hipSuccess)
+        e = hipMemcpyAsync(rec, (const char*)cert + nngp::cert_span_off(tiles), sizeof rec, hipMemcpyDeviceToHost, s);
+    if (e == hipSuccess) e = hipStreamSynchronize(s);
+    if (e != hipSuccess) return hip_fail(e, "nbr_cert counts");
+    double span = 0.0;
+    if (!nngp::cert_span_fold(rec, nngp::kCertSpanBlocks, dim, &span))
+        return fail(NNGP_EINVAL, "coordinates must be finite (and their bounding box's squared diagonal too)");
+    for (int k = 0; k < NNGP_CERT_INFO_LEN; ++k) info[k] = 0;
+    info[nngp::kCertIMagic] = nngp::kCertMagic;
+    info[nngp::kCertICoords] = (int64_t)(uintptr_t)coords;
+    info[nngp::kCertINbr] = (int64_t)(uintptr_t)nbr;
+    info[nngp::kCertIOrder] = (int64_t)(uintptr_t)order;
+    info[nngp::kCertINPoints] = n_points;
+    info[nngp::kCertIDim] = dim;
+    info[nngp::kCertINRows] = n_rows;
+    info[nngp::kCertIM] = m;
+    info[nngp::kCertII0] = i0;
+    info[nngp::kCertITiles] = tiles;
+    info[nngp::kCertIChecked] = n_checked;
+    memcpy(&info[nngp::kCertISpan], &span, sizeof span);
+    return NNGP_OK;
+}
+
+int64_t nngp_nbr_cert_trusted_tiles(const int64_t* info, int32_t kind, double sigma2, double phi, double tau2) {
+    return nngp::cert_trusted_tiles(info, kind, sigma2, phi, tau2);
+}
+
+int nngp_bf_sweep_cert(const double* coords, int64_t n_points, int32_t dim, const int32_t* nbr, const int32_t* order,
+                       int64_t n_rows, int32_t m, int64_t i0, int32_t kind, double sigma2, double phi, double tau2,
+                       double nu, const double* values, double* B, double* F, double* R, double* partials,
+                       void* workspace, size_t workspace_bytes, int32_t algo, const void* cert, size_t cert_bytes,
+                       const int64_t* info, void* stream) {
+    if (cert == nullptr || info == nullptr) return fail(NNGP_EINVAL, "cert and info must be non-null");
+    if (info[nngp::kCertIMagic] != nngp::kCertMagic) return fail(NNGP_EINVAL, "info is not a certificate's");
+    if (info[nngp::kCertICoords] != (int64_t)(uintptr_t)coords || info[nngp::kCertINbr] != (int64_t)(uintptr_t)nbr ||
+        info[nngp::kCertIOrder] != (int64_t)(uintptr_t)order)
+        return fail(NNGP_EINVAL, "the certificate was built for other coords / nbr / order buffers (rebuild it for "
+                                 "this sweep's)");
+    if (info[nngp::kCertINPoints] != n_points || info[nngp::kCertIDim] != dim || info[nngp::kCertINRows] != n_rows ||
+        info[nngp::kCertIM] != m || info[nngp::kCertII0] != i0)
+        return fail(NNGP_EINVAL, "the certificate was built for (n_points %lld, dim %lld, n_rows %lld, m %lld, i0 %lld), "
+                                 "not this sweep's (%lld, %d, %lld, %d, %lld)", (long long)info[nngp::kCertINPoints],
+                    (long long)info[nngp::kCertIDim], (long long)info[nngp::kCertINRows], (long long)info[nngp::kCertIM],
+                    (long long)info[nngp::kCertII0], (long long)n_points, dim, (long long)n_rows, m, (long long)i0);
+    if (n_rows < 0 || cert_bytes < nngp::cert_total_bytes(n_rows) || info[nngp::kCertITiles] != nngp::cert_tiles(n_rows))
+        return fail(NNGP_EINVAL, "cert too small for %lld rows", (long long)n_rows);
+    const bool use = nngp_nbr_cert_trusted_tiles(info, kind, sigma2, phi, tau2) > 0;
+    const uint32_t* checked = use ? (const uint32_t*)((const char*)cert + nngp::kCertMaskOff) : nullptr;
+    return bf_common(coords, n_points, dim, coords, n_points, nbr, order, n_rows, m, i0, kind, sigma2, phi, tau2, nu,
+                     values, values, B, F, R, partials, workspace, workspace_bytes, algo, stream, checked);
 }
 
 int nngp_bf_cross(const double* ref, int64_t n_ref, int32_t dim, const double* query, int64_t n_query,
diff --git a/pynngp_amd/csrc/nbr_cert.h b/pynngp_amd/csrc/nbr_cert.h
--- /dev/null
+++ b/pynngp_amd/csrc/nbr_cert.h
@@ -0,0 +1,93 @@
+#pragma once
+#include <math.h>
+#include <stdint.h>
+#include <string.h>
+
+#include "nngp_math.h"
+
+namespace nngp {
+
+constexpr int kCertInfoLen = 16;
+constexpr int64_t kCertMagic = 0x4e42524345525431ll;
+enum {
+    kCertIMagic = 0, kCertICoords, kCertINbr, kCertIOrder, kCertINPoints, kCertIDim, kCertINRows, kCertIM, kCertII0,
+    kCertITiles, kCertIChecked, kCertISpan
+};
+constexpr int kCertMaxM = 24;
+constexpr int kCertTileRows = 128;
+constexpr int kCertSpanBlocks = 256;
+
+inline int64_t cert_tiles(int64_t n_rows) { return n_rows > 0 ? (n_rows + kCertTileRows - 1) / kCertTileRows : 0; }
+inline size_t cert_align(size_t b) { return (b + 255) & ~(size_t)255; }
+constexpr size_t kCertMaskOff = 256;
+inline size_t cert_mask_bytes(int64_t tiles) { return cert_align((size_t)((tiles + 31) / 32) * 4); }
+inline size_t cert_span_off(int64_t tiles) { return kCertMaskOff + cert_mask_bytes(tiles); }
+inline size_t cert_total_bytes(int64_t n_rows) {
+    return cert_span_off(cert_tiles(n_rows)) + (size_t)kCertSpanBlocks * 8 * sizeof(double);
+}
+
+NNGP_HD bool cert_slot_checked(int32_t j, int64_t n_points) { return j < 0 || (int64_t)j >= n_points; }
+
+inline int64_t cert_tile_row0(int64_t t, int64_t q, int64_t rem) { return t * q + (t < rem ? t : rem); }
+
+inline int64_t cert_mask_host(const int32_t* nbr, int64_t n_rows, int m, int64_t n_points, uint32_t* mask) {
+    const int64_t T = cert_tiles(n_rows);
+    for (int64_t w = 0; w < (T + 31) / 32; ++w) mask[w] = 0;
+    if (T == 0) return 0;
+    const int64_t q = n_rows / T, rem = n_rows % T;
+    int64_t checked = 0;
+    for (int64_t t = 0; t < T; ++t) {
+        const int64_t r0 = cert_tile_row0(t, q, rem), rows = q + (t < rem ? 1 : 0);
+        bool any = false;
+        for (int64_t r = r0; r < r0 + rows && !any; ++r)
+            for (int s = 0; s < m && !any; ++s) any = cert_slot_checked(nbr[r * m + s], n_points);
+        if (any) {
+            mask[t >> 5] |= 1u << (t & 31);
+            ++checked;
+        }
+    }
+    return checked;
+}
+
+inline bool cert_span_fold(const double* rec, int n_blocks, int dim, double* d2_span) {
+    double mn[3] = {INFINITY, INFINITY, INFINITY}, mx[3] = {-INFINITY, -INFINITY, -INFINITY};
+    bool finite = true;
+    for (int b = 0; b < n_blocks; ++b) {
+        for (int c = 0; c < dim; ++c) {
+            mn[c] = fmin(mn[c], rec[8 * b + c]);
+            mx[c] = fmax(mx[c], rec[8 * b + 3 + c]);
+        }
+        finite = finite && rec[8 * b + 6] == 0.0;
+    }
+    double s = 0.0;
+    for (int c = 0; c < dim; ++c) {
+        const double e = mx[c] - mn[c];
+        s += e * e;
+    }
+    *d2_span = s;
+    return finite && isfinite(s);
+}
+
+inline double cert_info_span(const int64_t* info) {
+    double s;
+    memcpy(&s, &info[kCertISpan], sizeof s);
+    return s;
+}
+
+inline int64_t cert_trusted_tiles(const int64_t* info, int kind, double sigma2, double phi, double tau2) {
+    if (info == nullptr || info[kCertIMagic] != kCertMagic) return 0;
+    if (kind < 0 || kind > 4) return 0;
+    if (info[kCertIM] < 1 || info[kCertIM] > kCertMaxM || info[kCertIDim] < 1 || info[kCertIDim] > 3) return 0;
+    if (!(sigma2 > 0.0) || !(phi > 0.0) || !(tau2 >= 0.0) || !isfinite(sigma2) || !isfinite(phi) || !isfinite(tau2))
+        return 0;
+    const double span = cert_info_span(info) * (1.0 + 0x1p-40);
+    if (!(span >= 0.0) || !isfinite(span)) return 0;
+    if (kind != NNGP_KIND_SPHERICAL) {
+        const CovParams P = nngp_cov_params_unit(kind, phi, tau2 / sigma2);
+        if (!(span < P.d2max)) return 0;
+    }
+    const int64_t t = info[kCertITiles] - info[kCertIChecked];
+    return t > 0 ? t : 0;
+}
+
+}
diff --git a/pynngp_amd/csrc/nbr_cert.hip b/pynngp_amd/csrc/nbr_cert.hip
--- /dev/null
+++ b/pynngp_amd/csrc/nbr_cert.hip
@@ -0,0 +1,90 @@
+#include <hip/hip_runtime.h>
+
+#include "bf_pairb.h"
+#include "nbr_cert.h"
+#include "nngp_internal.h"
+
+namespace nngp {
+
+static_assert(kCertTileRows == kPairbTile && kCertMaxM == kPairbCertMaxM, "nbr_cert.h mirrors bf_pairb.h");
+
+__global__ __launch_bounds__(kCertTileRows) void cert_tiles_kernel(const int32_t* __restrict__ nbr, int64_t n_rows,
+                                                                   int m, int64_t n_points, int64_t tq, int64_t trem,
+                                                                   uint32_t* __restrict__ mask,
+                                                                   int32_t* __restrict__ n_checked) {
+    const int64_t t = blockIdx.x;
+    const int64_t r = t * tq + (t < trem ? t : trem) + threadIdx.x;
+    const bool live = (int64_t)threadIdx.x < tq + (t < trem ? 1 : 0) && r < n_rows;
+    bool any = false;
+    if (live) {
+        const int32_t* row = nbr + r * m;
+        for (int s = 0; s < m; ++s) any |= cert_slot_checked(row[s], n_points);
+    }
+    if (__syncthreads_or(any ? 1 : 0) != 0 && threadIdx.x == 0) {
+        atomicOr(&mask[t >> 5], 1u << (t & 31));
+        atomicAdd(n_checked, 1);
+    }
+}
+
+__global__ __launch_bounds__(256) void cert_span_kernel(const double* __restrict__ coords, int64_t n_points, int dim,
+                                                        double* __restrict__ rec) {
+    double mn[3] = {INFINITY, INFINITY, INFINITY}, mx[3] = {-INFINITY, -INFINITY, -INFINITY}, bad = 0.0;
+    for (int64_t p = (int64_t)blockIdx.x * 256 + threadIdx.x; p < n_points; p += (int64_t)gridDim.x * 256) {
+#pragma unroll
+        for (int c = 0; c < 3; ++c) {
+            if (c < dim) {
+                const double x = coords[p * dim + c];
+                if (!isfinite(x)) bad = 1.0;
+                mn[c] = fmin(mn[c], x);
+                mx[c] = fmax(mx[c], x);
+            }
+        }
+    }
+    __shared__ double sh[4][8];
+    const int w = threadIdx.x >> 6;
+#pragma unroll
+    for (int c = 0; c < 3; ++c) {
+        mn[c] = wave_min(mn[c]);
+        mx[c] = -wave_min(-mx[c]);
+    }
+    bad = -wave_min(-bad);
+    if ((threadIdx.x & 63) == 0) {
+#pragma unroll
+        for (int c = 0; c < 3; ++c) {
+            sh[w][c] = mn[c];
+            sh[w][3 + c] = mx[c];
+        }
+        sh[w][6] = bad;
+    }
+    __syncthreads();
+    if (threadIdx.x == 0) {
+        double* o = rec + 8 * (int64_t)blockIdx.x;
+#pragma unroll
+        for (int c = 0; c < 3; ++c) {
+            o[c] = fmin(fmin(sh[0][c], sh[1][c]), fmin(sh[2][c], sh[3][c]));
+            o[3 + c] = fmax(fmax(sh[0][3 + c], sh[1][3 + c]), fmax(sh[2][3 + c], sh[3][3 + c]));
+        }
+        o[6] = fmax(fmax(sh[0][6], sh[1][6]), fmax(sh[2][6], sh[3][6]));
+        o[7] = 0.0;
+    }
+}
+
+hipError_t nbr_cert_launch(const double* coords, int64_t n_points, int dim, const int32_t* nbr, int64_t n_rows, int m,
+                           void* cert, hipStream_t s) {
+    const PairbTiling tl = pairb_tiling(n_rows, m, 0);
+    if (tl.tiles != cert_tiles(n_rows)) return hipErrorInvalidValue;
+    char* base = (char*)cert;
+    hipError_t e = hipMemsetAsync(base, 0, cert_span_off(tl.tiles), s);
+    if (e != hipSuccess) return e;
+    if (tl.tiles > 0) {
+        hipLaunchKernelGGL(cert_tiles_kernel, dim3((unsigned)tl.tiles), dim3(kCertTileRows), 0, s, nbr, n_rows, m, n_points,
+                           tl.q, tl.rem, (uint32_t*)(base + kCertMaskOff), (int32_t*)base);
+        e = hipGetLastError();
+        if (e != hipSuccess) return e;
+    }
+    hipLaunchKernelGGL(cert_span_kernel, dim3(kCertSpanBlocks), dim3(256), 0, s, coords, n_points, dim,
+                       (double*)(base + cert_span_off(tl.tiles)));
+    return hipGetLastError();
+}
+
+}
diff --git a/pynngp_amd/csrc/nngp_internal.h b/pynngp_amd/csrc/nngp_internal.h
--- a/pynngp_amd/csrc/nngp_internal.h
+++ b/pynngp_amd/csrc/nngp_internal.h
@@ -80,6 +80,7 @@
     const double* cblk = nullptr;
     const int32_t* tiles = nullptr;
     int64_t n_tiles = 0, n_tile_list = 0, n_plan_blocks = 0;
+    const uint32_t* checked = nullptr;
 };
 
 int64_t bf_record_count(int64_t n_rows, int algo, int m);
@@ -99,6 +100,8 @@
 size_t pair_plan_build_lds(int m);
 hipError_t pair_plan_build_launch(const int32_t* nbr, const int32_t* order, int64_t n_rows, int m, int dim, int64_t i0,
                                   int64_t n_points, int64_t tq, int64_t trem, void* plan, hipStream_t s);
+hipError_t nbr_cert_launch(const double* coords, int64_t n_points, int dim, const int32_t* nbr, int64_t n_rows, int m,
+                           void* cert, hipStream_t s);
 bool bf_pairb_blocks_supported(int m);
 bool bf_group_blocks_launch(const BfArgs& a, hipStream_t s);
 bool bf_group_blocks_supported(int m);
diff --git a/pynngp_amd/csrc/nngp_math.h b/pynngp_amd/csrc/nngp_math.h
--- a/pynngp_amd/csrc/nngp_math.h
+++ b/pynngp_amd/csrc/nngp_math.h
@@ -450,10 +450,10 @@
     return fma(Ts, fq, Ts);
 }
 
-template <int KIND>
+template <int KIND, bool CLAMP = true>
 NNGP_FN double nngp_cov_unit(const CovParams& P, const double* tab, double d2) {
     if (KIND == NNGP_KIND_MATERN) return nngp_matern_tab(P, tab, d2);
-    const double x = fmin(d2, P.d2max);
+    const double x = CLAMP ? fmin(d2, P.d2max) : d2;
     if (KIND == NNGP_KIND_GAUSSIAN) return nngp_exp_unit(P, tab, x);
     const double d = nngp_sqrt(x);
     if (KIND == NNGP_KIND_SPHERICAL) {
diff --git a/pynngp_amd/csrc/torch_ops.cpp b/pynngp_amd/csrc/torch_ops.cpp
--- a/pynngp_amd/csrc/torch_ops.cpp
+++ b/pynngp_amd/csrc/torch_ops.cpp
@@ -93,7 +93,8 @@
                   const c10::optional<at::Tensor>& B, const c10::optional<at::Tensor>& F,
                   const c10::optional<at::Tensor>& R, const at::Tensor& partials, const at::Tensor& ws,
                   int64_t algo, double nu, const c10::optional<at::Tensor>& plan,
-                  const c10::optional<at::Tensor>& plan_info) {
+                  const c10::optional<at::Tensor>& plan_info, const c10::optional<at::Tensor>& cert,
+                  const c10::optional<at::Tensor>& cert_info) {
     check_coords(coords, "coords");
     const at::OptionalDeviceGuard guard(coords.device());
     check_nbr(nbr, coords);
@@ -125,6 +126,20 @@
                  "nngp_bf_sweep_plan");
         return;
     }
+    if (cert.has_value()) {
+        TORCH_CHECK(cert_info.has_value() && cert_info->device().is_cpu() && cert_info->scalar_type() == at::kLong &&
+                        cert_info->numel() == NNGP_CERT_INFO_LEN && cert_info->is_contiguous(),
+                    "cert_info must be the nbr_cert op's CPU int64 (", NNGP_CERT_INFO_LEN, ",) tensor");
+        TORCH_CHECK(cert->scalar_type() == at::kByte && cert->is_contiguous(), "cert must be a contiguous uint8 tensor");
+        check_same_device(coords, *cert, "cert");
+        check_rc(nngp_bf_sweep_cert(coords.data_ptr<double>(), n, (int32_t)d, nbr.data_ptr<int32_t>(), ptr<int32_t>(order),
+                                    rows, (int32_t)m, i0, (int32_t)kind, sigma2, phi, tau2, nu, ptr<double>(values),
+                                    ptr<double>(B), ptr<double>(F), ptr<double>(R), partials.data_ptr<double>(),
+                                    ws.data_ptr(), (size_t)ws.nbytes(), (int32_t)algo, cert->data_ptr(),
+                                    (size_t)cert->nbytes(), cert_info->data_ptr<int64_t>(), stream(coords)),
+                 "nngp_bf_sweep_cert");
+        return;
+    }
     check_rc(nngp_bf_sweep(coords.data_ptr<double>(), n, (int32_t)d, nbr.data_ptr<int32_t>(), ptr<int32_t>(order), rows,
                            (int32_t)m, i0, (int32_t)kind, sigma2, phi, tau2, nu, ptr<double>(values), ptr<double>(B),
                            ptr<double>(F), ptr<double>(R), partials.data_ptr<double>(), ws.data_ptr(),
@@ -150,7 +165,7 @@
     bf_sweep_out(coords, nbr, order, i0, kind, sigma2, phi, tau2, values,
                  want_bf ? c10::optional<at::Tensor>(B) : c10::nullopt,
                  want_bf ? c10::optional<at::Tensor>(F) : c10::nullopt, c10::nullopt, p, ws, algo, nu, c10::nullopt,
-                 c10::nullopt);
+                 c10::nullopt, c10::nullopt, c10::nullopt);
     return {B, F, p};
 }
 
@@ -203,6 +218,26 @@
     return {plan, info};
 }
 
+std::tuple<at::Tensor, at::Tensor> nbr_cert(const at::Tensor& coords, const at::Tensor& nbr,
+                                            const c10::optional<at::Tensor>& order, int64_t i0) {
+    check_coords(coords, "coords");
+    const at::OptionalDeviceGuard guard(coords.device());
+    check_nbr(nbr, coords);
+    const int64_t rows = nbr.size(0), m = nbr.size(1), n = coords.size(0), d = coords.size(1);
+    if (order.has_value()) {
+        TORCH_CHECK(order->scalar_type() == at::kInt && order->sizes() == at::IntArrayRef{rows} && order->is_contiguous(),
+                    "order must be a contiguous int32 (rows,) tensor");
+        check_same_device(coords, *order, "order");
+    }
+    auto cert = workspace((int64_t)nngp_nbr_cert_bytes(rows), coords);
+    auto info = at::empty({NNGP_CERT_INFO_LEN}, at::TensorOptions().dtype(at::kLong));
+    check_rc(nngp_nbr_cert_build(coords.data_ptr<double>(), n, (int32_t)d, nbr.data_ptr<int32_t>(), ptr<int32_t>(order),
+                                 rows, (int32_t)m, i0, cert.data_ptr(), (size_t)cert.nbytes(), info.data_ptr<int64_t>(),
+                                 stream(coords)),
+             "nngp_nbr_cert_build");
+    return {cert, info};
+}
+
 std::tuple<at::Tensor, at::Tensor> row_order(const at::Tensor& coords, int64_t i0, int64_t rows,
                                              const c10::optional<at::Tensor>& nbr) {
     check_coords(coords, "coords");
@@ -250,7 +285,9 @@
           "bool want_bf, int algo, Tensor? order=None, float nu=-1.0) -> (Tensor, Tensor, Tensor)");
     m.def("bf_sweep_out(Tensor coords, Tensor nbr, Tensor? order, int i0, int kind, float sigma2, float phi, "
           "float tau2, Tensor? values, Tensor(a!)? B, Tensor(b!)? F, Tensor(c!)? R, Tensor(d!) partials, "
-          "Tensor(e!) workspace, int algo, float nu=-1.0, Tensor? plan=None, Tensor? plan_info=None) -> ()");
+          "Tensor(e!) workspace, int algo, float nu=-1.0, Tensor? plan=None, Tensor? plan_info=None, "
+          "Tensor? cert=None, Tensor? cert_info=None) -> ()");
+    m.def("nbr_cert(Tensor coords, Tensor nbr, Tensor? order, int i0) -> (Tensor, Tensor)");
     m.def("pair_plan(Tensor nbr, Tensor? order, int i0, int n_points, int dim) -> (Tensor, Tensor)");
     m.def("bf_cross(Tensor ref, Tensor query, Tensor nbr, int kind, float sigma2, float phi, float tau2, "
           "Tensor? ref_values, int algo, float nu=-1.0) -> (Tensor, Tensor, Tensor)");
@@ -267,5 +304,6 @@
     m.impl("bf_cross", &bf_cross);
     m.impl("row_order", &row_order);
     m.impl("pair_plan", &pair_plan);
+    m.impl("nbr_cert", &nbr_cert);
     m.impl("combine_partials_out", &combine_partials_out);
 }
diff --git a/pynngp_amd/gibbs.py b/pynngp_amd/gibbs.py
--- a/pynngp_amd/gibbs.py
+++ b/pynngp_amd/gibbs.py
@@ -255,6 +255,9 @@
         if (self._use_plan and self._custom is None and algo in ("auto", "pairb")
                 and _lib.pair_plan_supported(self.m, kind, self.coords.shape[1])):
             self._plan = ops.pair_plan(self.nbr, None, 0, n, self.coords.shape[1])
+        self._cert = (None, None)
+        if self._custom is None and self._plan[0] is None and self.m >= 1 and ops.cert_default():
+            self._cert = ops.nbr_cert(self.coords, self.nbr, None, 0)
         self._stats_buf = z(2 + self.p)
         self._sweep_into(self.phi, self.B, self.Ft, self.r)
         self._prep = _lib.gibbs_prepare(self.B, self.Ft, self.off, self.rev_j, self.rev_k)
@@ -301,7 +304,8 @@
                                  partials=self._part, workspace=self._ws)
             return
         torch.ops.nngp.bf_sweep_out(self.coords, self.nbr, None, 0, self._kind_code, 1.0, float(phi), 0.0, self.w, B,
-                                    Ft, r, self._part, self._ws, self._algo_code, self._nu_arg, *self._plan)
+                                    Ft, r, self._part, self._ws, self._algo_code, self._nu_arg, *self._plan,
+                                    *self._cert)
 
     @staticmethod
     def _check(p):
diff --git a/pynngp_amd/ops.py b/pynngp_amd/ops.py
--- a/pynngp_amd/ops.py
+++ b/pynngp_amd/ops.py
@@ -52,8 +52,12 @@
 
     @fake("bf_sweep_out")
     def _(coords, nbr, order, i0, kind, sigma2, phi, tau2, values, B, F, R, partials, workspace, algo, nu=-1.0,
-          plan=None, plan_info=None):
+          plan=None, plan_info=None, cert=None, cert_info=None):
         return None
+
+    @fake("nbr_cert")
+    def _(coords, nbr, order, i0):
+        raise RuntimeError("nbr_cert is a setup call (it synchronises to read its tile counts): build it eagerly")
 
     @fake("pair_plan")
     def _(nbr, order, i0, n_points, dim):
@@ -89,13 +93,31 @@
 
 
 def bf_sweep_out(coords, nbr, order, i0, kind: str, theta, values, B, F, R, partials, workspace,
-                 algo: str = "auto", plan=None) -> None:
+                 algo: str = "auto", plan=None, cert=None) -> None:
     load()
     nu = float(theta[3]) if len(theta) > 3 else -1.0
     pbuf, pinfo = plan if plan is not None else (None, None)
+    cbuf, cinfo = cert if cert is not None else (None, None)
     torch.ops.nngp.bf_sweep_out(coords, nbr, order, int(i0), kind_code(kind), float(theta[0]), float(theta[1]),
                                 float(theta[2]), values, B, F, R, partials, workspace, algo_code(algo), nu, pbuf,
-                                pinfo)
+                                pinfo, cbuf, cinfo)
+
+
+def nbr_cert(coords, nbr, order, i0: int):
+    load()
+    return torch.ops.nngp.nbr_cert(coords, nbr, order, int(i0))
+
+
+def nbr_cert_trusted_tiles(cert_info, kind: str, theta) -> int:
+    import ctypes
+
+    info = (ctypes.c_int64 * _lib.CERT_INFO_LEN)(*[int(v) for v in cert_info.tolist()])
+    return int(_lib.load().nngp_nbr_cert_trusted_tiles(info, _lib.KIND_CODES.get(kind, 99), float(theta[0]),
+                                                       float(theta[1]), float(theta[2])))
+
+
+def cert_default() -> bool:
+    return os.environ.get("NNGP_NBR_CERT", "1") != "0"
 
 
 def pair_plan(nbr, order, i0: int, n_points: int, dim: int):
diff --git a/pynngp_amd/sweep.py b/pynngp_amd/sweep.py
--- a/pynngp_amd/sweep.py
+++ b/pynngp_amd/sweep.py
@@ -1,5 +1,6 @@
 from __future__ import annotations
 
+import ctypes
 import math
 import time
 from typing import Callable, Optional
@@ -106,6 +107,10 @@
             self.plan_read_bytes = _lib.pair_plan_read_bytes(self._plan[0], self.m)
         elif plan:
             raise ValueError(f"pair plans serve algo auto / pairb, 2 <= m <= 17, dim 1..3 (m={self.m}, dim={d})")
+        self._cert = self._cert_ctypes = None
+        if compute is None and self._plan is None and self.hi > self.lo and self.m >= 1 and ops.cert_default():
+            self._cert = ops.nbr_cert(self._coords_sweep, self._nbr_sweep, self.order, self.lo)
+            self._cert_ctypes = (self._cert[0], (ctypes.c_int64 * _lib.CERT_INFO_LEN)(*self._cert[1].tolist()))
 
     @property
     def planned(self) -> bool:
@@ -131,12 +136,14 @@
         if self.api == "ctypes":
             _lib.bf_sweep(self._coords_sweep, self._nbr_sweep, self.lo, cov.kind, s2, phi, tau2, values=values,
                           want_bf=want_bf, algo=self.algo, B=B, F=F, partials=p, workspace=self._ws, order=self.order,
-                          nu=cov.nu_arg, plan=self._plan_ctypes if plan is not None else None)
+                          nu=cov.nu_arg, plan=self._plan_ctypes if plan is not None else None,
+                          cert=self._cert_ctypes)
             return p
         pb, pi = plan if plan is not None else (None, None)
+        cb, ci = self._cert if self._cert is not None else (None, None)
         self._sweep_op(self._coords_sweep, self._nbr_sweep, self.order, self.lo, ops.kind_code(cov.kind),
                        float(s2), float(phi), float(tau2), values, B, F, None, p, self._ws, self._algo_code,
-                       -1.0 if cov.nu_arg is None else cov.nu_arg, pb, pi)
+                       -1.0 if cov.nu_arg is None else cov.nu_arg, pb, pi, cb, ci)
         return p
 
     def partials(self, cov: Covariance, values: Optional[torch.Tensor], want_bf: bool = True,
```

After: 5.944 billion (median of 6 runs). 1.02x the previous value.
